# Joao-M-Silva/padel_analytics

Measured on AMD Instinct MI355X. Metric: frames/sec (all trackers) on 1280x720, higher is better.
Workload: dtype f32-equivalent (h2: fp16 pairs h + m/2048, 2 or 3 f16 MFMA products per multiply, fp32 accumulate)

## Files before the change

### include/padel_hip.h

```cpp
#ifndef PADEL_HIP_H
#define PADEL_HIP_H

#include <stddef.h>
#include <stdint.h>

#ifdef __cplusplus
extern "C" {
#endif

typedef struct pa_engine pa_engine;
typedef struct pa_model pa_model;

#define PA_ABI_VERSION 5


enum pa_op_kind {
    PA_OP_STEM = 1,
    PA_OP_CONV = 2,
    PA_OP_SPPF_POOL = 3,
    PA_OP_UPSAMPLE2X = 4,
    PA_OP_MAXPOOL2 = 5,
    PA_OP_STEM7 = 6,
    PA_OP_MAXPOOL3S2 = 7,
    PA_OP_GAP_FC = 8,
    PA_OP_DWCONV3 = 9,
    PA_OP_PSA_ATTN = 10
};

enum pa_act { PA_ACT_NONE = 0, PA_ACT_SILU = 1, PA_ACT_RELU = 2, PA_ACT_SIGMOID = 3, PA_ACT_LEAKY = 4  };

typedef struct pa_buf_desc {
    int32_t level;
    int32_t channels;
} pa_buf_desc;

typedef struct pa_op_desc {
    int32_t kind;
    int32_t in_buf, in_choff, cin;
    int32_t out_buf, out_choff, cout;
    int32_t ksize, stride, act;
    int32_t res_buf, res_choff;
    int32_t npad;
    int32_t reserved;
    int64_t w_off, b_off;
    int32_t flags;
    int32_t pad_;
} pa_op_desc;
#define PA_CONV_W_SINGLE 1
#define PA_CONV_RES_PREACT 4

enum pa_task { PA_TASK_DETECT = 0, PA_TASK_POSE = 1, PA_TASK_TRACKNET = 2, PA_TASK_RESNET = 3  };

enum pa_dtype { PA_DTYPE_F32 = 0, PA_DTYPE_F16 = 1, PA_DTYPE_H2 = 2 };

typedef struct pa_model_desc {
    int32_t task;
    int32_t nc;
    int32_t nk, kpt_dim;
    int32_t n_bufs;
    const pa_buf_desc* bufs;
    int32_t n_ops;
    const pa_op_desc* ops;
    int32_t head_buf[3];
    int32_t in_channels;
    int32_t dtype;
} pa_model_desc;

int pa_abi_version(void);
int pa_device_count(void);
int pa_engine_create(int device_id, pa_engine** out);
void pa_engine_destroy(pa_engine* eng);
const char* pa_last_error(pa_engine* eng);
int pa_engine_synchronize(pa_engine* eng);

int pa_device_malloc(pa_engine* eng, size_t nbytes, void** out_dev);
int pa_device_free(pa_engine* eng, void* dev);
int pa_memcpy_h2d(pa_engine* eng, void* dst_dev, const void* src_host, size_t nbytes);
int pa_memcpy_d2h(pa_engine* eng, void* dst_host, const void* src_dev, size_t nbytes);
int pa_upload(pa_engine* eng, void* dst_dev, const void* src_host, size_t nbytes);

int pa_host_register(pa_engine* eng, void* ptr, size_t nbytes);
int pa_host_unregister(pa_engine* eng, void* ptr);

enum pa_yuv_layout {
    PA_YUV_NV12 = 0,
    PA_YUV_I420 = 1
};
typedef struct pa_yuv_desc {
    int32_t layout;
    int32_t pitch_y, pitch_c;
    int32_t off_u, off_v;
    int32_t reserved;
    int64_t frame_stride;
    int32_t y_off, cy, cvr, cug, cvg, cub;
} pa_yuv_desc;
int pa_yuv420_to_bgr(pa_engine* eng, const uint8_t* src, int src_on_device, int n, int h, int w,
                     const pa_yuv_desc* d, uint8_t* dst_bgr_dev);
int pa_yuv_last_path(pa_engine* eng);

enum pa_mark_kind { PA_MARK_DISC = 1, PA_MARK_SEGMENT = 2, PA_MARK_FILL = 3, PA_MARK_BOX = 4, PA_MARK_GLYPH = 5, PA_MARK_BLEND = 6 };
typedef struct pa_mark {
    int32_t kind;
    int32_t x0, y0, x1, y1;
    int32_t size;
    uint32_t bgr;
    int32_t arg;
} pa_mark;
typedef struct pa_yuv_enc {
    int32_t y_off;
    int32_t yr, yg, yb, ur, ug, ub, vr, vg, vb;
} pa_yuv_enc;
enum pa_render_out { PA_RENDER_BGR = 0, PA_RENDER_YUV420 = 1 };
int pa_render(pa_engine* eng, const uint8_t* src_bgr_dev, int n, int h, int w, const pa_mark* marks_host, const int32_t* first_host,
              int out, const pa_yuv_desc* geom, const pa_yuv_enc* enc, uint8_t* dst_dev);
int pa_render_check(int n, int h, int w, const pa_mark* marks_host, const int32_t* first_host, int out, const pa_yuv_desc* geom,
                    const pa_yuv_enc* enc, char* why, size_t cap);
int pa_render_last_path(pa_engine* eng);
int pa_glyph_rows(int code, uint8_t rows[7]);

#define PA_JPEG_MAX_WIDTH 2560
int pa_jpeg_encode(pa_engine* eng, const uint8_t* src_yuv_dev, int n, int h, int w, const pa_yuv_desc* geom, int quality,
                   uint8_t* dst_host, size_t cap, int64_t* offsets_host);
int pa_jpeg_check(int n, int h, int w, const pa_yuv_desc* geom, int quality, char* why, size_t cap);
size_t pa_jpeg_interval_bytes(int w);

#define PA_JPEG_DEC_MAX_DIM 4096
#define PA_JPEG_DEC_MAX_BYTES (1 << 27)
enum { PA_JPEG_ST_CODE = 1, PA_JPEG_ST_INDEX = 2, PA_JPEG_ST_SIZE = 4, PA_JPEG_ST_DATA = 8, PA_JPEG_ST_MARKERS = 16 };
typedef struct pa_jpeg_huff {
    uint8_t bits[16];
    uint8_t vals[256];
    int32_t nvals;
} pa_jpeg_huff;
typedef struct pa_jpeg_interval {
    int64_t begin, end;
    int32_t first_mcu, mcus;
} pa_jpeg_interval;
typedef struct pa_jpeg_frame_info {
    int32_t w, h, mcus_x, mcus_y;
    int32_t restart_interval;
    int32_t n_intervals;
    int32_t default_huffman;
    int32_t status;
    int64_t scan_begin, scan_end;
    uint8_t quant[3][64];
    uint8_t comp_dc[3], comp_ac[3], pad_[2];
    pa_jpeg_huff dc[2], ac[2];
} pa_jpeg_frame_info;
int pa_jpeg_parse(const uint8_t* jpeg, size_t len, pa_jpeg_frame_info* info, pa_jpeg_interval* ivls, size_t ivl_cap, char* why,
                  size_t cap);
int pa_jpeg_decode(pa_engine* eng, const uint8_t* jpegs_host, const int64_t* offsets, int n, int h, int w, uint8_t* dst_bgr_dev,
                   int32_t* status_host);
int pa_jpeg_decode_last_path(pa_engine* eng);
int pa_jpeg_decode_last_times(pa_engine* eng, double ms[5]);

int pa_engine_timer_start(pa_engine* eng);
int pa_engine_timer_stop(pa_engine* eng, float* ms);

int pa_engine_set_tuning(pa_engine* eng, const char* key, int value);
int pa_engine_set_timeline_path(pa_engine* eng, const char* path);

int pa_model_create(pa_engine* eng, const pa_model_desc* desc, const float* weights, size_t n_floats,
                    pa_model** out);
void pa_model_destroy(pa_model* m);
int pa_model_take_overflow(pa_model* m, int* out);
int pa_model_set_max_batch(pa_model* m, int max_batch);
int pa_model_plan_bytes(pa_model* m, size_t* arena_bytes, size_t* logical_bytes);

int pa_model_fill_arena(pa_model* m, int byte_value);

enum pa_pre_mode {
    PA_PRE_LETTERBOX = 0,
    PA_PRE_PIL_STRETCH = 1
};

typedef struct pa_yolo_params {
    int32_t imgsz;
    int32_t pre_mode;
    int32_t channel_reverse;
    int32_t letterbox_auto;
    float conf, iou;
    int32_t max_det;
    int32_t n_classes;
    const int32_t* classes;
    int32_t frames_on_device;
} pa_yolo_params;

int pa_yolo_infer(pa_model* m, const uint8_t* frames, int n, int h, int w, const pa_yolo_params* p,
                  float* out_boxes, float* out_kpts, int32_t* out_counts);

#define PA_MAX_INFLIGHT 4
int pa_yolo_submit(pa_model* m, const uint8_t* frames, int n, int h, int w, const pa_yolo_params* p,
                   float* out_boxes, float* out_kpts, int32_t* out_counts, int* ticket);
int pa_yolo_wait(pa_model* m, int ticket, int* overflow);

int pa_yolo_postprocess(pa_model* m, const float* const* heads, int n, int h, int w, const pa_yolo_params* p,
                        float* out_boxes, float* out_kpts, int32_t* out_counts);

int pa_yolo_head_shape(pa_model* m, int level, int* h, int* w, int* c);
int pa_yolo_read_head(pa_model* m, int level, int n, float* out);

int pa_yolo_netin_shape(pa_model* m, int* h, int* w);
int pa_yolo_read_netin(pa_model* m, int n, uint8_t* out);

int pa_tracknet_infer(pa_model* m, const float* x, int n, int h, int w, int x_on_device, float* out,
                      int out_on_device);

int pa_resnet_infer(pa_model* m, const uint8_t* frames, int n, int h, int w, int frames_on_device, float* out_xy, float* out_logits);
int pa_resnet_read_netin(pa_model* m, int n, uint8_t* out);
int pa_resnet_read_fc(pa_model* m, int n, float* out_xy, float* out_logits);
int pa_resnet_read_head(pa_model* m, int n, float* out);

int pa_pil_coeffs(int in_size, int out_size, int filter, int32_t* bounds, int32_t* coefs, int coefs_cap, int* ksize);

typedef struct pa_ball pa_ball;
int pa_ball_create(pa_model* tracknet, int src_h, int src_w, pa_ball** out);
void pa_ball_destroy(pa_ball* b);
int pa_ball_set_background(pa_ball* b, const uint8_t* median_rgb);
int pa_ball_background_from_frames(pa_ball* b, const uint8_t* frames_bgr, int n, int frames_on_device,
                                   uint8_t* out_median_rgb);
int pa_ball_feed(pa_ball* b, const uint8_t* frames_bgr, int n, int frames_on_device, int flush,
                 uint8_t* out_masks, float* out_heat, int32_t* out_rects, int* out_count);

int pa_ball_locate(pa_ball* b, const uint8_t* masks, int n, int32_t* out_rects);

int pa_ball_read_resized(pa_ball* b, long long frame, uint8_t* out);

int pa_comm_unique_id(void* out, size_t cap);
int pa_engine_comm_init(pa_engine* eng, const void* unique_id, size_t id_bytes, int nranks, int rank);
void pa_engine_comm_destroy(pa_engine* eng);
int pa_engine_bcast_weights(pa_engine* eng, pa_model* m, int root);
int pa_engine_bcast_weights_from(pa_engine* eng, pa_model* src, pa_model* dst, int root);
int pa_engine_bcast(pa_engine* eng, void* dev_ptr, size_t nbytes, int root);
int pa_engine_allreduce_max(pa_engine* eng, double* value);
int pa_engine_gather_sizes(pa_engine* eng, size_t nbytes, uint64_t* sizes);
int pa_engine_gather(pa_engine* eng, const void* send, size_t nbytes, void* recv, size_t recv_cap, const uint64_t* sizes, int root);

typedef struct pa_bytetrack pa_bytetrack;
int pa_bytetrack_create(double track_activation_threshold, int lost_track_buffer, double minimum_matching_threshold,
                        int frame_rate, pa_bytetrack** out);
void pa_bytetrack_destroy(pa_bytetrack* b);
void pa_bytetrack_reset(pa_bytetrack* b);
int pa_bytetrack_update_batch(pa_bytetrack* b, const float* boxes, const int32_t* counts, const uint8_t* keep,
                              int n_frames, int stride, int32_t* out_ids);

int pa_engine_set_profiling(pa_engine* eng, int enable);
int pa_model_last_profile(pa_model* m, int cap, int32_t* kinds, float* ms, double* flops, int32_t* ksizes);
int pa_model_profile_text(pa_model* m, char* buf, size_t cap);

#ifdef __cplusplus
}
#endif
#endif
```

### padel_analytics_amd/csrc/engine.cpp

```cpp
#include "engine_internal.h"

thread_local std::string g_err;

static int knob_raw(int v) { return v; }
static int knob_flag(int v) { return v ? 1 : 0; }
static int knob_tap_pd(int v) { return v == 3 ? 3 : 2; }
static const struct Knob { const char* key; const char* env; int Tuning::*field; int (*norm)(int); } kKnobs[] = {
    {"variant", "PADEL_CONV_VARIANT", &Tuning::variant, knob_raw},
    {"tune", "PADEL_CONV_TUNE", &Tuning::tune, knob_raw},
    {"tap_pd", "PADEL_CONV_TAP_PD", &Tuning::tap_pd, knob_tap_pd},
    {"graph", "PADEL_GRAPH", &Tuning::graph, knob_flag},
    {"timeline", nullptr, &Tuning::timeline, knob_flag},
    {"alias", "PADEL_ALIAS", &Tuning::alias, knob_flag},
    {"fold_up", "PADEL_FOLD_UP", &Tuning::fold_up, knob_flag},
    {"fuse_stem", "PADEL_FUSE_STEM", &Tuning::fuse_stem, knob_raw},
    {"fuse_sppf", "PADEL_FUSE_SPPF", &Tuning::fuse_sppf, knob_raw},
    {"w_single", nullptr, &Tuning::w_single, knob_flag},
};

int pa_abi_version(void) { return PA_ABI_VERSION; }

int pa_device_count(void) {
    int n = 0;
    if (hipGetDeviceCount(&n) != hipSuccess) return 0;
    return n;
}

const char* pa_last_error(pa_engine* eng) { return eng ? eng->err.c_str() : g_err.c_str(); }

int pa_engine_create(int device_id, pa_engine** out) {
    if (!out) PA_FAIL((pa_engine*)nullptr, "pa_engine_create: out is NULL");
    int n = 0;
    PA_HIP((pa_engine*)nullptr, hipGetDeviceCount(&n));
    if (device_id < 0 || device_id >= n) PA_FAIL((pa_engine*)nullptr, "pa_engine_create: device %d of %d", device_id, n);
    PA_HIP((pa_engine*)nullptr, hipSetDevice(device_id));
    pa_engine* e = new pa_engine();
    e->dev = device_id;
    hipError_t r = hipStreamCreateWithFlags(&e->stream, hipStreamNonBlocking);
    if (r != hipSuccess) { delete e; PA_FAIL((pa_engine*)nullptr, "hipStreamCreate: %s", hipGetErrorString(r)); }
    if (r == hipSuccess) r = hipStreamCreateWithFlags(&e->copy_stream, hipStreamNonBlocking);
    if (r != hipSuccess) { delete e; PA_FAIL((pa_engine*)nullptr, "hipStreamCreate: %s", hipGetErrorString(r)); }
    r = hipMalloc((void**)&e->zeros, 256);
    if (r == hipSuccess) r = hipMemset(e->zeros, 0, 256);
    if (r != hipSuccess) { delete e; PA_FAIL((pa_engine*)nullptr, "zero page: %s", hipGetErrorString(r)); }
    r = padel::init_misc_kernels();
    if (r != hipSuccess) { delete e; PA_FAIL((pa_engine*)nullptr, "kernel attributes: %s", hipGetErrorString(r)); }
    if (const char* v = getenv("PADEL_CONV_IMPL")) {
        if (v[0] == 'l') { delete e; PA_FAIL((pa_engine*)nullptr, "PADEL_CONV_IMPL=%s: the LDS kernel was retired in round 5; tap or bx3", v); }
        e->t.impl = (v[0] == 'b') ? 2 : 0;
    }
    for (const Knob& k : kKnobs)
        if (const char* v = k.env ? getenv(k.env) : nullptr) e->t.*k.field = k.norm(atoi(v));
    *out = e;
    return 0;
}

int pa_engine_set_tuning(pa_engine* e, const char* key, int value) {
    if (!e || !key) return 1;
    if (!strcmp(key, "impl")) {
        if (value != 0 && value != 2) PA_FAIL(e, "tuning impl = %d: 0 (fp32-input MFMA tap kernels) or 2 (bf16x3); 1 was the LDS kernel, retired in round 5 (tools/legacy_conv)", value);
        e->t.impl = value;
    } else {
        const Knob* k = std::find_if(std::begin(kKnobs), std::end(kKnobs), [&](const Knob& c) { return !strcmp(c.key, key); });
        if (k == std::end(kKnobs)) PA_FAIL(e, "pa_engine_set_tuning: unknown key '%s'", key);
        e->t.*k->field = k->norm(value);
    }
    e->tuning_epoch++;
    return 0;
}

int pa_engine_set_timeline_path(pa_engine* e, const char* path) {
    if (!e) return 1;
    e->timeline_path = path ? path : "";
    return 0;
}

void pa_engine_destroy(pa_engine* e) {
    if (!e) return;
    hipSetDevice(e->dev);
    pa_engine_comm_destroy(e);
    if (e->zeros) hipFree(e->zeros);
    if (e->yuv_stage) { if (e->stream) hipStreamSynchronize(e->stream); hipFree(e->yuv_stage); }
    if (e->render_stage) { if (e->stream) hipStreamSynchronize(e->stream); hipFree(e->render_stage); }
    jpeg_scratch_free(e);
    jpeg_dec_scratch_free(e);
    for (hipEvent_t ev : e->timer_ev) if (ev) hipEventDestroy(ev);
    if (e->stream) hipStreamDestroy(e->stream);
    if (e->copy_stream) hipStreamDestroy(e->copy_stream);
    delete e;
}

int pa_engine_synchronize(pa_engine* e) {
    PA_HIP(e, hipSetDevice(e->dev));
    PA_HIP(e, hipStreamSynchronize(e->stream));
    return 0;
}

int pa_engine_set_profiling(pa_engine* e, int enable) { e->profiling = enable != 0; return 0; }

int pa_device_malloc(pa_engine* e, size_t nbytes, void** out) {
    PA_HIP(e, hipSetDevice(e->dev));
    PA_HIP(e, hipMalloc(out, nbytes));
    return 0;
}
int pa_device_free(pa_engine* e, void* p) {
    PA_HIP(e, hipSetDevice(e->dev));
    PA_HIP(e, hipFree(p));
    return 0;
}
int pa_memcpy_h2d(pa_engine* e, void* dst, const void* src, size_t n) {
    PA_HIP(e, hipSetDevice(e->dev));
    PA_HIP(e, hipMemcpyAsync(dst, src, n, hipMemcpyHostToDevice, e->stream));
    PA_HIP(e, hipStreamSynchronize(e->stream));
    return 0;
}
int pa_upload(pa_engine* e, void* dst, const void* src, size_t n) {
    PA_HIP(e, hipSetDevice(e->dev));
    PA_HIP(e, hipMemcpyAsync(dst, src, n, hipMemcpyHostToDevice, e->copy_stream));
    PA_HIP(e, hipStreamSynchronize(e->copy_stream));
    return 0;
}
int pa_host_register(pa_engine* e, void* ptr, size_t nbytes) {
    PA_HIP(e, hipSetDevice(e->dev));
    PA_HIP(e, hipHostRegister(ptr, nbytes, hipHostRegisterDefault));
    return 0;
}
int pa_host_unregister(pa_engine* e, void* ptr) {
    PA_HIP(e, hipSetDevice(e->dev));
    PA_HIP(e, hipHostUnregister(ptr));
    return 0;
}
int pa_memcpy_d2h(pa_engine* e, void* dst, const void* src, size_t n) {
    PA_HIP(e, hipSetDevice(e->dev));
    PA_HIP(e, hipMemcpyAsync(dst, src, n, hipMemcpyDeviceToHost, e->stream));
    PA_HIP(e, hipStreamSynchronize(e->stream));
    return 0;
}

int pa_engine_timer_start(pa_engine* e) {
    if (!e) return 1;
    PA_HIP(e, hipSetDevice(e->dev));
    for (hipEvent_t& ev : e->timer_ev) if (!ev) PA_HIP(e, hipEventCreate(&ev));
    PA_HIP(e, hipEventRecord(e->timer_ev[0], e->stream));
    return 0;
}
int pa_engine_timer_stop(pa_engine* e, float* ms) {
    if (!e || !ms) return 1;
    if (!e->timer_ev[0] || !e->timer_ev[1]) PA_FAIL(e, "pa_engine_timer_stop without pa_engine_timer_start");
    PA_HIP(e, hipSetDevice(e->dev));
    PA_HIP(e, hipEventRecord(e->timer_ev[1], e->stream));
    PA_HIP(e, hipEventSynchronize(e->timer_ev[1]));
    PA_HIP(e, hipEventElapsedTime(ms, e->timer_ev[0], e->timer_ev[1]));
    return 0;
}

int pa_model_create(pa_engine* e, const pa_model_desc* desc, const float* weights, size_t n_floats, pa_model** out) {
    if (!e || !desc || !out) PA_FAIL(e, "pa_model_create: NULL argument");
    std::string why;
    if (validate_desc(desc, n_floats, why)) PA_FAIL(e, "%s", why.c_str());
    PA_HIP(e, hipSetDevice(e->dev));
    pa_model* m = new pa_model();
    m->e = e;
    m->d = *desc;
    m->bufs.assign(desc->bufs, desc->bufs + desc->n_bufs);
    m->ops.assign(desc->ops, desc->ops + desc->n_ops);
    m->d.bufs = m->bufs.data();
    m->d.ops = m->ops.data();
    find_upsample_folds(m->d, m->fold_src, m->fold_dst);
    m->stem_fuse.resize(m->ops.size());
    for (size_t i = 0; i < m->ops.size(); ++i) m->stem_fuse[i] = stem_fusable(m->d, i);
    m->n_w = n_floats;
    hipError_t r = hipMalloc((void**)&m->d_w, n_floats * sizeof(float) + kConvReadSlack);
    if (r == hipSuccess)
        r = weights ? hipMemcpyAsync(m->d_w, weights, n_floats * sizeof(float), hipMemcpyHostToDevice, e->stream)
                    : hipMemsetAsync(m->d_w, 0, n_floats * sizeof(float), e->stream);
    if (r == hipSuccess) r = hipMemsetAsync(m->d_w + n_floats, 0, kConvReadSlack, e->stream);
    if (r == hipSuccess) r = hipMalloc((void**)&m->d_ovf, 256);
    if (r == hipSuccess) r = hipMemsetAsync(m->d_ovf, 0, 256, e->stream);
    if (r == hipSuccess) r = hipHostMalloc((void**)&m->h_pin, 64 * sizeof(unsigned), hipHostMallocDefault);
    if (r == hipSuccess) memset(m->h_pin, 0, 64 * sizeof(unsigned));
    for (int k = 0; k < PA_MAX_INFLIGHT && r == hipSuccess; ++k) r = hipEventCreateWithFlags(&m->tk_ev[k], hipEventDisableTiming);
    if (r == hipSuccess) r = hipStreamSynchronize(e->stream);
    if (r != hipSuccess) { delete m; PA_FAIL(e, "weights upload: %s", hipGetErrorString(r)); }
    *out = m;
    return 0;
}

static void destroy_graphs(pa_model* m) {
    for (auto& g : m->graphs) hipGraphExecDestroy(g.second);
    m->graphs.clear();
}

void free_plan(pa_model* m) {
    destroy_graphs(m);
    if (m->arena) hipFree(m->arena);
    m->arena = nullptr;
    m->bptr.clear();
    void* ptrs[] = {m->d_netin, m->d_xtab, m->d_ytab, m->d_cand,
                    m->d_cidx, m->d_ccnt, m->d_keys, m->d_order, m->d_supp, m->d_oboxes, m->d_okpts, m->d_ocnt, m->d_fc};
    for (void* p : ptrs) if (p) hipFree(p);
    resample_free(&m->rs);
    m->d_fc = nullptr;
    m->d_netin = nullptr;
    m->d_xtab = m->d_ytab = nullptr;
    m->d_cand = nullptr; m->d_cidx = m->d_ccnt = nullptr; m->d_keys = nullptr; m->d_order = nullptr; m->d_supp = nullptr;
    m->d_oboxes = m->d_okpts = nullptr; m->d_ocnt = nullptr;
    m->planned = false;
}

void pa_model_destroy(pa_model* m) {
    if (!m) return;
    hipSetDevice(m->e->dev);
    hipStreamSynchronize(m->e->stream);
    free_plan(m);
    for (auto& r : m->prof) { hipEventDestroy(r.e0); hipEventDestroy(r.e1); }
    if (m->d_frames) hipFree(m->d_frames);
    if (m->d_classes) hipFree(m->d_classes);
    if (m->d_w) hipFree(m->d_w);
    if (m->d_wr) hipFree(m->d_wr);
    if (m->d_ovf) hipFree(m->d_ovf);
    if (m->d_stage) hipFree(m->d_stage);
    if (m->h_pin) hipHostFree(m->h_pin);
    for (int k = 0; k < PA_MAX_INFLIGHT; ++k) if (m->tk_ev[k]) hipEventDestroy(m->tk_ev[k]);
    delete m;
}

int pa_model_take_overflow(pa_model* m, int* out) {
    if (!m || !out) return 1;
    pa_engine* e = m->e;
    *out = 0;
    if (m->d.dtype != PA_DTYPE_H2) return 0;
    PA_HIP(e, hipSetDevice(e->dev));
    unsigned v = 0;
    if (m->ovf_cached) {
        v = m->h_ovf;
    } else {
        PA_HIP(e, hipMemcpyAsync(&v, m->d_ovf, sizeof(v), hipMemcpyDeviceToHost, e->stream));
        PA_HIP(e, hipStreamSynchronize(e->stream));
    }
    m->ovf_cached = false;
    m->h_ovf = 0;
    if (v) {
        PA_HIP(e, hipMemsetAsync(m->d_ovf, 0, sizeof(v), e->stream));
        PA_HIP(e, hipStreamSynchronize(e->stream));
    }
    *out = v ? 1 : 0;
    return 0;
}

int pa_model_set_max_batch(pa_model* m, int max_batch) {
    if (max_batch < 1) PA_FAIL(m->e, "max_batch %d", max_batch);
    if (max_batch != m->max_batch) { hipSetDevice(m->e->dev); hipStreamSynchronize(m->e->stream); free_plan(m); m->max_batch = max_batch; }
    return 0;
}

int plan_buffers(pa_model* m, int batch) {
    pa_engine* e = m->e;
    BufferPlan bp;
    std::string why;
    if (plan_activations(m->d, m->fold_src, m->net_h, m->net_w, batch, e->t.alias != 0, bp, why)) PA_FAIL(e, "%s", why.c_str());
    m->fc_nout = 0;
    for (const auto& o : m->ops) if (o.kind == PA_OP_GAP_FC) m->fc_nout = o.cout;
    if (m->fc_nout) {
        PA_HIP(e, hipMalloc((void**)&m->d_fc, (size_t)batch * 2 * kGapFcMaxOut * sizeof(float)));
        PA_HIP(e, hipMemsetAsync(m->d_fc, 0, (size_t)batch * 2 * kGapFcMaxOut * sizeof(float), e->stream));
    }
    PA_HIP(e, hipMalloc(&m->arena, bp.arena_bytes + kConvReadSlack));
    PA_HIP(e, hipMemsetAsync(m->arena, 0, bp.arena_bytes + kConvReadSlack, e->stream));
    m->bptr.assign(m->bufs.size(), nullptr);
    for (size_t i = 0; i < m->bufs.size(); ++i) m->bptr[i] = reinterpret_cast<float*>(static_cast<char*>(m->arena) + bp.off[i]);
    m->arena_bytes = bp.arena_bytes;
    m->logical_bytes = bp.logical_bytes;
    m->p_batch = batch;
    return 0;
}

ProfRec* prof_begin(pa_model* m, size_t idx, int kind, int ksize, double flops) {
    if (!m->e->profiling) return nullptr;
    if (m->prof.size() <= idx) {
        m->prof.resize(idx + 1);
        hipEventCreate(&m->prof[idx].e0);
        hipEventCreate(&m->prof[idx].e1);
    }
    ProfRec* r = &m->prof[idx];
    r->kind = kind; r->ksize = ksize; r->flops = flops; r->ms = 0.f;
    r->M = r->cout = r->cin = r->stride = r->mf = r->nf = r->res = 0;
    r->tile = -1; r->family = "";
    hipEventRecord(r->e0, m->e->stream);
    return r;
}

static bool fold_active(const pa_model* m, int conv_op) {
    if (m->d.dtype == PA_DTYPE_H2) return m->e->t.fold_up && m->fold_src[conv_op] >= 0;
    return m->e->t.fold_up && m->e->t.impl == 2 && m->d.dtype != PA_DTYPE_F16 && m->fold_src[conv_op] >= 0;
}

static int conv_launch_args(const pa_model* m, size_t i, int n, ConvArgs& a, int* path_out = nullptr) {
    const pa_engine* e = m->e;
    const pa_op_desc& o = m->ops[i];
    const pa_buf_desc& ob = m->bufs[o.out_buf];
    const pa_buf_desc& ib = m->bufs[o.in_buf];
    const int Ho = m->net_h >> ob.level, Wo = m->net_w >> ob.level;
    a.in = m->bptr[o.in_buf]; a.in_cs = ib.channels; a.in_choff = o.in_choff;
    a.out = m->bptr[o.out_buf]; a.out_cs = ob.channels; a.out_choff = o.out_choff;
    a.res = o.res_buf >= 0 ? m->bptr[o.res_buf] : nullptr;
    a.res_cs = o.res_buf >= 0 ? m->bufs[o.res_buf].channels : 0; a.res_choff = o.res_choff;
    a.res_pre = (o.res_buf >= 0 && (o.flags & PA_CONV_RES_PREACT)) ? 1 : 0;
    a.zeros = e->zeros;
    a.w = m->d_w + o.w_off; a.bias = m->d_w + o.b_off;
    a.H = m->net_h >> ib.level; a.W = m->net_w >> ib.level; a.Ho = Ho; a.Wo = Wo;
    a.cin = o.cin; a.cout = o.cout; a.n16 = o.npad / 16; a.ksize = o.ksize; a.stride = o.stride; a.act = o.act;
    a.M = n * Ho * Wo;
    fill_fastdiv((unsigned)(Ho * Wo), &a.howo_magic, &a.howo_shift);
    fill_fastdiv((unsigned)Wo, &a.wo_magic, &a.wo_shift);
    a.tune = e->t.tune; a.tap_pd = e->t.tap_pd;
    const bool f16 = m->d.dtype == PA_DTYPE_F16, h2 = m->d.dtype == PA_DTYPE_H2;
    const bool use_bx3 = !f16 && !h2 && e->t.impl == 2 && o.reserved > 0;
    a.w3 = use_bx3 ? (const void*)(m->d_w + o.reserved) : nullptr;
    a.out_f32 = (f16 || h2) && is_head_buf(m->d, o.out_buf);
    const int path = h2 ? CONV_PATH_H2 : f16 ? CONV_PATH_F16 : use_bx3 ? CONV_PATH_BX3 : CONV_PATH_TAP;
    if (path_out) *path_out = path;
    if (h2) {
        a.oscale = m->d_w + o.reserved;
        a.ovf_flag = m->d_ovf;
        a.w_single = (o.flags & PA_CONV_W_SINGLE) && e->t.w_single ? 1 : 0;
        a.wr = (m->wr_valid && i < m->wr_off.size() && m->wr_off[i] >= 0) ? (const void*)(m->d_wr + m->wr_off[i]) : nullptr;
    }
    const int lv = e->t.variant >= 0 ? e->t.variant
                   : h2 ? choose_conv_h2_variant(a)
                   : f16 ? choose_conv_tap16_variant(a)
                   : use_bx3 ? choose_conv_bx3_variant(a)
                         : choose_conv_tap_variant(a.M, a.n16);
    if ((h2 || use_bx3) && fold_active(m, (int)i)) {
        const pa_op_desc& u = m->ops[m->fold_src[i]];
        a.in2 = m->bptr[u.in_buf]; a.in2_cs = m->bufs[u.in_buf].channels; a.in2_choff = u.in_choff; a.up_c = u.cin;
        if (!resolve_conv(path, a, lv, nullptr)) { a.in2 = nullptr; a.in2_cs = a.in2_choff = a.up_c = 0; }
    }
    return lv;
}

static int run_ops(pa_model* m, int n, size_t* pi) {
    pa_engine* e = m->e;
    hipStream_t s = e->stream;
    for (size_t i = 0; i < m->ops.size(); ++i) {
        const pa_op_desc& o = m->ops[i];
        const pa_buf_desc& ob = m->bufs[o.out_buf];
        const int Ho = m->net_h >> ob.level, Wo = m->net_w >> ob.level;
        hipError_t r = hipSuccess;
        ProfRec* pr = nullptr;
        if (o.kind == PA_OP_CONV) {
            ConvArgs a{};
            int path = CONV_PATH_TAP;
            const int lv = conv_launch_args(m, i, n, a, &path);
            const bool f16 = path == CONV_PATH_F16, h2 = path == CONV_PATH_H2, use_bx3 = path == CONV_PATH_BX3;
            int bm = 0, bn = 0;
            conv_tile_shape(path, lv, &bm, &bn);
            pr = prof_begin(m, (*pi)++, o.kind, o.ksize, 2.0 * a.M * (double)o.cout * o.cin * o.ksize * o.ksize);
            if (pr) { pr->M = a.M; pr->cout = o.cout; pr->cin = o.cin; pr->stride = o.stride; pr->mf = bm; pr->nf = bn; pr->res = a.res != nullptr; }
            unsigned long long* dbg_dev = nullptr;
            size_t dbg_bytes = 0;
            ConvLaunched will{-1, ""};
            if (e->t.timeline && !e->timeline_path.empty() && resolve_conv(path, a, lv, &will) && will.tile == lv) {
                const size_t patches = (size_t)n * ((a.Ho + 7) / 8) * ((a.Wo + 15) / 16);
                const size_t records = h2 ? 8 * ((patches + 7) / 8) * (size_t)((a.n16 + 5) / 6) : (size_t)((a.M + 63) / 64) * ((o.npad + 95) / 96);
                dbg_bytes = records * conv_timeline_words(will, o.ksize) * 8;
            }
            if (dbg_bytes) {
                if (hipMalloc(&dbg_dev, dbg_bytes) == hipSuccess) (void)hipMemsetAsync(dbg_dev, 0, dbg_bytes, s);
                else dbg_dev = nullptr;
                a.dbg = dbg_dev;
            }
            ConvLaunched ran{-1, ""};
            if (a.res_pre && !h2 && !use_bx3)
                PA_FAIL(e, "op %zu: PA_CONV_RES_PREACT needs the h2 or the bf16x3 kernels (tuning impl = 2, bf16x3 weights in the blob), not the %s family",
                        i, f16 ? "fp16" : "fp32-MFMA tap");
            r = launch_conv(path, a, lv, s, &ran);
            if (pr) { pr->tile = ran.tile; pr->family = ran.family; }
            if (dbg_dev) {
                (void)hipStreamSynchronize(s);
                std::vector<unsigned long long> host(dbg_bytes / 8);
                (void)hipMemcpy(host.data(), dbg_dev, dbg_bytes, hipMemcpyDeviceToHost);
                if (FILE* f = fopen(e->timeline_path.c_str(), "wb")) { fwrite(host.data(), 1, dbg_bytes, f); fclose(f); }
                (void)hipFree(dbg_dev);
            }
        } else if (o.kind == PA_OP_STEM) {
            StemArgs a{};
            a.in = m->d_netin; a.w = m->d_w + o.w_off; a.bias = m->d_w + o.b_off;
            a.out = m->bptr[o.out_buf]; a.out_cs = ob.channels; a.out_choff = o.out_choff;
            a.H = m->net_h; a.W = m->net_w; a.Ho = Ho; a.Wo = Wo; a.cout = o.cout; a.B = n;
            a.out_f16 = m->d.dtype == PA_DTYPE_F16 ? 1 : m->d.dtype == PA_DTYPE_H2 ? 2 : 0;
            a.ovf_flag = m->d_ovf;
            a.opw = (m->wr_valid && i < m->wr_off.size() && m->wr_off[i] >= 0) ? (const void*)(m->d_wr + m->wr_off[i]) : nullptr;
            pr = prof_begin(m, (*pi)++, o.kind, 3, 2.0 * n * Ho * Wo * (double)o.cout * 27);
            if (e->t.fuse_stem && m->d.dtype == PA_DTYPE_H2 && m->stem_fuse[i]) {
                ConvArgs ca{};
                conv_launch_args(m, i + 1, n, ca);
                if (stem_l1_h2_supported(a, ca)) {
                    r = launch_stem_l1_h2(a, ca, s);
                    prof_end(m, pr);
                    if (r != hipSuccess) PA_FAIL(e, "fused stem + layer 1 launch failed: %s", hipGetErrorString(r));
                    ++i;
                    continue;
                }
            }
            r = launch_stem(a, s);
        } else if (o.kind == PA_OP_SPPF_POOL) {
            pr = prof_begin(m, (*pi)++, o.kind, 5, 0.0);
            r = launch_sppf_pool(m->bptr[o.in_buf], m->bufs[o.in_buf].channels, o.in_choff, o.cin, n, Ho, Wo, s, (int)m->d.dtype, e->t.fuse_sppf);
        } else if (o.kind == PA_OP_UPSAMPLE2X) {
            if (m->fold_dst[i] >= 0) {
                ConvArgs ca{};
                conv_launch_args(m, (size_t)m->fold_dst[i], n, ca);
                if (ca.in2) continue;
            }
            pr = prof_begin(m, (*pi)++, o.kind, 0, 0.0);
            r = launch_upsample2x(m->bptr[o.in_buf], m->bufs[o.in_buf].channels, o.in_choff, m->bptr[o.out_buf],
                                  ob.channels, o.out_choff, o.cin, n, Ho / 2, Wo / 2, s, (int)m->d.dtype);
        } else if (o.kind == PA_OP_MAXPOOL2) {
            pr = prof_begin(m, (*pi)++, o.kind, 2, 0.0);
            r = launch_maxpool2(m->bptr[o.in_buf], m->bufs[o.in_buf].channels, o.in_choff, m->bptr[o.out_buf],
                                ob.channels, o.out_choff, o.cin, n, Ho * 2, Wo * 2, s, (int)m->d.dtype);
        } else if (o.kind == PA_OP_MAXPOOL3S2) {
            const int lin = m->bufs[o.in_buf].level;
            pr = prof_begin(m, (*pi)++, o.kind, 3, 0.0);
            r = launch_maxpool3s2(m->bptr[o.in_buf], m->bufs[o.in_buf].channels, o.in_choff, m->bptr[o.out_buf], ob.channels, o.out_choff,
                                  o.cin, n, m->net_h >> lin, m->net_w >> lin, Ho, Wo, s, m->d.dtype == PA_DTYPE_H2 ? 1 : 0);
        } else if (o.kind == PA_OP_STEM7) {
            if (!m->d_netin) PA_FAIL(e, "op %zu: the 7x7 stem reads the u8 network input of pa_resnet_infer", i);
            const bool head = is_head_buf(m->d, o.out_buf);
            Stem7Args a{};
            a.in = m->d_netin; a.w = m->d_w + o.w_off; a.bias = m->d_w + o.b_off; a.lut = m->d_w + o.reserved;
            a.out = m->bptr[o.out_buf]; a.out_cs = ob.channels; a.out_choff = o.out_choff;
            a.H = m->net_h; a.W = m->net_w; a.Ho = Ho; a.Wo = Wo; a.B = n; a.act = o.act;
            a.out_h2 = (m->d.dtype == PA_DTYPE_H2 && !head) ? 1 : 0;
            a.ovf_flag = m->d_ovf;
            pr = prof_begin(m, (*pi)++, o.kind, 7, 2.0 * n * Ho * Wo * 64.0 * 147.0);
            if (pr) { pr->M = n * Ho * Wo; pr->cout = 64; pr->cin = 3; pr->stride = 2; }
            r = launch_stem7(a, s);
        } else if (o.kind == PA_OP_GAP_FC) {
            const int lin = m->bufs[o.in_buf].level;
            const int hw = (m->net_h >> lin) * (m->net_w >> lin);
            pr = prof_begin(m, (*pi)++, o.kind, 0, 2.0 * n * (double)o.cout * o.cin);
            if (pr) { pr->M = n; pr->cout = o.cout; pr->cin = o.cin; }
            r = launch_gap_fc(m->bptr[o.in_buf], m->bufs[o.in_buf].channels, o.in_choff, o.cin, n, hw, m->d_w + o.w_off, m->d_w + o.b_off,
                              o.cout, m->d_fc, m->d_fc + (size_t)m->p_batch * kGapFcMaxOut, s, m->d.dtype == PA_DTYPE_H2 ? 1 : 0);
        } else if (o.kind == PA_OP_DWCONV3) {
            const bool h2 = m->d.dtype == PA_DTYPE_H2;
            const bool head = is_head_buf(m->d, o.out_buf);
            DwConvArgs a{};
            a.in = m->bptr[o.in_buf]; a.in_cs = m->bufs[o.in_buf].channels; a.in_choff = o.in_choff;
            a.w = m->d_w + o.w_off; a.bias = m->d_w + o.b_off;
            a.out = m->bptr[o.out_buf]; a.out_cs = ob.channels; a.out_choff = o.out_choff;
            if (o.res_buf >= 0) { a.res = m->bptr[o.res_buf]; a.res_cs = m->bufs[o.res_buf].channels; a.res_choff = o.res_choff; }
            a.C = o.cin; a.B = n; a.H = Ho; a.W = Wo; a.act = o.act;
            a.h2 = h2 ? 1 : 0; a.out_f32 = (h2 && head) ? 1 : 0; a.ovf_flag = m->d_ovf;
            pr = prof_begin(m, (*pi)++, o.kind, 3, 2.0 * n * Ho * Wo * (double)o.cin * 9.0);
            if (pr) { pr->M = n * Ho * Wo; pr->cout = o.cout; pr->cin = o.cin; pr->stride = 1; pr->res = o.res_buf >= 0; }
            r = launch_dwconv3(a, s);
        } else if (o.kind == PA_OP_PSA_ATTN) {
            const bool h2 = m->d.dtype == PA_DTYPE_H2;
            const bool head = is_head_buf(m->d, o.out_buf);
            AttnArgs a{};
            a.heads = o.stride; a.kd = o.ksize; a.hd = o.npad;
            a.qkv = m->bptr[o.in_buf]; a.cs = m->bufs[o.in_buf].channels;
            a.q_choff = o.in_choff; a.k_choff = o.in_choff + a.heads * a.kd; a.v_choff = o.in_choff + 2 * a.heads * a.kd;
            a.out = m->bptr[o.out_buf]; a.out_cs = ob.channels; a.out_choff = o.out_choff;
            a.N = Ho * Wo; a.B = n; a.scale = (float)(1.0 / std::sqrt((double)a.kd));
            a.h2 = h2 ? 1 : 0; a.out_f32 = (h2 && head) ? 1 : 0; a.ovf_flag = m->d_ovf;
            pr = prof_begin(m, (*pi)++, o.kind, 0, 2.0 * n * (double)a.heads * a.N * (double)a.N * (a.kd + a.hd));
            if (pr) { pr->M = n * a.N; pr->cout = o.cout; pr->cin = o.cin; pr->stride = a.heads; }
            r = launch_psa_attn(a, s);
        }
        prof_end(m, pr);
        if (r != hipSuccess) PA_FAIL(e, "op %zu (kind %d) launch failed: %s", i, o.kind, hipGetErrorString(r));
    }
    return 0;
}

static int ensure_operand_copies(pa_model* m) {
    if (m->wr_valid || m->d.dtype != PA_DTYPE_H2) return 0;
    pa_engine* e = m->e;
    {
        bool any = false;
        PA_HIP(e, hipMemsetAsync(m->d_ovf + 32, 0, sizeof(unsigned) * 8, e->stream));
        for (size_t i = 0; i < m->ops.size(); ++i) {
            const pa_op_desc& o = m->ops[i];
            if (o.kind != PA_OP_CONV || !(o.flags & PA_CONV_W_SINGLE)) continue;
            PA_HIP(e, launch_h2_mplane_check(m->d_w + o.w_off, (long long)o.npad * h2_ksteps(o.cin, o.ksize), m->d_ovf + 32, e->stream));
            any = true;
        }
        if (any) {
            unsigned bad = 0;
            PA_HIP(e, hipMemcpyAsync(&bad, m->d_ovf + 32, sizeof(bad), hipMemcpyDeviceToHost, e->stream));
            PA_HIP(e, hipStreamSynchronize(e->stream));
            if (bad) PA_FAIL(e, "a conv flagged PA_CONV_W_SINGLE has a non-zero m plane in the weight blob (pack it without the flag, or with fp16-number weights)");
        }
    }
    if (m->wr_off.empty()) {
        std::vector<long long> off(m->ops.size(), -1);
        size_t total = 0;
        for (size_t i = 0; i < m->ops.size(); ++i) {
            const pa_op_desc& o = m->ops[i];
            if (o.kind == PA_OP_STEM && m->stem_fuse[i] && (o.cout == 16 || o.cout == 32 || o.cout == 48)) {
                off[i] = (long long)total;
                total += (stem_l1_operand_bytes(o.cout) + 2047) / 2048 * 2048;
                continue;
            }
            if (o.kind != PA_OP_CONV || !conv_wants_operand_copy(o.ksize, o.stride, o.cin, (o.flags & PA_CONV_W_SINGLE) != 0)) continue;
            off[i] = (long long)total;
            total += conv_h2r_copy_bytes(o.npad / 16, o.cin, o.ksize);
        }
        if (total) {
            PA_HIP(e, hipMalloc((void**)&m->d_wr, total + 8192));
            PA_HIP(e, hipMemsetAsync(m->d_wr + total, 0, 8192, e->stream));
        }
        m->wr_off = std::move(off);
    }
    for (size_t i = 0; i < m->ops.size(); ++i) {
        if (m->wr_off[i] < 0) continue;
        const pa_op_desc& o = m->ops[i];
        if (o.kind == PA_OP_STEM) {
            PA_HIP(e, launch_stem_l1_operands(m->d_w + o.w_off, o.cout, m->d_wr + m->wr_off[i], e->stream));
            continue;
        }
        PA_HIP(e, launch_h2r_repack(m->d_w + o.w_off, m->d_wr + m->wr_off[i], o.npad / 16, o.cin, o.ksize, e->stream));
    }
    m->wr_valid = true;
    return 0;
}

int run_graph(pa_model* m, int n, size_t* pi) {
    pa_engine* e = m->e;
    if (ensure_operand_copies(m)) return 1;
    if (!e->t.graph || e->profiling || e->t.timeline) return run_ops(m, n, pi);
    if (m->graph_epoch != e->tuning_epoch) {
        PA_HIP(e, hipStreamSynchronize(e->stream));
        destroy_graphs(m);
        m->graph_epoch = e->tuning_epoch;
    }
    auto it = m->graphs.find(n);
    if (it == m->graphs.end()) {
        hipGraph_t g = nullptr;
        hipGraphExec_t ge = nullptr;
        PA_HIP(e, hipStreamBeginCapture(e->stream, hipStreamCaptureModeThreadLocal));
        size_t dummy = 0;
        const int rc = run_ops(m, n, &dummy);
        const hipError_t r = hipStreamEndCapture(e->stream, &g);
        if (rc) { if (g) hipGraphDestroy(g); return 1; }
        if (r != hipSuccess) PA_FAIL(e, "hipStreamEndCapture: %s", hipGetErrorString(r));
        const hipError_t ri = hipGraphInstantiate(&ge, g, nullptr, nullptr, 0);
        hipGraphDestroy(g);
        if (ri != hipSuccess) PA_FAIL(e, "hipGraphInstantiate: %s", hipGetErrorString(ri));
        it = m->graphs.emplace(n, ge).first;
    }
    PA_HIP(e, hipGraphLaunch(it->second, e->stream));
    return 0;
}

int finish_profile(pa_model* m, size_t n_rec) {
    if (!m->e->profiling) { m->n_prof = 0; return 0; }
    for (size_t i = 0; i < n_rec && i < m->prof.size(); ++i)
        hipEventElapsedTime(&m->prof[i].ms, m->prof[i].e0, m->prof[i].e1);
    m->n_prof = n_rec;
    return 0;
}

int pa_model_plan_bytes(pa_model* m, size_t* arena_bytes, size_t* logical_bytes) {
    if (!m->planned) PA_FAIL(m->e, "pa_model_plan_bytes: no plan yet");
    if (arena_bytes) *arena_bytes = m->arena_bytes;
    if (logical_bytes) *logical_bytes = m->logical_bytes;
    return 0;
}

int pa_model_fill_arena(pa_model* m, int byte_value) {
    if (!m) return 1;
    pa_engine* e = m->e;
    if (!m->planned || !m->arena) PA_FAIL(e, "pa_model_fill_arena: no plan yet");
    PA_HIP(e, hipSetDevice(e->dev));
    PA_HIP(e, hipMemsetAsync(m->arena, byte_value & 0xFF, m->arena_bytes, e->stream));
    if (m->d_netin) PA_HIP(e, hipMemsetAsync(m->d_netin, byte_value & 0xFF, (size_t)m->p_batch * m->net_h * m->net_w * 4, e->stream));
    PA_HIP(e, hipStreamSynchronize(e->stream));
    return 0;
}

int pa_model_profile_text(pa_model* m, char* buf, size_t cap) {
    size_t off = 0;
    for (size_t i = 0; i < m->n_prof && i < m->prof.size(); ++i) {
        const ProfRec& r = m->prof[i];
        int n = snprintf(buf + off, off < cap ? cap - off : 0, "%d,%d,%d,%d,%d,%d,%d,%d,%.5f,%.0f,%d,%d,%s\n", r.kind, r.ksize, r.M, r.cout,
                         r.cin, r.stride, r.mf, r.nf, r.ms, r.flops, r.res, r.tile, r.family ? r.family : "");
        if (n < 0 || off + n >= cap) break;
        off += n;
    }
    if (off < cap) buf[off] = 0;
    return (int)off;
}

int pa_model_last_profile(pa_model* m, int cap, int32_t* kinds, float* ms, double* flops, int32_t* ksizes) {
    int n = 0;
    for (size_t i = 0; i < m->n_prof && i < m->prof.size() && n < cap; ++i, ++n) {
        kinds[n] = m->prof[i].kind; ms[n] = m->prof[i].ms; flops[n] = m->prof[i].flops; ksizes[n] = m->prof[i].ksize;
    }
    return n;
}
```

### padel_analytics_amd/csrc/engine_internal.h

```cpp
#pragma once
#include "../../include/padel_hip.h"
#include "graph_plan.h"
#include "kernels.h"

#include <algorithm>
#include <cmath>
#include <cstdio>
#include <cstdlib>
#include <cstring>
#include <map>
#include <string>
#include <vector>

using namespace padel;

struct Tuning {
    int impl = 2;
    int variant = -1;
    int tune = 1;
    int tap_pd = 2;
    int graph = 0;
    int timeline = 0;
    int alias = 1;
    int fuse_stem = 1;
    int w_single = 1;
    int fuse_sppf = 1;
    int fold_up = 1;
};

struct pa_comm;
struct JpegScratch;
struct JpegDecScratch;

struct pa_engine {
    int dev = 0;
    hipStream_t stream = nullptr;
    hipStream_t copy_stream = nullptr;
    std::string err;
    bool profiling = false;
    float* zeros = nullptr;
    Tuning t;
    int tuning_epoch = 0;
    std::string timeline_path;
    pa_comm* comm = nullptr;
    uint8_t* yuv_stage = nullptr; size_t yuv_stage_cap = 0;
    int yuv_last_path = 0;
    hipEvent_t timer_ev[2]{};
    uint8_t* render_stage = nullptr; size_t render_stage_cap = 0;
    int render_last_path = 0;
    JpegScratch* jpeg = nullptr;
    JpegDecScratch* jpeg_dec = nullptr;
    int jpeg_dec_last_path = 0;
};

extern thread_local std::string g_err;

#define PA_FAIL(eng, ...)                                        \
    do {                                                         \
        char _b[512];                                            \
        snprintf(_b, sizeof(_b), __VA_ARGS__);                   \
        if (eng) (eng)->err = _b; else g_err = _b;               \
        return 1;                                                \
    } while (0)

#define PA_HIP(eng, call)                                                                  \
    do {                                                                                   \
        hipError_t _e = (call);                                                            \
        if (_e != hipSuccess) {                                                            \
            (void)hipGetLastError();    \
            PA_FAIL(eng, "%s failed: %s (%s:%d)", #call, hipGetErrorString(_e), __FILE__, __LINE__); \
        }                                                                                  \
    } while (0)

struct ProfRec { int kind; int ksize; double flops; hipEvent_t e0, e1; float ms; int M, cout, cin, stride, mf, nf, res; int tile; const char* family; };
enum { PROF_PRE = 100, PROF_DECODE = 101, PROF_NMS = 102 };

struct ResamplePlan {
    int sh = 0, sw = 0, dh = 0, dw = 0;
    int32_t *d_hb = nullptr, *d_hk = nullptr, *d_vb = nullptr, *d_vk = nullptr;
    int hks = 0, vks = 0;
    uint8_t* d_tmp = nullptr;
};

struct pa_model {
    pa_engine* e = nullptr;
    pa_model_desc d{};
    std::vector<pa_buf_desc> bufs;
    std::vector<pa_op_desc> ops;
    std::vector<int> fold_src;
    std::vector<int> fold_dst;
    std::vector<char> stem_fuse;
    float* d_w = nullptr;
    size_t n_w = 0;
    char* d_wr = nullptr;
    std::vector<long long> wr_off;
    bool wr_valid = false;
    unsigned* d_ovf = nullptr;
    float* d_stage = nullptr; size_t stage_cap = 0;
    float* d_fc = nullptr;
    int fc_nout = 0;
    int max_batch = 64;

    bool planned = false;
    int p_h0 = 0, p_w0 = 0, p_imgsz = 0, p_pre = 0, p_auto = 0, p_batch = 0;
    int net_h = 0, net_w = 0;
    int rw = 0, rh = 0, top = 0, left = 0, lb_mode = 0;
    std::vector<float*> bptr;
    void* arena = nullptr;
    size_t arena_bytes = 0, logical_bytes = 0;
    unsigned h_ovf = 0;
    bool ovf_cached = false;
    unsigned* h_pin = nullptr;
    hipEvent_t tk_ev[PA_MAX_INFLIGHT]{};
    bool tk_busy[PA_MAX_INFLIGHT]{};
    int next_ticket = 0, n_inflight = 0;
    std::vector<int32_t> classes_host;
    std::map<int, hipGraphExec_t> graphs;
    int graph_epoch = -1;
    uint8_t* d_frames = nullptr; size_t frames_cap = 0;
    uint8_t* d_netin = nullptr;
    int32_t *d_xtab = nullptr, *d_ytab = nullptr;
    ResamplePlan rs;
    int A = 0, P2 = 0;
    HeadLevel lv[3]{};
    float* d_cand = nullptr; int32_t* d_cidx = nullptr; int32_t* d_ccnt = nullptr;
    uint64_t* d_keys = nullptr; int32_t* d_order = nullptr; uint8_t* d_supp = nullptr;
    float* d_oboxes = nullptr; float* d_okpts = nullptr; int32_t* d_ocnt = nullptr;
    int32_t* d_classes = nullptr; int classes_cap = 0;
    int last_n = 0;
    std::vector<ProfRec> prof;
    size_t n_prof = 0;
};

ProfRec* prof_begin(pa_model* m, size_t idx, int kind, int ksize, double flops);
inline void prof_end(pa_model* m, ProfRec* r) { if (r) hipEventRecord(r->e1, m->e->stream); }
int finish_profile(pa_model* m, size_t n_rec);
void free_plan(pa_model* m);
int plan_buffers(pa_model* m, int batch);
int run_graph(pa_model* m, int n, size_t* pi);

void jpeg_scratch_free(pa_engine* e);

void jpeg_dec_scratch_free(pa_engine* e);

hipError_t upload_table(pa_engine* e, int32_t** dptr, const std::vector<int32_t>& v);
int stage_frames(pa_model* m, const uint8_t** src, int nb, size_t frame_bytes);
int resample_plan(pa_engine* e, ResamplePlan* rs, int sh, int sw, int dh, int dw, int filter, int max_batch, bool identity_pass = false);
void resample_free(ResamplePlan* rs);
hipError_t resample_enqueue(const ResamplePlan& rs, const uint8_t* src, uint8_t* dst, int n, int out_c, int reverse, hipStream_t s);
```

### padel_analytics_amd/csrc/engine_yolo.cpp

```cpp
#include "engine_internal.h"

static int plan_yolo(pa_model* m, int h0, int w0, const pa_yolo_params* p) {
    pa_engine* e = m->e;
    PA_HIP(e, hipStreamSynchronize(e->stream));
    free_plan(m);
    const int S = p->imgsz;
    YoloGeometry g;
    std::string why;
    if (yolo_geometry(h0, w0, S, p->pre_mode, p->letterbox_auto, g, why)) PA_FAIL(e, "%s", why.c_str());
    m->rw = g.rw; m->rh = g.rh; m->top = g.top; m->left = g.left; m->lb_mode = g.lb_mode;
    m->net_h = g.net_h; m->net_w = g.net_w;
    if (m->lb_mode == 2) {
        std::vector<int32_t> xt, yt;
        cv2_linear_table(w0, m->rw, xt);
        cv2_linear_table(h0, m->rh, yt);
        PA_HIP(e, upload_table(e, &m->d_xtab, xt));
        PA_HIP(e, upload_table(e, &m->d_ytab, yt));
    }
    if (p->pre_mode == PA_PRE_PIL_STRETCH && resample_plan(e, &m->rs, h0, w0, S, S, PIL_BICUBIC, m->max_batch)) return 1;
    const int B = m->max_batch;
    PA_HIP(e, hipMalloc((void**)&m->d_netin, (size_t)B * m->net_h * m->net_w * 4));
    if (plan_buffers(m, B)) return 1;
    for (int l = 0; l < 3; ++l) m->lv[l] = HeadLevel{m->bptr[m->d.head_buf[l]], g.lv[l].H, g.lv[l].W, g.lv[l].stride, g.lv[l].anchor0};
    m->A = g.A;
    m->P2 = g.P2;
    PA_HIP(e, hipMalloc((void**)&m->d_cand, (size_t)B * m->A * 6 * sizeof(float)));
    PA_HIP(e, hipMalloc((void**)&m->d_cidx, (size_t)B * m->A * sizeof(int32_t)));
    PA_HIP(e, hipMalloc((void**)&m->d_ccnt, (size_t)B * sizeof(int32_t)));
    PA_HIP(e, hipMalloc((void**)&m->d_keys, (size_t)B * m->P2 * sizeof(uint64_t)));
    PA_HIP(e, hipMalloc((void**)&m->d_order, (size_t)B * m->A * sizeof(int32_t)));
    PA_HIP(e, hipMalloc((void**)&m->d_supp, (size_t)B * m->A));
    PA_HIP(e, hipMalloc((void**)&m->d_oboxes, (size_t)B * 300 * 6 * sizeof(float)));
    PA_HIP(e, hipMalloc((void**)&m->d_ocnt, (size_t)B * sizeof(int32_t)));
    if (m->d.nk) PA_HIP(e, hipMalloc((void**)&m->d_okpts, (size_t)B * 300 * m->d.nk * sizeof(float)));
    PA_HIP(e, hipStreamSynchronize(e->stream));
    m->p_h0 = h0; m->p_w0 = w0; m->p_imgsz = S; m->p_pre = p->pre_mode; m->p_auto = p->letterbox_auto;
    m->planned = true;
    return 0;
}

static int run_post(pa_model* m, const pa_yolo_params* p, int nb, int oh, int ow, size_t* ppi, float* out_boxes, float* out_kpts,
                int32_t* out_counts, int ovf_slot) {
    pa_engine* e = m->e;
    hipStream_t s = e->stream;
    size_t& pi = *ppi;
    ProfRec* pr = nullptr;
    hipError_t r = hipSuccess;
    const double gain = std::min((double)m->net_h / oh, (double)m->net_w / ow);
    const double kpx = (m->net_w - ow * gain) / 2, kpy = (m->net_h - oh * gain) / 2;
    DecodeArgs da{};
    for (int l = 0; l < 3; ++l) da.lv[l] = m->lv[l];
    da.cs = m->bufs[m->d.head_buf[0]].channels; da.nc = m->d.nc; da.nk = m->d.nk; da.kdim = m->d.kpt_dim;
    da.A = m->A; da.B = nb; da.conf = p->conf; da.classes = m->d_classes; da.n_classes = p->n_classes;
    da.cand = m->d_cand; da.cand_idx = m->d_cidx; da.cand_cnt = m->d_ccnt;
    pr = prof_begin(m, pi++, PROF_DECODE, 0, 0.0);
    r = launch_decode(da, s);
    prof_end(m, pr);
    if (r != hipSuccess) PA_FAIL(e, "decode launch failed: %s", hipGetErrorString(r));
    NmsArgs na{};
    na.cand = m->d_cand; na.cand_idx = m->d_cidx; na.cand_cnt = m->d_ccnt; na.keys = m->d_keys;
    na.order = m->d_order; na.supp = m->d_supp;
    for (int l = 0; l < 3; ++l) na.lv[l] = m->lv[l];
    na.cs = da.cs; na.nc = m->d.nc; na.nk = m->d.nk; na.kdim = m->d.kpt_dim; na.A = m->A; na.B = nb; na.P2 = m->P2;
    na.iou = p->iou; na.max_det = p->max_det; na.max_nms = 30000;
    na.gain = (float)gain;
    na.pad_x = (float)std::nearbyint(kpx - 0.1); na.pad_y = (float)std::nearbyint(kpy - 0.1);
    na.kpad_x = (float)kpx; na.kpad_y = (float)kpy;
    na.w0 = (float)ow; na.h0 = (float)oh;
    na.out_boxes = m->d_oboxes; na.out_kpts = m->d_okpts; na.out_cnt = m->d_ocnt;
    pr = prof_begin(m, pi++, PROF_NMS, 0, 0.0);
    r = launch_nms(na, s);
    prof_end(m, pr);
    if (r != hipSuccess) PA_FAIL(e, "nms launch failed: %s", hipGetErrorString(r));
    if (m->d.dtype == PA_DTYPE_H2)
        PA_HIP(e, hipMemcpyAsync(m->h_pin + ovf_slot, m->d_ovf, sizeof(unsigned), hipMemcpyDeviceToHost, s));
    PA_HIP(e, hipMemcpyAsync(out_counts, m->d_ocnt, nb * sizeof(int32_t), hipMemcpyDeviceToHost, s));
    PA_HIP(e, hipMemcpyAsync(out_boxes, m->d_oboxes,
                             (size_t)nb * p->max_det * 6 * sizeof(float), hipMemcpyDeviceToHost, s));
    if (m->d.nk)
        PA_HIP(e, hipMemcpyAsync(out_kpts, m->d_okpts,
                                 (size_t)nb * p->max_det * m->d.nk * sizeof(float), hipMemcpyDeviceToHost, s));
    return 0;
}

static bool yolo_plan_current(const pa_model* m, int h, int w, const pa_yolo_params* p) {
    return m->planned && m->p_h0 == h && m->p_w0 == w && m->p_imgsz == p->imgsz && m->p_pre == p->pre_mode &&
           m->p_auto == p->letterbox_auto && m->p_batch == m->max_batch;
}

static int set_classes(pa_model* m, const pa_yolo_params* p) {
    pa_engine* e = m->e;
    if (p->n_classes <= 0) return 0;
    if ((int)m->classes_host.size() == p->n_classes && !memcmp(m->classes_host.data(), p->classes, p->n_classes * sizeof(int32_t))) return 0;
    PA_HIP(e, hipStreamSynchronize(e->stream));
    if (p->n_classes > m->classes_cap) {
        if (m->d_classes) hipFree(m->d_classes);
        m->d_classes = nullptr; m->classes_cap = 0; m->classes_host.clear();
        PA_HIP(e, hipMalloc((void**)&m->d_classes, p->n_classes * sizeof(int32_t)));
        m->classes_cap = p->n_classes;
    }
    m->classes_host.assign(p->classes, p->classes + p->n_classes);
    PA_HIP(e, hipMemcpy(m->d_classes, m->classes_host.data(), p->n_classes * sizeof(int32_t), hipMemcpyHostToDevice));
    return 0;
}

static int yolo_prepare(pa_model* m, const uint8_t* frames, int n, int h, int w, const pa_yolo_params* p, float* out_boxes,
                        float* out_kpts, int32_t* out_counts, const char* who) {
    pa_engine* e = m->e;
    if (m->d.task != PA_TASK_DETECT && m->d.task != PA_TASK_POSE) PA_FAIL(e, "%s on a non-YOLO model", who);
    if (!frames || n <= 0 || h <= 0 || w <= 0 || !out_boxes || !out_counts) PA_FAIL(e, "%s: bad arguments", who);
    if (m->d.nk && !out_kpts) PA_FAIL(e, "%s: out_kpts is NULL for a pose model", who);
    if (p->max_det < 1 || p->max_det > 300) PA_FAIL(e, "max_det %d outside [1,300]", p->max_det);
    PA_HIP(e, hipSetDevice(e->dev));
    if (!yolo_plan_current(m, h, w, p)) {
        if (m->n_inflight) PA_FAIL(e, "%s: the plan would change (source size / imgsz / batch) with %d ticket(s) in flight", who, m->n_inflight);
        if (plan_yolo(m, h, w, p)) return 1;
    }
    return set_classes(m, p);
}

static int yolo_enqueue(pa_model* m, const uint8_t* src, int nb, int h, int w, const pa_yolo_params* p, float* out_boxes,
                        float* out_kpts, int32_t* out_counts, int ovf_slot, size_t* ppi) {
    pa_engine* e = m->e;
    hipStream_t s = e->stream;
    size_t& pi = *ppi;
    const size_t frame_bytes = (size_t)h * w * 3;
    const int S = p->imgsz;
    const int oh = p->pre_mode == PA_PRE_PIL_STRETCH ? S : h, ow = p->pre_mode == PA_PRE_PIL_STRETCH ? S : w;
    if (!p->frames_on_device && stage_frames(m, &src, nb, frame_bytes)) return 1;
    ProfRec* pr = prof_begin(m, pi++, PROF_PRE, 0, 0.0);
    hipError_t r = hipSuccess;
    if (p->pre_mode == PA_PRE_LETTERBOX || (h == S && w == S)) {
        LetterboxArgs a{};
        a.src = src; a.dst = m->d_netin; a.B = nb; a.h0 = h; a.w0 = w; a.rw = m->rw; a.rh = m->rh;
        a.top = m->top; a.left = m->left; a.nh = m->net_h; a.nw = m->net_w; a.mode = m->lb_mode;
        a.reverse = p->channel_reverse; a.xtab = m->d_xtab; a.ytab = m->d_ytab;
        r = launch_letterbox(a, s);
    } else {
        r = resample_enqueue(m->rs, src, m->d_netin, nb, 4, p->channel_reverse, s);
    }
    prof_end(m, pr);
    if (r != hipSuccess) PA_FAIL(e, "preprocess launch failed: %s", hipGetErrorString(r));
    if (run_graph(m, nb, &pi)) return 1;
    return run_post(m, p, nb, oh, ow, &pi, out_boxes, m->d.nk ? out_kpts : nullptr, out_counts, ovf_slot);
}

int pa_yolo_infer(pa_model* m, const uint8_t* frames, int n, int h, int w, const pa_yolo_params* p,
                  float* out_boxes, float* out_kpts, int32_t* out_counts) {
    if (!m || !p) return 1;
    pa_engine* e = m->e;
    if (yolo_prepare(m, frames, n, h, w, p, out_boxes, out_kpts, out_counts, "pa_yolo_infer")) return 1;
    hipStream_t s = e->stream;
    const size_t frame_bytes = (size_t)h * w * 3;
    size_t pi = 0;
    for (int c0 = 0; c0 < n; c0 += m->max_batch) {
        const int nb = std::min(m->max_batch, n - c0);
        if (yolo_enqueue(m, frames + (size_t)c0 * frame_bytes, nb, h, w, p, out_boxes + (size_t)c0 * p->max_det * 6,
                         m->d.nk ? out_kpts + (size_t)c0 * p->max_det * m->d.nk : nullptr, out_counts + c0, PA_MAX_INFLIGHT, &pi))
            return 1;
        PA_HIP(e, hipStreamSynchronize(s));
        m->last_n = nb;
        if (m->d.dtype == PA_DTYPE_H2) { m->h_ovf |= m->h_pin[PA_MAX_INFLIGHT]; m->ovf_cached = true; }
    }
    finish_profile(m, pi);
    return 0;
}

int pa_yolo_submit(pa_model* m, const uint8_t* frames, int n, int h, int w, const pa_yolo_params* p,
                   float* out_boxes, float* out_kpts, int32_t* out_counts, int* ticket) {
    if (!m || !p || !ticket) return 1;
    pa_engine* e = m->e;
    if (!p->frames_on_device) PA_FAIL(e, "pa_yolo_submit: frames must be in HBM (frames_on_device = 1)");
    if (n > m->max_batch) PA_FAIL(e, "pa_yolo_submit: n = %d > max_batch %d", n, m->max_batch);
    if (e->profiling || e->t.timeline) PA_FAIL(e, "pa_yolo_submit: not while profiling (use pa_yolo_infer)");
    const int slot = m->next_ticket % PA_MAX_INFLIGHT;
    if (m->tk_busy[slot]) PA_FAIL(e, "pa_yolo_submit: %d tickets in flight (PA_MAX_INFLIGHT)", PA_MAX_INFLIGHT);
    if (yolo_prepare(m, frames, n, h, w, p, out_boxes, out_kpts, out_counts, "pa_yolo_submit")) return 1;
    size_t pi = 0;
    if (yolo_enqueue(m, frames, n, h, w, p, out_boxes, out_kpts, out_counts, slot, &pi)) {
        (void)hipStreamSynchronize(e->stream);
        return 1;
    }
    PA_HIP(e, hipEventRecord(m->tk_ev[slot], e->stream));
    m->tk_busy[slot] = true;
    ++m->n_inflight;
    m->last_n = n;
    m->n_prof = 0;
    m->ovf_cached = false;
    *ticket = m->next_ticket++;
    return 0;
}

int pa_yolo_wait(pa_model* m, int ticket, int* overflow) {
    if (!m) return 1;
    pa_engine* e = m->e;
    const int slot = ticket % PA_MAX_INFLIGHT;
    if (ticket < 0 || ticket >= m->next_ticket || ticket + PA_MAX_INFLIGHT < m->next_ticket || !m->tk_busy[slot])
        PA_FAIL(e, "pa_yolo_wait: ticket %d is not in flight", ticket);
    PA_HIP(e, hipSetDevice(e->dev));
    PA_HIP(e, hipEventSynchronize(m->tk_ev[slot]));
    m->tk_busy[slot] = false;
    --m->n_inflight;
    if (overflow) *overflow = (m->d.dtype == PA_DTYPE_H2 && m->h_pin[slot]) ? 1 : 0;
    return 0;
}

int pa_yolo_postprocess(pa_model* m, const float* const* heads, int n, int h, int w, const pa_yolo_params* p,
                        float* out_boxes, float* out_kpts, int32_t* out_counts) {
    if (!m || !p || !heads) return 1;
    pa_engine* e = m->e;
    if (m->d.task != PA_TASK_DETECT && m->d.task != PA_TASK_POSE) PA_FAIL(e, "pa_yolo_postprocess on a non-YOLO model");
    if (n <= 0 || n > m->max_batch || !out_boxes || !out_counts || (m->d.nk && !out_kpts)) PA_FAIL(e, "pa_yolo_postprocess: bad arguments");
    if (p->max_det < 1 || p->max_det > 300) PA_FAIL(e, "max_det %d outside [1,300]", p->max_det);
    PA_HIP(e, hipSetDevice(e->dev));
    if (!yolo_plan_current(m, h, w, p) && plan_yolo(m, h, w, p)) return 1;
    if (set_classes(m, p)) return 1;
    hipStream_t s = e->stream;
    const int cs = m->bufs[m->d.head_buf[0]].channels;
    for (int l = 0; l < 3; ++l) {
        if (!heads[l]) PA_FAIL(e, "pa_yolo_postprocess: heads[%d] is NULL", l);
        PA_HIP(e, hipMemcpyAsync(const_cast<float*>(m->lv[l].buf), heads[l], (size_t)n * m->lv[l].H * m->lv[l].W * cs * sizeof(float),
                                 hipMemcpyHostToDevice, s));
    }
    const int S = p->imgsz;
    const int oh = p->pre_mode == PA_PRE_PIL_STRETCH ? S : h, ow = p->pre_mode == PA_PRE_PIL_STRETCH ? S : w;
    size_t pi = 0;
    if (run_post(m, p, n, oh, ow, &pi, out_boxes, out_kpts, out_counts, PA_MAX_INFLIGHT)) return 1;
    PA_HIP(e, hipStreamSynchronize(s));
    m->last_n = n;
    finish_profile(m, pi);
    return 0;
}

int pa_yolo_head_shape(pa_model* m, int level, int* h, int* w, int* c) {
    if (!m->planned || level < 0 || level > 2) PA_FAIL(m->e, "pa_yolo_head_shape: no plan / bad level");
    *h = m->lv[level].H; *w = m->lv[level].W; *c = m->bufs[m->d.head_buf[0]].channels;
    return 0;
}

int pa_yolo_read_head(pa_model* m, int level, int n, float* out) {
    pa_engine* e = m->e;
    if (!m->planned || level < 0 || level > 2 || n > m->last_n) PA_FAIL(e, "pa_yolo_read_head: no plan / bad level / n");
    PA_HIP(e, hipSetDevice(e->dev));
    const size_t bytes = (size_t)n * m->lv[level].H * m->lv[level].W * m->bufs[m->d.head_buf[0]].channels * sizeof(float);
    PA_HIP(e, hipMemcpyAsync(out, m->lv[level].buf, bytes, hipMemcpyDeviceToHost, e->stream));
    PA_HIP(e, hipStreamSynchronize(e->stream));
    return 0;
}

int pa_yolo_netin_shape(pa_model* m, int* h, int* w) {
    if (!m->planned || m->d.task == PA_TASK_TRACKNET) PA_FAIL(m->e, "pa_yolo_netin_shape: no YOLO plan");
    *h = m->net_h; *w = m->net_w;
    return 0;
}

int pa_yolo_read_netin(pa_model* m, int n, uint8_t* out) {
    pa_engine* e = m->e;
    if (!m->planned || !m->d_netin || n < 1 || n > m->last_n || !out) PA_FAIL(e, "pa_yolo_read_netin: no plan / bad n");
    PA_HIP(e, hipSetDevice(e->dev));
    PA_HIP(e, hipMemcpyAsync(out, m->d_netin, (size_t)n * m->net_h * m->net_w * 4, hipMemcpyDeviceToHost, e->stream));
    PA_HIP(e, hipStreamSynchronize(e->stream));
    return 0;
}
```

### padel_analytics_amd/csrc/graph_plan.cpp

```cpp
#include "graph_plan.h"
#include "kernels.h"

#include <algorithm>
#include <cmath>
#include <cstdio>

namespace padel {

#define FAIL(...)                                                \
    do {                                                         \
        char _b[512];                                            \
        snprintf(_b, sizeof(_b), __VA_ARGS__);                   \
        err = _b;                                                \
        return 1;                                                \
    } while (0)

int validate_desc(const pa_model_desc* d, size_t n_floats, std::string& err) {
    if (d->n_bufs <= 0 || d->n_ops <= 0 || !d->bufs || !d->ops) FAIL("model desc: empty graph");
    const bool f16 = d->dtype == PA_DTYPE_F16, h2 = d->dtype == PA_DTYPE_H2;
    if (d->dtype != PA_DTYPE_F32 && d->dtype != PA_DTYPE_F16 && d->dtype != PA_DTYPE_H2) FAIL("model desc: dtype %d", d->dtype);
    const int kalign = f16 ? 31 : 15, valign = f16 ? 7 : 3;
    for (int i = 0; i < d->n_bufs; ++i)
        if (d->bufs[i].level < 0 || d->bufs[i].level > 6 || d->bufs[i].channels <= 0 || (d->bufs[i].channels & 3))
            FAIL("model desc: buffer %d (level %d, channels %d)", i, d->bufs[i].level, d->bufs[i].channels);
    auto okslice = [&](int b, int off, int c) {
        return b >= 0 && b < d->n_bufs && off >= 0 && c > 0 && off + c <= d->bufs[b].channels;
    };
    if (h2)
        for (int i = 0; i < d->n_bufs; ++i)
            if (!is_head_buf(*d, i) && (d->bufs[i].channels & 15)) FAIL("model desc: h2 buffer %d has %d channels", i, d->bufs[i].channels);
    for (int i = 0; i < d->n_ops; ++i) {
        const pa_op_desc& o = d->ops[i];
        if (o.kind != PA_OP_GAP_FC && !okslice(o.out_buf, o.out_choff, o.cout)) FAIL("op %d: bad output slice", i);
        if (f16 && (o.kind == PA_OP_SPPF_POOL || o.kind == PA_OP_UPSAMPLE2X || o.kind == PA_OP_MAXPOOL2) &&
            ((d->bufs[o.out_buf].channels & 7) || (o.in_buf >= 0 && o.in_buf < d->n_bufs && (d->bufs[o.in_buf].channels & 7))))
            FAIL("op %d: fp16 pool / upsample buffers must be a multiple of 8 channels wide", i);
        const bool from_netin = o.kind == PA_OP_STEM || o.kind == PA_OP_STEM7;
        if (h2 && !from_netin && (((o.in_choff | o.cin) & 15) || (!is_head_buf(*d, o.out_buf) && (o.out_choff & 3))))
            FAIL("op %d: h2 slices must start on a 16-channel group", i);
        if (!from_netin && !okslice(o.in_buf, o.in_choff, o.cin)) FAIL("op %d: bad input slice", i);
        if (o.kind == PA_OP_CONV) {
            if ((o.cin & kalign) || (o.in_choff & valign) || (o.ksize != 1 && o.ksize != 3) || (o.stride != 1 && o.stride != 2))
                FAIL("op %d: unsupported conv (cin %d choff %d k %d s %d)", i, o.cin, o.in_choff, o.ksize, o.stride);
            if (o.npad < o.cout || (o.npad & 15)) FAIL("op %d: npad %d for cout %d", i, o.npad, o.cout);
            const size_t ksteps3 = (size_t)h2_ksteps(o.cin, o.ksize);
            const size_t wn = h2 ? (size_t)o.npad * ksteps3 * 32 : (size_t)o.npad * o.cin * o.ksize * o.ksize / (f16 ? 2 : 1);
            if (o.w_off < 0 || (o.w_off & 3) || (size_t)o.w_off + wn > n_floats || o.b_off < 0 ||
                (size_t)o.b_off + o.npad > n_floats)
                FAIL("op %d: weights outside the blob", i);
            if (o.res_buf >= 0 && !okslice(o.res_buf, o.res_choff, o.cout)) FAIL("op %d: bad residual slice", i);
            if (o.flags & PA_CONV_RES_PREACT) {
                if (o.res_buf < 0) FAIL("op %d: PA_CONV_RES_PREACT without a residual slice", i);
                if (f16) FAIL("op %d: PA_CONV_RES_PREACT is not implemented for fp16 storage (h2 and fp32 / bf16x3 models only)", i);
            }
            if (h2) {
                if (o.reserved <= 0 || (o.reserved & 3) || (size_t)o.reserved + o.npad > n_floats) FAIL("op %d: h2 row scales outside the blob", i);
                if (o.res_buf >= 0 && (o.res_choff & 3)) FAIL("op %d: h2 residual slice alignment", i);
            } else if (o.reserved < 0 || (o.reserved & 3) || (o.reserved > 0 && (size_t)o.reserved + (size_t)o.npad * 48 * ksteps3 > n_floats))
                FAIL("op %d: bf16x3 weights outside the blob", i);
            const int lin = d->bufs[o.in_buf].level, lout = d->bufs[o.out_buf].level;
            if (lout != lin + (o.stride == 2 ? 1 : 0)) FAIL("op %d: level mismatch", i);
        } else if (o.kind == PA_OP_STEM) {
            if ((o.cout & 15) || (size_t)o.w_off + (size_t)o.cout * 27 > n_floats || (size_t)o.b_off + o.cout > n_floats)
                FAIL("op %d: bad stem", i);
            if (d->bufs[o.out_buf].level != 1) FAIL("op %d: stem output must be level 1", i);
        } else if (o.kind == PA_OP_SPPF_POOL) {
            if ((o.cin & valign) || (o.in_choff & valign) || o.in_buf != o.out_buf || !okslice(o.in_buf, o.in_choff, 4 * o.cin))
                FAIL("op %d: bad sppf slices", i);
        } else if (o.kind == PA_OP_UPSAMPLE2X) {
            if (d->bufs[o.out_buf].level != d->bufs[o.in_buf].level - 1 || o.cin != o.cout || ((o.cin | o.in_choff | o.out_choff) & valign))
                FAIL("op %d: bad upsample", i);
        } else if (o.kind == PA_OP_MAXPOOL2) {
            if (d->bufs[o.out_buf].level != d->bufs[o.in_buf].level + 1 || o.cin != o.cout || ((o.cin | o.in_choff | o.out_choff) & valign))
                FAIL("op %d: bad maxpool", i);
        } else if (o.kind == PA_OP_MAXPOOL3S2) {
            if (f16) FAIL("op %d: MaxPool2d(3, 2, 1) is not implemented for fp16 storage", i);
            if (d->bufs[o.out_buf].level != d->bufs[o.in_buf].level + 1 || o.cin != o.cout || ((o.cin | o.in_choff | o.out_choff) & 3))
                FAIL("op %d: bad 3x3 stride-2 maxpool", i);
        } else if (o.kind == PA_OP_STEM7) {
            if (f16) FAIL("op %d: the 7x7 stem is not implemented for fp16 storage", i);
            if (o.cout != 64 || o.w_off < 0 || (o.w_off & 3) || (size_t)o.w_off + 148 * 64 > n_floats || o.b_off < 0 || (o.b_off & 3) ||
                (size_t)o.b_off + 64 > n_floats || o.reserved <= 0 || (size_t)o.reserved + 768 > n_floats || (o.out_choff & (h2 ? 15 : 3)) ||
                (o.act != PA_ACT_RELU && o.act != PA_ACT_NONE))
                FAIL("op %d: bad 7x7 stem", i);
            if (d->bufs[o.out_buf].level != 1) FAIL("op %d: stem output must be level 1", i);
        } else if (o.kind == PA_OP_GAP_FC) {
            if (f16) FAIL("op %d: the pooled linear head is not implemented for fp16 storage", i);
            if (o.out_buf != o.in_buf || (o.cin & 3) || (o.in_choff & 3) || o.cin > kGapFcMaxC || o.cout < 1 || o.cout > kGapFcMaxOut || o.w_off < 0 ||
                (size_t)o.w_off + (size_t)o.cout * o.cin > n_floats || o.b_off < 0 || (size_t)o.b_off + o.cout > n_floats || o.act != PA_ACT_SIGMOID)
                FAIL("op %d: bad pooled linear head", i);
            for (int k = 0; k < i; ++k) if (d->ops[k].kind == PA_OP_GAP_FC) FAIL("op %d: a graph has one pooled linear head", i);
        } else if (o.kind == PA_OP_DWCONV3) {
            if (f16) FAIL("op %d: the depthwise conv is not implemented for fp16 storage", i);
            if (o.ksize != 3 || o.stride != 1 || o.cin != o.cout || ((o.cin | o.in_choff | o.out_choff) & 3) ||
                d->bufs[o.out_buf].level != d->bufs[o.in_buf].level || (o.act != PA_ACT_NONE && o.act != PA_ACT_SILU))
                FAIL("op %d: bad depthwise conv (3x3, stride 1, cin = cout, act none | SiLU)", i);
            if (o.w_off < 0 || (o.w_off & 3) || (size_t)o.w_off + (size_t)9 * o.cin > n_floats || o.b_off < 0 || (o.b_off & 3) ||
                (size_t)o.b_off + o.cin > n_floats)
                FAIL("op %d: weights outside the blob", i);
            if (h2 && is_head_buf(*d, o.in_buf)) FAIL("op %d: a depthwise conv cannot read an fp32 head map of an h2 model", i);
            if (o.in_buf == o.out_buf && o.in_choff < o.out_choff + o.cout && o.out_choff < o.in_choff + o.cin)
                FAIL("op %d: a depthwise conv cannot write the slice it reads", i);
            if (o.res_buf >= 0 && (!okslice(o.res_buf, o.res_choff, o.cout) || (o.res_choff & 3) || d->bufs[o.res_buf].level != d->bufs[o.out_buf].level ||
                                   (h2 && is_head_buf(*d, o.res_buf))))
                FAIL("op %d: bad residual slice", i);
        } else if (o.kind == PA_OP_PSA_ATTN) {
            if (f16) FAIL("op %d: PSA attention is not implemented for fp16 storage", i);
            if (o.ksize != 32 || o.npad != 64)
                FAIL("op %d: PSA attention is implemented for key dim 32 and head dim 64 only (got kd %d, hd %d)", i, o.ksize, o.npad);
            if (o.stride < 1 || o.cin != o.stride * 128 || o.cout != o.stride * 64 || ((o.in_choff | o.out_choff) & 3) ||
                d->bufs[o.out_buf].level != d->bufs[o.in_buf].level)
                FAIL("op %d: bad PSA attention (heads %d, cin %d, cout %d)", i, o.stride, o.cin, o.cout);
            if (h2 && is_head_buf(*d, o.in_buf)) FAIL("op %d: PSA attention cannot read an fp32 head map of an h2 model", i);
            if (o.in_buf == o.out_buf && o.in_choff < o.out_choff + o.cout && o.out_choff < o.in_choff + o.cin)
                FAIL("op %d: PSA attention cannot write the slice it reads", i);
        } else {
            FAIL("op %d: unknown kind %d", i, o.kind);
        }
    }
    if (d->task == PA_TASK_DETECT || d->task == PA_TASK_POSE) {
        for (int l = 0; l < 3; ++l) {
            const int b = d->head_buf[l];
            if (b < 0 || b >= d->n_bufs || d->bufs[b].channels < 64 + d->nc + d->nk || d->bufs[b].level != 3 + l ||
                d->bufs[b].channels != d->bufs[d->head_buf[0]].channels)
                FAIL("model desc: head buffer %d", l);
        }
        if (d->nk && (d->kpt_dim < 2 || d->kpt_dim > 3 || d->nk % d->kpt_dim)) FAIL("model desc: kpt shape");
    }
    return 0;
}

void find_upsample_folds(const pa_model_desc& d, std::vector<int>& fold_src, std::vector<int>& fold_dst) {
    const int nops = d.n_ops;
    fold_src.assign(nops, -1);
    fold_dst.assign(nops, -1);
    auto overlap = [](int a0, int an, int b0, int bn) { return a0 < b0 + bn && b0 < a0 + an; };
    for (int j = 0; j < nops; ++j) {
        const pa_op_desc& u = d.ops[j];
        if (u.kind != PA_OP_UPSAMPLE2X || (u.cin & 31)) continue;
        if (is_head_buf(d, u.out_buf)) continue;
        int reader = -1, readers = 0;
        for (int k = 0; k < nops; ++k) {
            const pa_op_desc& o = d.ops[k];
            if (k == j) continue;
            bool reads = false;
            if (o.kind == PA_OP_CONV) {
                reads = (o.in_buf == u.out_buf && overlap(o.in_choff, o.cin, u.out_choff, u.cin)) ||
                        (o.res_buf == u.out_buf && overlap(o.res_choff, o.cout, u.out_choff, u.cin));
            } else if (o.kind == PA_OP_DWCONV3) {
                reads = (o.in_buf == u.out_buf && overlap(o.in_choff, o.cin, u.out_choff, u.cin)) ||
                        (o.res_buf >= 0 && o.res_buf == u.out_buf && overlap(o.res_choff, o.cout, u.out_choff, u.cin));
            } else if (o.kind == PA_OP_SPPF_POOL) {
                reads = o.in_buf == u.out_buf && overlap(o.in_choff, 4 * o.cin, u.out_choff, u.cin);
            } else if (o.kind != PA_OP_STEM && o.kind != PA_OP_STEM7) {
                reads = o.in_buf == u.out_buf && overlap(o.in_choff, o.cin, u.out_choff, u.cin);
            }
            if (reads) { reader = k; ++readers; }
        }
        if (readers != 1 || reader < j) continue;
        const pa_op_desc& c = d.ops[reader];
        const bool shape_ok = c.kind == PA_OP_CONV && c.stride == 1 && (c.ksize == 1 || (c.ksize == 3 && (c.cin & 31) == 0));
        if (!shape_ok || c.reserved <= 0 || c.in_buf != u.out_buf || c.in_choff != u.out_choff || c.cin < u.cin ||
            fold_src[reader] >= 0)
            continue;
        bool clobbered = false;
        for (int k = j + 1; k < reader && !clobbered; ++k) {
            const pa_op_desc& o = d.ops[k];
            const int wc = o.kind == PA_OP_SPPF_POOL ? 4 * o.cin : o.cout;
            clobbered = o.out_buf == u.in_buf && overlap(o.out_choff, wc, u.in_choff, u.cin);
        }
        if (clobbered) continue;
        fold_src[reader] = j;
        fold_dst[j] = reader;
    }
}

bool stem_fusable(const pa_model_desc& d, size_t i) {
    if (i + 1 >= (size_t)d.n_ops) return false;
    const pa_op_desc& st = d.ops[i];
    const pa_op_desc& c = d.ops[i + 1];
    if (c.kind != PA_OP_CONV || c.ksize != 3 || c.stride != 2 || c.in_buf != st.out_buf || c.in_choff != st.out_choff || c.cin != st.cout ||
        c.res_buf >= 0)
        return false;
    if (is_head_buf(d, st.out_buf)) return false;
    for (size_t k = 0; k < (size_t)d.n_ops; ++k) {
        if (k == i || k == i + 1) continue;
        const pa_op_desc& o = d.ops[k];
        if (o.kind != PA_OP_STEM && o.in_buf == st.out_buf) return false;
        if ((o.kind == PA_OP_CONV || o.kind == PA_OP_DWCONV3) && o.res_buf == st.out_buf) return false;
    }
    return true;
}

int plan_activations(const pa_model_desc& d, const std::vector<int>& fold_src, int net_h, int net_w, int batch, bool alias,
                     BufferPlan& out, std::string& err) {
    int maxl = 0;
    for (int i = 0; i < d.n_bufs; ++i) maxl = std::max(maxl, d.bufs[i].level);
    const int mask = (1 << maxl) - 1;
    if ((net_h & mask) || (net_w & mask)) FAIL("network input %dx%d is not a multiple of %d", net_h, net_w, mask + 1);
    const int nb = d.n_bufs, nops = d.n_ops;
    std::vector<int> first(nb, nops + 1), last(nb, -2);
    auto touch = [&](int b, int i) { if (b >= 0 && b < nb) { first[b] = std::min(first[b], i); last[b] = std::max(last[b], i); } };
    for (int i = 0; i < nops; ++i) {
        const pa_op_desc& o = d.ops[i];
        if (o.kind != PA_OP_STEM && o.kind != PA_OP_STEM7) touch(o.in_buf, i);
        touch(o.out_buf, i);
        if ((o.kind == PA_OP_CONV || o.kind == PA_OP_DWCONV3) && o.res_buf >= 0) touch(o.res_buf, i);
        if (o.kind == PA_OP_CONV && fold_src[i] >= 0) touch(d.ops[fold_src[i]].in_buf, i);
    }
    if (d.task == PA_TASK_TRACKNET) touch(0, -1);
    const bool f16 = d.dtype == PA_DTYPE_F16;
    for (int l = 0; l < 3; ++l) touch(d.head_buf[l], nops + 1);
    if (f16) for (int l = 0; l < 3; ++l) touch(d.head_buf[l], -1);
    std::vector<size_t> bytes(nb), off(nb, 0);
    size_t logical = 0;
    for (int i = 0; i < nb; ++i) {
        const size_t H = net_h >> d.bufs[i].level, W = net_w >> d.bufs[i].level;
        const size_t es = (f16 && !is_head_buf(d, i)) ? 2 : 4;
        bytes[i] = ((size_t)batch * H * W * d.bufs[i].channels * es + kConvReadSlack + 255) & ~(size_t)255;
        logical += bytes[i];
    }
    size_t total = 0;
    if (alias) {
        std::vector<int> order(nb);
        for (int i = 0; i < nb; ++i) order[i] = i;
        std::stable_sort(order.begin(), order.end(), [&](int a, int b) { return first[a] < first[b]; });
        std::vector<int> act;
        for (int b : order) {
            if (last[b] < first[b]) continue;
            act.erase(std::remove_if(act.begin(), act.end(), [&](int a) { return last[a] < first[b]; }), act.end());
            size_t o = 0;
            for (int a : act) {
                if (o + bytes[b] <= off[a]) break;
                o = std::max(o, off[a] + bytes[a]);
            }
            off[b] = o;
            act.insert(std::upper_bound(act.begin(), act.end(), b, [&](int x, int y) { return off[x] < off[y]; }), b);
            total = std::max(total, o + bytes[b]);
        }
    } else {
        for (int i = 0; i < nb; ++i) { off[i] = total; total += bytes[i]; }
    }
    out.off = std::move(off);
    out.bytes = std::move(bytes);
    out.arena_bytes = total;
    out.logical_bytes = logical;
    return 0;
}

int yolo_geometry(int h0, int w0, int imgsz, int pre_mode, int letterbox_auto, YoloGeometry& g, std::string& err) {
    const int S = imgsz;
    if (S <= 0 || (S & 31)) FAIL("imgsz %d must be a positive multiple of 32", S);
    if (pre_mode == PA_PRE_LETTERBOX) {
        const double r = std::min((double)S / h0, (double)S / w0);
        g.rw = (int)std::nearbyint(w0 * r);
        g.rh = (int)std::nearbyint(h0 * r);
        double dw = S - g.rw, dh = S - g.rh;
        if (letterbox_auto) { dw = std::fmod(dw, 32.0); dh = std::fmod(dh, 32.0); }
        dw /= 2; dh /= 2;
        g.top = (int)std::nearbyint(dh - 0.1);
        const int bottom = (int)std::nearbyint(dh + 0.1);
        g.left = (int)std::nearbyint(dw - 0.1);
        const int right = (int)std::nearbyint(dw + 0.1);
        g.net_h = g.rh + g.top + bottom;
        g.net_w = g.rw + g.left + right;
        if (w0 == g.rw && h0 == g.rh) g.lb_mode = 0;
        else if (w0 == 2 * g.rw && h0 == 2 * g.rh) g.lb_mode = 1;
        else g.lb_mode = 2;
    } else if (pre_mode == PA_PRE_PIL_STRETCH) {
        g.net_h = g.net_w = S;
        g.rw = g.rh = S; g.top = g.left = 0; g.lb_mode = 0;
    } else {
        FAIL("unknown pre_mode %d", pre_mode);
    }
    int a0 = 0;
    for (int l = 0; l < 3; ++l) {
        g.lv[l].H = g.net_h >> (3 + l);
        g.lv[l].W = g.net_w >> (3 + l);
        g.lv[l].stride = 8 << l;
        g.lv[l].anchor0 = a0;
        a0 += g.lv[l].H * g.lv[l].W;
    }
    g.A = a0;
    if (g.A >= 65536) FAIL("%d anchors per image exceed the 16-bit sort key", g.A);
    g.P2 = 1;
    while (g.P2 < g.A) g.P2 <<= 1;
    return 0;
}

void cv2_linear_table(int src, int dst, std::vector<int32_t>& tab) {
    tab.resize((size_t)dst * 3);
    const double scale = (double)src / dst;
    for (int d = 0; d < dst; ++d) {
        float f = (float)((d + 0.5) * scale - 0.5);
        int s = (int)std::floor(f);
        f -= s;
        if (s < 0) { s = 0; f = 0.f; }
        if (s >= src - 1) { s = src - 1; f = 0.f; }
        tab[d * 3 + 0] = s;
        tab[d * 3 + 1] = (int)std::nearbyint((1.f - f) * 2048.f);
        tab[d * 3 + 2] = (int)std::nearbyint(f * 2048.f);
    }
}

static double pil_bicubic(double x) {
    const double a = -0.5;
    if (x < 0.0) x = -x;
    if (x < 1.0) return ((a + 2.0) * x - (a + 3.0)) * x * x + 1;
    if (x < 2.0) return (((x - 5) * x + 8) * x - 4) * a;
    return 0.0;
}
static double pil_bilinear(double x) {
    if (x < 0.0) x = -x;
    return x < 1.0 ? 1.0 - x : 0.0;
}
int pil_coeffs(int in_size, int out_size, std::vector<int32_t>& bounds, std::vector<int32_t>& kk, int filter) {
    const double scale = (double)in_size / out_size;
    double filterscale = scale < 1.0 ? 1.0 : scale;
    const double support = (filter == PIL_BILINEAR ? 1.0 : 2.0) * filterscale;
    const int ksize = (int)std::ceil(support) * 2 + 1;
    bounds.assign((size_t)out_size * 2, 0);
    kk.assign((size_t)out_size * ksize, 0);
    std::vector<double> k(ksize);
    for (int xx = 0; xx < out_size; ++xx) {
        const double center = (xx + 0.5) * scale;
        const double ss = 1.0 / filterscale;
        int xmin = (int)(center - support + 0.5);
        if (xmin < 0) xmin = 0;
        int xmax = (int)(center + support + 0.5);
        if (xmax > in_size) xmax = in_size;
        xmax -= xmin;
        double ww = 0.0;
        for (int x = 0; x < xmax; ++x) {
            const double arg = (x + xmin - center + 0.5) * ss;
            k[x] = filter == PIL_BILINEAR ? pil_bilinear(arg) : pil_bicubic(arg);
            ww += k[x];
        }
        for (int x = 0; x < xmax; ++x) {
            double v = ww != 0.0 ? k[x] / ww : k[x];
            kk[(size_t)xx * ksize + x] = v < 0 ? (int)(-0.5 + v * (1 << 22)) : (int)(0.5 + v * (1 << 22));
        }
        bounds[xx * 2] = xmin;
        bounds[xx * 2 + 1] = xmax;
    }
    return ksize;
}

int yuv_validate(int n, int h, int w, const pa_yuv_desc* d, size_t* span, std::string& err) {
    if (!d) FAIL("pa_yuv420_to_bgr: descriptor is NULL");
    if (w < 2 || h < 2 || (w & 1) || (h & 1)) FAIL("pa_yuv420_to_bgr: %d x %d frames: 4:2:0 needs an even width and height of at least 2", w, h);
    if (n < 1 || n > 65535) FAIL("pa_yuv420_to_bgr: n = %d frames outside [1, 65535]", n);
    if (d->layout != PA_YUV_NV12 && d->layout != PA_YUV_I420) FAIL("pa_yuv420_to_bgr: unknown layout %d", d->layout);
    const bool nv12 = d->layout == PA_YUV_NV12;
    const int crow = nv12 ? w : w / 2;
    if (d->pitch_y < w) FAIL("pa_yuv420_to_bgr: pitch_y %d is smaller than a luma row of %d bytes", d->pitch_y, w);
    if (d->pitch_c < crow) FAIL("pa_yuv420_to_bgr: pitch_c %d is smaller than a chroma row of %d bytes", d->pitch_c, crow);
    if (d->off_u < 0 || d->off_v < 0) FAIL("pa_yuv420_to_bgr: negative plane offset (off_u %d, off_v %d)", d->off_u, d->off_v);
    if (nv12 && d->off_v != d->off_u + 1) FAIL("pa_yuv420_to_bgr: NV12 needs off_v == off_u + 1 (off_u %d, off_v %d)", d->off_u, d->off_v);
    const long long y_end = (long long)(h - 1) * d->pitch_y + w;
    const long long c_len = (long long)(h / 2 - 1) * d->pitch_c + crow;
    const long long extent = std::max(y_end, std::max(d->off_u + c_len, nv12 ? 0ll : d->off_v + c_len));
    if (extent > 0x7fffffffll) FAIL("pa_yuv420_to_bgr: a frame of %lld bytes is beyond 2 GiB", extent);
    if (d->frame_stride < extent)
        FAIL("pa_yuv420_to_bgr: frame_stride %lld is smaller than the %lld bytes the planes of one frame span (they would overlap the next frame)",
                (long long)d->frame_stride, extent);
    const auto mag = [](int32_t c) { return (long long)(c < 0 ? -(long long)c : c); };
    const long long worst = 255 * mag(d->cy) + (1 << 19) + 128 * std::max(mag(d->cvr), std::max(mag(d->cug) + mag(d->cvg), mag(d->cub)));
    if (d->y_off < 0 || d->y_off > 255 || worst > 0x7fffffffll) FAIL("pa_yuv420_to_bgr: coefficients leave int32 (worst case %lld) or y_off %d outside [0, 255]", worst, d->y_off);
    *span = (size_t)(n - 1) * (size_t)d->frame_stride + (size_t)extent;
    return 0;
}

}
```

### padel_analytics_amd/csrc/graph_plan.h

```cpp
#pragma once
#include "../../include/padel_hip.h"

#include <cstddef>
#include <cstdint>
#include <string>
#include <vector>

namespace padel {

inline bool is_head_buf(const pa_model_desc& d, int b) { return b == d.head_buf[0] || b == d.head_buf[1] || b == d.head_buf[2]; }

int validate_desc(const pa_model_desc* d, size_t n_floats, std::string& err);
void find_upsample_folds(const pa_model_desc& d, std::vector<int>& fold_src, std::vector<int>& fold_dst);
bool stem_fusable(const pa_model_desc& d, size_t i);

struct BufferPlan {
    std::vector<size_t> off, bytes;
    size_t arena_bytes = 0, logical_bytes = 0;
};
int plan_activations(const pa_model_desc& d, const std::vector<int>& fold_src, int net_h, int net_w, int batch, bool alias,
                     BufferPlan& out, std::string& err);

struct YoloGeometry {
    int rw = 0, rh = 0, top = 0, left = 0, net_h = 0, net_w = 0, lb_mode = 0;
    struct { int H, W, stride, anchor0; } lv[3]{};
    int A = 0, P2 = 0;
};
int yolo_geometry(int h0, int w0, int imgsz, int pre_mode, int letterbox_auto, YoloGeometry& g, std::string& err);

void cv2_linear_table(int src, int dst, std::vector<int32_t>& tab);
enum { PIL_BICUBIC = 0, PIL_BILINEAR = 1 };
int pil_coeffs(int in_size, int out_size, std::vector<int32_t>& bounds, std::vector<int32_t>& kk, int filter = PIL_BICUBIC);

int yuv_validate(int n, int h, int w, const pa_yuv_desc* d, size_t* span, std::string& err);

}
```

### padel_analytics_amd/csrc/kernels.h

```cpp
#pragma once
#include <hip/hip_runtime.h>
#include <stdint.h>

namespace padel {

enum Act : int { ACT_NONE = 0, ACT_SILU = 1, ACT_RELU = 2, ACT_SIGMOID = 3, ACT_LEAKY = 4 };

struct ConvArgs {
    const float* in;
    const float* w;
    const void* w3;
    const float* bias;
    const float* res;
    int res_pre;
    const float* zeros;
    const float* in2;
    int in2_cs, in2_choff, up_c;
    float* out;
    int in_cs, in_choff;
    int out_cs, out_choff;
    int res_cs, res_choff;
    int H, W;
    int Ho, Wo;
    int cin;
    int cout;
    int n16;
    int ksize, stride;
    int act;
    int M;
    int n_mtiles;
    int n_ntiles;
    int tune;
    int tap_pd;
    int out_f32;
    const float* oscale;
    unsigned* ovf_flag;
    int w_single;
    const void* wr;
    unsigned long long* dbg;
    unsigned howo_magic, howo_shift, wo_magic, wo_shift;
};
inline void fill_fastdiv(unsigned d, unsigned* magic, unsigned* shift) {
    unsigned s = 0;
    while ((1ull << s) < d) ++s;
    *magic = (unsigned)((((1ull << 32) * ((1ull << s) - d)) / d) + 1ull);
    *shift = s;
}
constexpr int conv_dbg_words(int steps) { return 8 + 4 * steps * 5; }
constexpr int kConvDbgSteps = 64;
constexpr int kConvDbgWords = conv_dbg_words(kConvDbgSteps);
constexpr int kPatchDbgSteps = 32;
constexpr int kPatchDbgWords = conv_dbg_words(kPatchDbgSteps);

enum ConvPath : int { CONV_PATH_TAP = 0, CONV_PATH_BX3 = 1, CONV_PATH_H2 = 2, CONV_PATH_F16 = 3 };
bool conv_tile_shape(int path, int id, int* bm, int* bn);
struct ConvLaunched { int tile; const char* family; };
enum ConvFamily : int { CONV_TAP, CONV_BX3T, CONV_BX3P, CONV_H2T, CONV_H2D, CONV_H2S, CONV_H2S3, CONV_H2P, CONV_H2Q, CONV_H2R, CONV_H2W, CONV_H2V,
                        CONV_TAP16, CONV_TAP16D, CONV_P16, CONV_P16Q };
const char* conv_family_name(ConvFamily f);
bool resolve_conv(int path, const ConvArgs& a, int requested, ConvLaunched* out, ConvFamily* family = nullptr);
int conv_timeline_words(const ConvLaunched& k, int ksize);
hipError_t launch_conv(int path, const ConvArgs& a, int variant, hipStream_t s, ConvLaunched* ran = nullptr);
constexpr size_t kConvReadSlack = 512;
int choose_conv_tap_variant(int M, int n16);
int choose_conv_bx3_variant(const ConvArgs& a);
int choose_conv_h2_variant(const ConvArgs& a);
int choose_conv_tap16_variant(const ConvArgs& a);
bool conv_wants_operand_copy(int ksize, int stride, int cin, bool w_single);
int h2_ksteps(int cin, int ksize);
size_t conv_h2r_copy_bytes(int n16, int cin, int ksize);

hipError_t launch_conv_tapt(const ConvArgs& a, int tile, hipStream_t s);
hipError_t launch_conv_bx3t(const ConvArgs& a, int tile, hipStream_t s);
hipError_t launch_conv_bx3p(const ConvArgs& a, int tile, hipStream_t s);
hipError_t launch_conv_h2t(const ConvArgs& a, int tile, hipStream_t s);
hipError_t launch_conv_h2d(const ConvArgs& a, int tile, hipStream_t s);
hipError_t launch_conv_h2s(const ConvArgs& a, int tile, hipStream_t s);
hipError_t launch_conv_h2s3(const ConvArgs& a, int tile, hipStream_t s);
hipError_t launch_conv_h2p(const ConvArgs& a, int tile, hipStream_t s);
hipError_t launch_conv_h2q(const ConvArgs& a, int tile, hipStream_t s);
hipError_t launch_conv_h2r(const ConvArgs& a, int tile, hipStream_t s);
hipError_t launch_conv_h2w(const ConvArgs& a, int tile, hipStream_t s);
hipError_t launch_conv_h2v(const ConvArgs& a, int tile, hipStream_t s);
hipError_t launch_conv_t16(const ConvArgs& a, int tile, hipStream_t s);
hipError_t launch_conv_p16(const ConvArgs& a, int tile, hipStream_t s);
hipError_t launch_h2r_repack(const float* w, void* wr, int n16, int cin, int ksize, hipStream_t s);
hipError_t launch_h2_mplane_check(const float* w, long long rows_x_ksteps, unsigned* flag, hipStream_t s);

struct StemArgs {
    const uint8_t* in;
    const float* w;
    const float* bias;
    float* out;
    int out_cs, out_choff;
    int H, W, Ho, Wo, cout, B;
    int out_f16;
    unsigned* ovf_flag;
    unsigned howo_magic, howo_shift, wo_magic, wo_shift;
    const void* opw;
};
hipError_t launch_stem(const StemArgs& a, hipStream_t s);
struct ConvArgs;
bool stem_l1_h2_supported(const StemArgs& st, const ConvArgs& cv);
hipError_t launch_stem_l1_h2(const StemArgs& st, const ConvArgs& cv, hipStream_t s);
size_t stem_l1_operand_bytes(int cout);
hipError_t launch_stem_l1_operands(const float* w, int cout, void* blk, hipStream_t s);

hipError_t init_misc_kernels();
hipError_t launch_sppf_pool(float* buf, int cs, int choff, int c, int B, int H, int W, hipStream_t s, int f16 = 0, int fused = 1);
hipError_t launch_upsample2x(const float* in, int in_cs, int in_choff, float* out, int out_cs, int out_choff,
                             int c, int B, int H, int W, hipStream_t s, int f16 = 0);
hipError_t launch_h2_encode(const float* in, float* out, long long n_floats, unsigned* ovf_flag, hipStream_t s);
hipError_t launch_maxpool2(const float* in, int in_cs, int in_choff, float* out, int out_cs, int out_choff,
                           int c, int B, int H, int W, hipStream_t s, int f16 = 0);

struct Stem7Args {
    const uint8_t* in;
    const float* w;
    const float* bias;
    const float* lut;
    float* out;
    int out_cs, out_choff;
    int H, W, Ho, Wo, B;
    int act;
    int out_h2;
    unsigned* ovf_flag;
    unsigned howo_magic, howo_shift, wo_magic, wo_shift;
};
hipError_t launch_stem7(const Stem7Args& a, hipStream_t s);
hipError_t launch_maxpool3s2(const float* in, int in_cs, int in_choff, float* out, int out_cs, int out_choff,
                             int c, int B, int H, int W, int Ho, int Wo, hipStream_t s, int h2);
hipError_t launch_gap_fc(const float* in, int in_cs, int in_choff, int c, int B, int HW, const float* w, const float* bias, int nout,
                         float* logits, float* probs, hipStream_t s, int h2);
constexpr int kGapFcMaxC = 4096, kGapFcMaxOut = 64;

struct DwConvArgs {
    const float* in;
    const float* w;
    const float* bias;
    const float* res;
    float* out;
    int in_cs, in_choff, out_cs, out_choff, res_cs, res_choff;
    int C, B, H, W;
    int act;
    int h2, out_f32;
    unsigned* ovf_flag;
};
hipError_t launch_dwconv3(const DwConvArgs& a, hipStream_t s);
struct AttnArgs {
    const float* qkv;
    float* out;
    int cs, q_choff, k_choff, v_choff, out_cs, out_choff;
    int heads, kd, hd, N, B;
    float scale;
    int h2, out_f32;
    unsigned* ovf_flag;
};
hipError_t launch_psa_attn(const AttnArgs& a, hipStream_t s);

struct LetterboxArgs {
    const uint8_t* src;
    uint8_t* dst;
    int B, h0, w0;
    int rw, rh;
    int top, left;
    int nh, nw;
    int mode;
    int reverse;
    const int32_t* xtab;
    const int32_t* ytab;
};
hipError_t launch_letterbox(const LetterboxArgs& a, hipStream_t s);

struct YuvArgs {
    const uint8_t* src;
    uint8_t* dst;
    int n, h, w;
    int nv12;
    int pitch_y, pitch_c;
    int off_u, off_v;
    long long frame_stride;
    int y_off, cy, cvr, cug, cvg, cub;
};
bool yuv_vector_path_ok(const YuvArgs& a);
hipError_t launch_yuv420_to_bgr(const YuvArgs& a, hipStream_t s, int* vec_out = nullptr);

struct RenderArgs {
    const uint8_t* src;
    uint8_t* dst;
    const void* marks;
    const void* boxes;
    const int32_t* first;
    int n, h, w;
    int out;
    int in_place;
    int pitch_y, pitch_c, off_u, off_v;
    long long frame_stride;
    int y_off, yr, yg, yb, ur, ug, ub, vr, vg, vb;
#ifdef PADEL_RENDER_PROBE
    unsigned long long* probe;
#endif
};
bool render_vector_path_ok(const RenderArgs& a);
hipError_t launch_render(const RenderArgs& a, hipStream_t s, int* vec_out = nullptr);

struct ResamplePassArgs {
    const uint8_t* in; uint8_t* out;
    int B, in_h, in_w, in_c;
    int out_h, out_w, out_c;
    int vertical;
    const int32_t* bounds;
    const int32_t* coefs;
    int ksize;
    int reverse;
};
hipError_t launch_resample_pass(const ResamplePassArgs& a, hipStream_t s);

struct HeadLevel { const float* buf; int H, W, stride, anchor0; };
struct DecodeArgs {
    HeadLevel lv[3];
    int cs;
    int nc, nk, kdim;
    int A, B;
    float conf;
    const int32_t* classes; int n_classes;
    float* cand;
    int32_t* cand_idx;
    int32_t* cand_cnt;
};
hipError_t launch_decode(const DecodeArgs& a, hipStream_t s);

struct NmsArgs {
    const float* cand; const int32_t* cand_idx; const int32_t* cand_cnt;
    uint64_t* keys;
    int32_t* order;
    uint8_t* supp;
    HeadLevel lv[3];
    int cs, nc, nk, kdim, A, B, P2;
    float iou; int max_det; int max_nms;
    float gain; float pad_x, pad_y;
    float kpad_x, kpad_y;
    float w0, h0;
    float* out_boxes;
    float* out_kpts;
    int32_t* out_cnt;
};
hipError_t launch_nms(const NmsArgs& a, hipStream_t s);

struct BallAssembleArgs {
    const uint8_t* median;
    const uint8_t* frames;
    const float* lut;
    float* out;
    int B, H, W, ring, first_slot;
    int out_f16;
};
hipError_t launch_ball_assemble(const BallAssembleArgs& a, hipStream_t s);

struct BallEnsembleArgs {
    const float* Y;
    int cs, H, W;
    const int32_t* row0;
    const int32_t* mode;
    const float* div;
    float w[8];
    float threshold;
    float* heat;
    uint8_t* mask;
};
hipError_t launch_ball_ensemble(const BallEnsembleArgs& a, int nout, hipStream_t s);

struct BallLocateArgs {
    const uint8_t* mask;
    int32_t* label;
    int32_t* bbox;
    int32_t* rect;
    int H, W;
};
hipError_t launch_ball_locate(const BallLocateArgs& a, int nout, hipStream_t s);
hipError_t launch_median(const uint8_t* frames, int N, long long frame_bytes, uint8_t* out_rgb, hipStream_t s);

}
```

### padel_analytics_amd/csrc/postproc.hip

```cpp
#include "kernels.h"

namespace padel {

__device__ __forceinline__ float sigmoidf_(float x) { return 1.0f / (1.0f + expf(-x)); }

__global__ void __launch_bounds__(256) decode_kernel(const DecodeArgs a) {
    const int b = blockIdx.y;
    const int ai = blockIdx.x * 256 + threadIdx.x;
    bool pass = ai < a.A;
    int l = 0;
    if (pass) { if (ai >= a.lv[2].anchor0) l = 2; else if (ai >= a.lv[1].anchor0) l = 1; }
    const HeadLevel lv = a.lv[l];
    const int pix = pass ? ai - lv.anchor0 : 0;
    const float* h = lv.buf + ((long long)b * lv.H * lv.W + pix) * a.cs;

    const float* cl = h + 64;
    float score = 0.0f;
    int cls = 0;
    if (pass) {
        float mx = cl[0];
        for (int c = 1; c < a.nc; ++c) mx = fmaxf(mx, cl[c]);
        score = sigmoidf_(mx);
        pass = score > a.conf;
    }
    if (pass) {
        for (int c = 0; c < a.nc; ++c) {
            if (sigmoidf_(cl[c]) == score) { cls = c; break; }
        }
        if (a.n_classes > 0) {
            bool ok = false;
            for (int k = 0; k < a.n_classes; ++k) ok |= (a.classes[k] == cls);
            pass = ok;
        }
    }
    float bx[4] = {0.f, 0.f, 0.f, 0.f};
    if (pass) {
        float d[4];
#pragma unroll
        for (int s = 0; s < 4; ++s) {
            float v[16];
            float m = h[s * 16];
#pragma unroll
            for (int i = 0; i < 16; ++i) { v[i] = h[s * 16 + i]; m = fmaxf(m, v[i]); }
            float sum = 0.0f;
#pragma unroll
            for (int i = 0; i < 16; ++i) { v[i] = expf(v[i] - m); sum += v[i]; }
            float e = 0.0f;
#pragma unroll
            for (int i = 0; i < 16; ++i) e += (v[i] / sum) * (float)i;
            d[s] = e;
        }
        const float ax = (float)(pix % lv.W) + 0.5f, ay = (float)(pix / lv.W) + 0.5f;
        const float st = (float)lv.stride;
        const float x1 = ax - d[0], y1 = ay - d[1], x2 = ax + d[2], y2 = ay + d[3];
        const float cx = ((x1 + x2) / 2.0f) * st, cy = ((y1 + y2) / 2.0f) * st;
        const float w = (x2 - x1) * st, hh = (y2 - y1) * st;
        const float hw = w / 2.0f, hhh = hh / 2.0f;
        bx[0] = cx - hw; bx[1] = cy - hhh; bx[2] = cx + hw; bx[3] = cy + hhh;
    }
    const unsigned long long m = __builtin_amdgcn_ballot_w64(pass);
    if (m == 0ull) return;
    const int lane = threadIdx.x & 63;
    int base = 0;
    if (lane == 0) base = atomicAdd(&a.cand_cnt[b], __builtin_popcountll(m));
    base = __builtin_amdgcn_readfirstlane(base);
    if (!pass) return;
    const int slot = base + __builtin_popcountll(m & ((1ull << lane) - 1ull));
    float* o = a.cand + ((long long)b * a.A + slot) * 6;
    o[0] = bx[0]; o[1] = bx[1]; o[2] = bx[2]; o[3] = bx[3]; o[4] = score; o[5] = (float)cls;
    a.cand_idx[(long long)b * a.A + slot] = ai;
}

__global__ void zero_i32_kernel(int32_t* p, int n) {
    const int i = blockIdx.x * 256 + threadIdx.x;
    if (i < n) p[i] = 0;
}

hipError_t launch_decode(const DecodeArgs& a, hipStream_t s) {
    hipLaunchKernelGGL(zero_i32_kernel, dim3((a.B + 255) / 256), dim3(256), 0, s, a.cand_cnt, a.B);
    hipError_t e = hipGetLastError();
    if (e != hipSuccess) return e;
    dim3 grid((a.A + 255) / 256, a.B, 1);
    hipLaunchKernelGGL(decode_kernel, grid, dim3(256), 0, s, a);
    return hipGetLastError();
}

#define NMS_THREADS 1024
#define NMS_WAVES (NMS_THREADS / 64)
#define NMS_LDS_KEYS 16384
#define NMS_CHUNK 4096

__device__ __forceinline__ bool nms_over(const float4 bi, const float iarea, const float4 bj, const float jarea, const float iou) {
    const float xx1 = fmaxf(bi.x, bj.x), yy1 = fmaxf(bi.y, bj.y);
    const float xx2 = fminf(bi.z, bj.z), yy2 = fminf(bi.w, bj.w);
    const float ww = fmaxf(0.0f, xx2 - xx1), hh = fmaxf(0.0f, yy2 - yy1);
    const float inter = ww * hh;
    if (!(inter > 0.0f)) return false;
    const float uni = iarea + jarea - inter;
    const float t = iou * uni;
    if (inter > t * 1.000001f) return true;
    if (inter < t * 0.999999f) return false;
    return inter / uni > iou;
}

__global__ void __launch_bounds__(NMS_THREADS) nms_kernel(const NmsArgs a) {
    __shared__ uint64_t skeys[NMS_LDS_KEYS];
    float4* const sbox = reinterpret_cast<float4*>(skeys);
    float* const sarea = reinterpret_cast<float*>(skeys + NMS_CHUNK * 2);
    int* const sord = reinterpret_cast<int*>(skeys + NMS_CHUNK * 2 + NMS_CHUNK / 2);
    static_assert(NMS_CHUNK * (16 + 4 + 4) <= NMS_LDS_KEYS * 8, "chunk staging fits the sort buffer");
    __shared__ int skeep[300];
    __shared__ float4 kbox[300];
    __shared__ float karea[300];
    __shared__ unsigned long long smask[64];
    __shared__ unsigned long long s_sup;
    __shared__ int s_kept, s_done;
    const int b = blockIdx.x;
    const int tid = threadIdx.x;
    const int lane = tid & 63, wave = tid >> 6;
    int n = a.cand_cnt[b];
    if (n > a.A) n = a.A;
    const float* cand = a.cand + (long long)b * a.A * 6;
    const int32_t* cidx = a.cand_idx + (long long)b * a.A;
    int32_t* order = a.order + (long long)b * a.A;

    int p2 = 1;
    while (p2 < n) p2 <<= 1;
    uint64_t* keys = (p2 <= NMS_LDS_KEYS) ? skeys : (a.keys + (long long)b * a.P2);

    for (int i = tid; i < p2; i += NMS_THREADS) {
        uint64_t k = ~0ull;
        if (i < n) {
            const uint32_t sb = __float_as_uint(cand[i * 6 + 4]);
            k = ((uint64_t)(~sb) << 32) | ((uint64_t)(uint32_t)cidx[i] << 16) | (uint32_t)i;
        }
        keys[i] = k;
    }
    __syncthreads();
    for (int k = 2; k <= p2; k <<= 1) {
        for (int j = k >> 1; j > 0; j >>= 1) {
            for (int i = tid; i < p2; i += NMS_THREADS) {
                const int ixj = i ^ j;
                if (ixj > i) {
                    const uint64_t x = keys[i], y = keys[ixj];
                    const bool up = (i & k) == 0;
                    if ((x > y) == up) { keys[i] = y; keys[ixj] = x; }
                }
            }
            __syncthreads();
        }
    }
    int ne = n < a.max_nms ? n : a.max_nms;
    for (int i = tid; i < ne; i += NMS_THREADS) order[i] = (int)(keys[i] & 0xffffu);
    if (tid == 0) { s_kept = 0; s_done = 0; s_sup = 0ull; }
    __syncthreads();

    for (int c0 = 0; c0 < ne && !s_done; c0 += NMS_CHUNK) {
        const int nc = min(NMS_CHUNK, ne - c0);
        __syncthreads();
        for (int i = tid; i < nc; i += NMS_THREADS) {
            const int slot = order[c0 + i];
            sord[i] = slot;
            const float* bi = cand + slot * 6;
            const float off = bi[5] * 7680.0f;
            const float4 bx = make_float4(bi[0] + off, bi[1] + off, bi[2] + off, bi[3] + off);
            sbox[i] = bx;
            sarea[i] = (bx.z - bx.x) * (bx.w - bx.y);
        }
        __syncthreads();
        for (int w0 = 0; w0 < nc; w0 += 64) {
            const int j = w0 + lane;
            const bool valid = j < nc;
            const float4 bj = sbox[valid ? j : w0];
            const float ja = sarea[valid ? j : w0];
            const unsigned long long vmask = __ballot(valid);
            const int K = s_kept;
            bool sup = false;
            for (int k = wave; k < K; k += NMS_WAVES) {
                sup = sup || nms_over(kbox[k], karea[k], bj, ja, a.iou);
                if ((__ballot(sup) & vmask) == vmask) break;
            }
            const unsigned long long sw = __ballot(sup);
            if (lane == 0 && sw) atomicOr(&s_sup, sw);
#pragma unroll
            for (int r = 0; r < 64 / NMS_WAVES; ++r) {
                const int il = wave * (64 / NMS_WAVES) + r, i = w0 + il;
                unsigned long long bits = 0ull;
                if (i < nc) bits = __ballot(valid && lane > il && nms_over(sbox[i], sarea[i], bj, ja, a.iou));
                if (lane == 0) smask[il] = bits;
            }
            __syncthreads();
            if (wave == 0) {
                unsigned long long rem = s_sup | ~vmask;
                int k = K;
                bool done = false;
                unsigned long long cur = ~rem;
                while (cur) {
                    const int il = __builtin_ctzll(cur);
                    if (lane == 0) { skeep[k] = sord[w0 + il]; kbox[k] = sbox[w0 + il]; karea[k] = sarea[w0 + il]; }
                    ++k;
                    if (k >= a.max_det) { done = true; break; }
                    rem |= smask[il];
                    cur = il == 63 ? 0ull : (~rem & (~0ull << (il + 1)));
                }
                if (lane == 0) { s_kept = k; s_done = done ? 1 : 0; s_sup = 0ull; }
            }
            __syncthreads();
            if (s_done) break;
        }
    }
    const int kept = s_kept;
    __syncthreads();
    if (tid == 0) a.out_cnt[b] = kept;

    const int nkv = a.nk;
    for (int k = kept * 6 + tid; k < a.max_det * 6; k += NMS_THREADS) a.out_boxes[(long long)b * a.max_det * 6 + k] = 0.0f;
    if (nkv > 0 && a.out_kpts)
        for (int k = kept * nkv + tid; k < a.max_det * nkv; k += NMS_THREADS) a.out_kpts[(long long)b * a.max_det * nkv + k] = 0.0f;
    for (int k = tid; k < kept; k += NMS_THREADS) {
        const int slot = skeep[k];
        const float* c = cand + slot * 6;
        float* o = a.out_boxes + ((long long)b * a.max_det + k) * 6;
        float x1 = (c[0] - a.pad_x) / a.gain, y1 = (c[1] - a.pad_y) / a.gain;
        float x2 = (c[2] - a.pad_x) / a.gain, y2 = (c[3] - a.pad_y) / a.gain;
        o[0] = fminf(fmaxf(x1, 0.0f), a.w0); o[1] = fminf(fmaxf(y1, 0.0f), a.h0);
        o[2] = fminf(fmaxf(x2, 0.0f), a.w0); o[3] = fminf(fmaxf(y2, 0.0f), a.h0);
        o[4] = c[4]; o[5] = c[5];
        if (nkv > 0 && a.out_kpts) {
            const int ai = cidx[slot];
            int l = 0;
            if (ai >= a.lv[2].anchor0) l = 2; else if (ai >= a.lv[1].anchor0) l = 1;
            const HeadLevel lv = a.lv[l];
            const int pix = ai - lv.anchor0;
            const float* h = lv.buf + ((long long)b * lv.H * lv.W + pix) * a.cs + 64 + a.nc;
            const float ax = (float)(pix % lv.W) + 0.5f, ay = (float)(pix / lv.W) + 0.5f;
            const float st = (float)lv.stride;
            float* ko = a.out_kpts + ((long long)b * a.max_det + k) * nkv;
            const int K = nkv / a.kdim;
            for (int q = 0; q < K; ++q) {
                float kx = (h[q * a.kdim] * 2.0f + (ax - 0.5f)) * st;
                float ky = (h[q * a.kdim + 1] * 2.0f + (ay - 0.5f)) * st;
                kx = (kx - a.kpad_x) / a.gain;
                ky = (ky - a.kpad_y) / a.gain;
                ko[q * a.kdim] = fminf(fmaxf(kx, 0.0f), a.w0);
                ko[q * a.kdim + 1] = fminf(fmaxf(ky, 0.0f), a.h0);
                if (a.kdim == 3) ko[q * a.kdim + 2] = sigmoidf_(h[q * a.kdim + 2]);
            }
        }
    }
}

hipError_t launch_nms(const NmsArgs& a, hipStream_t s) {
    hipLaunchKernelGGL(nms_kernel, dim3(a.B), dim3(NMS_THREADS), 0, s, a);
    return hipGetLastError();
}

}
```

### padel_analytics_amd/engine.py

```python
from __future__ import annotations

import ctypes as C
import sys as _sys
import os
from pathlib import Path
from typing import Optional, Sequence

import numpy as np

from . import graph as G

_LIB_PATH = Path(os.environ["PADEL_LIB"]).resolve() if os.environ.get("PADEL_LIB") else Path(__file__).resolve().parent / "libpadel_hip.so"
_lib = None


class EngineUnavailable(RuntimeError):
    pass


class EngineError(RuntimeError):
    pass


class RangeOverflow(EngineError):
    """An activation of an h2 model (fp16 pairs, |x| <= 65504) did not fit: the results of that call are invalid and
    the caller repeats it on the full-range fp32 (bf16x3) model (yolo.py / trackers/ball_tracker.py do)."""


def fp32_mode() -> str:
    m = os.environ.get("PADEL_FP32_MODE", "h2").lower()
    if m not in ("h2", "bx3"):
        raise ValueError(f"PADEL_FP32_MODE={m!r}: expected 'h2' or 'bx3'")
    return m


class pa_buf_desc(C.Structure):
    _fields_ = [("level", C.c_int32), ("channels", C.c_int32)]


class pa_op_desc(C.Structure):
    _fields_ = [("kind", C.c_int32), ("in_buf", C.c_int32), ("in_choff", C.c_int32), ("cin", C.c_int32),
                ("out_buf", C.c_int32), ("out_choff", C.c_int32), ("cout", C.c_int32),
                ("ksize", C.c_int32), ("stride", C.c_int32), ("act", C.c_int32),
                ("res_buf", C.c_int32), ("res_choff", C.c_int32), ("npad", C.c_int32), ("reserved", C.c_int32),
                ("w_off", C.c_int64), ("b_off", C.c_int64), ("flags", C.c_int32), ("pad_", C.c_int32)]


class pa_model_desc(C.Structure):
    _fields_ = [("task", C.c_int32), ("nc", C.c_int32), ("nk", C.c_int32), ("kpt_dim", C.c_int32),
                ("n_bufs", C.c_int32), ("bufs", C.POINTER(pa_buf_desc)),
                ("n_ops", C.c_int32), ("ops", C.POINTER(pa_op_desc)),
                ("head_buf", C.c_int32 * 3), ("in_channels", C.c_int32), ("dtype", C.c_int32)]


class pa_yolo_params(C.Structure):
    _fields_ = [("imgsz", C.c_int32), ("pre_mode", C.c_int32), ("channel_reverse", C.c_int32),
                ("letterbox_auto", C.c_int32), ("conf", C.c_float), ("iou", C.c_float),
                ("max_det", C.c_int32), ("n_classes", C.c_int32), ("classes", C.POINTER(C.c_int32)),
                ("frames_on_device", C.c_int32)]


class pa_yuv_desc(C.Structure):
    _fields_ = [("layout", C.c_int32), ("pitch_y", C.c_int32), ("pitch_c", C.c_int32), ("off_u", C.c_int32),
                ("off_v", C.c_int32), ("reserved", C.c_int32), ("frame_stride", C.c_int64),
                ("y_off", C.c_int32), ("cy", C.c_int32), ("cvr", C.c_int32), ("cug", C.c_int32), ("cvg", C.c_int32),
                ("cub", C.c_int32)]


class pa_mark(C.Structure):
    _fields_ = [("kind", C.c_int32), ("x0", C.c_int32), ("y0", C.c_int32), ("x1", C.c_int32), ("y1", C.c_int32),
                ("size", C.c_int32), ("bgr", C.c_uint32), ("arg", C.c_int32)]


class pa_yuv_enc(C.Structure):
    _fields_ = [("y_off", C.c_int32), ("yr", C.c_int32), ("yg", C.c_int32), ("yb", C.c_int32), ("ur", C.c_int32), ("ug", C.c_int32),
                ("ub", C.c_int32), ("vr", C.c_int32), ("vg", C.c_int32), ("vb", C.c_int32)]


MARK_DTYPE = np.dtype([("kind", "<i4"), ("x0", "<i4"), ("y0", "<i4"), ("x1", "<i4"), ("y1", "<i4"), ("size", "<i4"), ("bgr", "<u4"),
                       ("arg", "<i4")])
MARK_DISC, MARK_SEGMENT, MARK_FILL, MARK_BOX, MARK_GLYPH, MARK_BLEND = 1, 2, 3, 4, 5, 6
RENDER_BGR, RENDER_YUV420 = 0, 1
RENDER_PATH_VECTOR, RENDER_PATH_BYTE = 1, 2

PRE_LETTERBOX, PRE_PIL_STRETCH = 0, 1
YUV_NV12, YUV_I420 = 0, 1
YUV_PATH_VECTOR, YUV_PATH_BYTE = 1, 2

ABI_SYMBOLS = [
    "pa_abi_version", "pa_device_count", "pa_engine_create", "pa_engine_destroy", "pa_last_error",
    "pa_engine_synchronize", "pa_device_malloc", "pa_device_free", "pa_memcpy_h2d", "pa_memcpy_d2h",
    "pa_model_create", "pa_model_destroy", "pa_model_set_max_batch", "pa_yolo_infer", "pa_yolo_head_shape",
    "pa_yolo_read_head", "pa_tracknet_infer", "pa_engine_set_profiling", "pa_model_last_profile",
    "pa_model_profile_text", "pa_ball_create", "pa_ball_destroy", "pa_ball_set_background", "pa_ball_feed",
    "pa_ball_locate", "pa_ball_background_from_frames",
    "pa_upload", "pa_engine_set_tuning", "pa_engine_set_timeline_path", "pa_model_plan_bytes",
    "pa_yolo_netin_shape", "pa_yolo_read_netin",
    "pa_comm_unique_id", "pa_engine_comm_init", "pa_engine_comm_destroy", "pa_engine_bcast_weights",
    "pa_engine_bcast", "pa_engine_allreduce_max", "pa_engine_gather_sizes", "pa_engine_gather",
    "pa_bytetrack_create", "pa_bytetrack_destroy", "pa_bytetrack_reset", "pa_bytetrack_update_batch",
    "pa_model_take_overflow", "pa_yolo_postprocess", "pa_host_register", "pa_host_unregister",
    "pa_engine_bcast_weights_from", "pa_model_fill_arena", "pa_yolo_submit", "pa_yolo_wait",
    "pa_resnet_infer", "pa_resnet_read_netin", "pa_resnet_read_fc", "pa_resnet_read_head", "pa_pil_coeffs",
    "pa_yuv420_to_bgr", "pa_yuv_last_path", "pa_engine_timer_start", "pa_engine_timer_stop",
    "pa_render", "pa_render_check", "pa_render_last_path", "pa_glyph_rows", "pa_ball_read_resized",
    "pa_jpeg_encode", "pa_jpeg_check", "pa_jpeg_interval_bytes",
    "pa_jpeg_parse", "pa_jpeg_decode", "pa_jpeg_decode_last_path", "pa_jpeg_decode_last_times",
]


def lib_path() -> Path:
    return _LIB_PATH


def load_library():
    global _lib
    if _lib is not None:
        return _lib
    if not _LIB_PATH.exists():
        raise EngineUnavailable(f"{_LIB_PATH} not built — run `python -c 'import __graft_entry__ as g; g.build()'`")
    if os.environ.get("PADEL_HIP_STANDALONE") != "1":
        import torch
    lib = C.CDLL(str(_LIB_PATH))
    vp, i32, sz = C.c_void_p, C.c_int, C.c_size_t
    lib.pa_abi_version.restype = i32
    lib.pa_device_count.restype = i32
    lib.pa_engine_create.argtypes = [i32, C.POINTER(vp)]
    lib.pa_engine_destroy.argtypes = [vp]
    lib.pa_engine_destroy.restype = None
    lib.pa_last_error.argtypes = [vp]
    lib.pa_last_error.restype = C.c_char_p
    lib.pa_engine_synchronize.argtypes = [vp]
    lib.pa_device_malloc.argtypes = [vp, sz, C.POINTER(vp)]
    lib.pa_device_free.argtypes = [vp, vp]
    lib.pa_memcpy_h2d.argtypes = [vp, vp, vp, sz]
    lib.pa_memcpy_d2h.argtypes = [vp, vp, vp, sz]
    lib.pa_model_create.argtypes = [vp, C.POINTER(pa_model_desc), vp, sz, C.POINTER(vp)]
    lib.pa_model_destroy.argtypes = [vp]
    lib.pa_model_destroy.restype = None
    lib.pa_model_set_max_batch.argtypes = [vp, i32]
    lib.pa_yolo_infer.argtypes = [vp, vp, i32, i32, i32, C.POINTER(pa_yolo_params), vp, vp, vp]
    lib.pa_yolo_submit.argtypes = [vp, vp, i32, i32, i32, C.POINTER(pa_yolo_params), vp, vp, vp, C.POINTER(C.c_int)]
    lib.pa_yolo_wait.argtypes = [vp, i32, C.POINTER(C.c_int)]
    lib.pa_yolo_head_shape.argtypes = [vp, i32, C.POINTER(i32), C.POINTER(i32), C.POINTER(i32)]
    lib.pa_yolo_read_head.argtypes = [vp, i32, i32, vp]
    lib.pa_tracknet_infer.argtypes = [vp, vp, i32, i32, i32, i32, vp, i32]
    lib.pa_resnet_infer.argtypes = [vp, vp, i32, i32, i32, i32, vp, vp]
    lib.pa_resnet_read_netin.argtypes = [vp, i32, vp]
    lib.pa_resnet_read_fc.argtypes = [vp, i32, vp, vp]
    lib.pa_resnet_read_head.argtypes = [vp, i32, vp]
    lib.pa_pil_coeffs.argtypes = [i32, i32, i32, vp, vp, i32, C.POINTER(i32)]
    lib.pa_engine_set_profiling.argtypes = [vp, i32]
    lib.pa_model_last_profile.argtypes = [vp, i32, vp, vp, vp, vp]
    lib.pa_model_profile_text.argtypes = [vp, C.c_char_p, sz]
    lib.pa_ball_create.argtypes = [vp, i32, i32, C.POINTER(vp)]
    lib.pa_ball_destroy.argtypes = [vp]
    lib.pa_ball_destroy.restype = None
    lib.pa_ball_set_background.argtypes = [vp, vp]
    lib.pa_ball_feed.argtypes = [vp, vp, i32, i32, i32, vp, vp, vp, C.POINTER(i32)]
    lib.pa_ball_locate.argtypes = [vp, vp, i32, vp]
    lib.pa_ball_background_from_frames.argtypes = [vp, vp, i32, i32, vp]
    lib.pa_ball_read_resized.argtypes = [vp, C.c_longlong, vp]
    lib.pa_upload.argtypes = [vp, vp, vp, sz]
    lib.pa_engine_set_tuning.argtypes = [vp, C.c_char_p, i32]
    lib.pa_engine_set_timeline_path.argtypes = [vp, C.c_char_p]
    lib.pa_model_plan_bytes.argtypes = [vp, C.POINTER(sz), C.POINTER(sz)]
    lib.pa_yolo_netin_shape.argtypes = [vp, C.POINTER(i32), C.POINTER(i32)]
    lib.pa_yolo_read_netin.argtypes = [vp, i32, vp]
    lib.pa_comm_unique_id.argtypes = [vp, sz]
    lib.pa_engine_comm_init.argtypes = [vp, vp, sz, i32, i32]
    lib.pa_engine_comm_destroy.argtypes = [vp]
    lib.pa_engine_comm_destroy.restype = None
    lib.pa_engine_bcast_weights.argtypes = [vp, vp, i32]
    lib.pa_engine_bcast.argtypes = [vp, vp, sz, i32]
    lib.pa_engine_bcast_weights_from.argtypes = [vp, vp, vp, i32]
    lib.pa_engine_allreduce_max.argtypes = [vp, C.POINTER(C.c_double)]
    lib.pa_engine_gather_sizes.argtypes = [vp, sz, C.POINTER(C.c_uint64)]
    lib.pa_engine_gather.argtypes = [vp, vp, sz, vp, sz, C.POINTER(C.c_uint64), i32]
    lib.pa_bytetrack_create.argtypes = [C.c_double, i32, C.c_double, i32, C.POINTER(vp)]
    lib.pa_bytetrack_destroy.argtypes = [vp]
    lib.pa_bytetrack_destroy.restype = None
    lib.pa_bytetrack_reset.argtypes = [vp]
    lib.pa_bytetrack_reset.restype = None
    lib.pa_bytetrack_update_batch.argtypes = [vp, vp, vp, vp, i32, i32, vp]
    lib.pa_model_fill_arena.argtypes = [vp, i32]
    lib.pa_host_register.argtypes = [vp, vp, sz]
    lib.pa_host_unregister.argtypes = [vp, vp]
    lib.pa_model_take_overflow.argtypes = [vp, C.POINTER(i32)]
    lib.pa_yolo_postprocess.argtypes = [vp, C.POINTER(vp), i32, i32, i32, C.POINTER(pa_yolo_params), vp, vp, vp]
    lib.pa_yuv420_to_bgr.argtypes = [vp, vp, i32, i32, i32, i32, C.POINTER(pa_yuv_desc), vp]
    lib.pa_yuv_last_path.argtypes = [vp]
    lib.pa_render.argtypes = [vp, vp, i32, i32, i32, vp, vp, i32, C.POINTER(pa_yuv_desc), C.POINTER(pa_yuv_enc), vp]
    lib.pa_render_check.argtypes = [i32, i32, i32, vp, vp, i32, C.POINTER(pa_yuv_desc), C.POINTER(pa_yuv_enc), C.c_char_p, sz]
    lib.pa_render_last_path.argtypes = [vp]
    lib.pa_glyph_rows.argtypes = [i32, vp]
    lib.pa_jpeg_encode.argtypes = [vp, vp, i32, i32, i32, C.POINTER(pa_yuv_desc), i32, vp, sz, vp]
    lib.pa_jpeg_check.argtypes = [i32, i32, i32, C.POINTER(pa_yuv_desc), i32, C.c_char_p, sz]
    lib.pa_jpeg_interval_bytes.argtypes = [i32]
    lib.pa_jpeg_interval_bytes.restype = sz
    lib.pa_jpeg_parse.argtypes = [vp, sz, C.POINTER(pa_jpeg_frame_info), vp, sz, C.c_char_p, sz]
    lib.pa_jpeg_decode.argtypes = [vp, vp, vp, i32, i32, i32, vp, vp]
    lib.pa_jpeg_decode_last_path.argtypes = [vp]
    lib.pa_jpeg_decode_last_times.argtypes = [vp, vp]
    lib.pa_engine_timer_start.argtypes = [vp]
    lib.pa_engine_timer_stop.argtypes = [vp, C.POINTER(C.c_float)]
    if lib.pa_abi_version() != 5:
        raise EngineUnavailable("libpadel_hip.so ABI version mismatch")
    _lib = lib
    return lib


PIL_BICUBIC, PIL_BILINEAR = 0, 1


def pil_coeffs(in_size: int, out_size: int, filter: int = PIL_BICUBIC):
    lib = load_library()
    ks = C.c_int(0)
    if lib.pa_pil_coeffs(in_size, out_size, filter, None, None, 0, C.byref(ks)) != 0:
        raise EngineError("pa_pil_coeffs: bad arguments")
    bounds = np.zeros((out_size, 2), np.int32)
    coefs = np.zeros((out_size, ks.value), np.int32)
    if lib.pa_pil_coeffs(in_size, out_size, filter, bounds.ctypes.data, coefs.ctypes.data, coefs.size, C.byref(ks)) != 0:
        raise EngineError("pa_pil_coeffs failed")
    return bounds, coefs


def graph_dtype(mode: Optional[str] = None) -> str:
    return {"h2": "h2", "bx3": "f32"}[mode or fp32_mode()]


def yuv_span_bytes(n: int, h: int, w: int, d: "pa_yuv_desc") -> Optional[int]:
    if n < 1 or h < 2 or w < 2 or h % 2 or w % 2 or d.layout not in (YUV_NV12, YUV_I420):
        return None
    crow = w if d.layout == YUV_NV12 else w // 2
    if d.pitch_y < w or d.pitch_c < crow or d.off_u < 0 or d.off_v < 0:
        return None
    c_len = (h // 2 - 1) * d.pitch_c + crow
    extent = max((h - 1) * d.pitch_y + w, d.off_u + c_len, 0 if d.layout == YUV_NV12 else d.off_v + c_len)
    if d.frame_stride < extent:
        return None
    return (n - 1) * d.frame_stride + extent


def glyph_rows(code) -> Optional[np.ndarray]:
    rows = np.zeros(7, np.uint8)
    code = ord(code) if isinstance(code, str) else int(code)
    return rows if load_library().pa_glyph_rows(code, rows.ctypes.data) == 0 else None


def _render_args(marks, first, geom, enc):
    marks = np.ascontiguousarray(marks, MARK_DTYPE).reshape(-1)
    first = np.ascontiguousarray(first, np.int32).reshape(-1)
    if geom is not None and not isinstance(geom, pa_yuv_desc):
        geom = pa_yuv_desc(**{k: int(v) for k, v in geom.items()})
    if enc is not None and not isinstance(enc, pa_yuv_enc):
        enc = pa_yuv_enc(*(int(c) for c in enc))
    return marks, first, geom, enc


def render_check(n: int, h: int, w: int, marks, first, out: int = RENDER_BGR, geom=None, enc=None) -> Optional[str]:
    marks, first, geom, enc = _render_args(marks, first, geom, enc)
    if first.size != max(int(n), 0) + 1:
        return f"pa_render: first has {first.size} entries, n + 1 = {int(n) + 1} are needed"
    if marks.size < int(first[-1]):
        return f"pa_render: first[] announces {int(first[-1])} marks, marks holds {marks.size}"
    why = C.create_string_buffer(512)
    rc = load_library().pa_render_check(int(n), int(h), int(w), marks.ctypes.data if marks.size else None, first.ctypes.data, int(out),
                                        C.byref(geom) if geom is not None else None, C.byref(enc) if enc is not None else None, why, 512)
    return why.value.decode() if rc else None


JPEG_MAX_WIDTH = 2560


def _yuv_desc_arg(desc):
    return desc if desc is None or isinstance(desc, pa_yuv_desc) else pa_yuv_desc(**{k: int(v) for k, v in desc.items()})


def jpeg_check(n: int, h: int, w: int, desc, quality: int = 90) -> Optional[str]:
    desc = _yuv_desc_arg(desc)
    why = C.create_string_buffer(512)
    rc = load_library().pa_jpeg_check(int(n), int(h), int(w), C.byref(desc) if desc is not None else None, int(quality), why, 512)
    return why.value.decode() if rc else None


def jpeg_interval_bytes(w: int) -> int:
    return int(load_library().pa_jpeg_interval_bytes(int(w)))


JPEG_DEC_MAX_DIM = 4096
JPEG_DEC_PATH_VECTOR, JPEG_DEC_PATH_BYTE = 1, 2


class pa_jpeg_huff(C.Structure):
    _fields_ = [("bits", C.c_uint8 * 16), ("vals", C.c_uint8 * 256), ("nvals", C.c_int32)]


class pa_jpeg_interval(C.Structure):
    _fields_ = [("begin", C.c_int64), ("end", C.c_int64), ("first_mcu", C.c_int32), ("mcus", C.c_int32)]


class pa_jpeg_frame_info(C.Structure):
    _fields_ = [("w", C.c_int32), ("h", C.c_int32), ("mcus_x", C.c_int32), ("mcus_y", C.c_int32), ("restart_interval", C.c_int32),
                ("n_intervals", C.c_int32), ("default_huffman", C.c_int32), ("status", C.c_int32), ("scan_begin", C.c_int64),
                ("scan_end", C.c_int64), ("quant", (C.c_uint8 * 64) * 3), ("comp_dc", C.c_uint8 * 3), ("comp_ac", C.c_uint8 * 3),
                ("pad_", C.c_uint8 * 2), ("dc", pa_jpeg_huff * 2), ("ac", pa_jpeg_huff * 2)]


def jpeg_parse(jpeg) -> dict:
    raw = np.frombuffer(bytes(jpeg), np.uint8)
    info, why = pa_jpeg_frame_info(), C.create_string_buffer(512)
    lib = load_library()
    if lib.pa_jpeg_parse(raw.ctypes.data, raw.size, C.byref(info), None, 0, why, 512):
        raise ValueError(why.value.decode())
    ivls = (pa_jpeg_interval * max(info.n_intervals, 1))()
    if lib.pa_jpeg_parse(raw.ctypes.data, raw.size, C.byref(info), ivls, info.n_intervals, why, 512):
        raise ValueError(why.value.decode())
    table = lambda t: (list(t.bits), list(t.vals)[:t.nvals])
    return dict(w=info.w, h=info.h, mcus_x=info.mcus_x, mcus_y=info.mcus_y, restart_interval=info.restart_interval,
                n_intervals=info.n_intervals, default_huffman=info.default_huffman, status=info.status, scan_begin=info.scan_begin,
                scan_end=info.scan_end, quant=np.array([list(q) for q in info.quant], np.uint8), comp_dc=list(info.comp_dc),
                comp_ac=list(info.comp_ac), dc=[table(t) for t in info.dc], ac=[table(t) for t in info.ac],
                intervals=[(v.begin, v.end, v.first_mcu, v.mcus) for v in ivls[:info.n_intervals]])


class DeviceBuffer:

    def __init__(self, engine: "Engine", nbytes: int, _ptr: Optional[int] = None):
        self.engine, self.nbytes = engine, nbytes
        self.owner = _ptr is None
        if _ptr is None:
            p = C.c_void_p()
            engine._check(engine.lib.pa_device_malloc(engine.handle, nbytes, C.byref(p)))
            _ptr = p.value
        self.ptr = _ptr

    def view(self, offset: int, nbytes: int) -> "DeviceBuffer":
        assert 0 <= offset and offset + nbytes <= self.nbytes
        return DeviceBuffer(self.engine, nbytes, _ptr=self.ptr + offset)

    def upload(self, arr: np.ndarray, copy_stream: bool = False) -> "DeviceBuffer":
        arr = np.ascontiguousarray(arr)
        assert arr.nbytes <= self.nbytes
        f = self.engine.lib.pa_upload if copy_stream else self.engine.lib.pa_memcpy_h2d
        self.engine._check(f(self.engine.handle, self.ptr, arr.ctypes.data, arr.nbytes))
        return self

    def download(self, arr: np.ndarray) -> np.ndarray:
        assert arr.flags.c_contiguous and arr.nbytes <= self.nbytes
        self.engine._check(self.engine.lib.pa_memcpy_d2h(self.engine.handle, arr.ctypes.data, self.ptr, arr.nbytes))
        return arr

    def free(self):
        if self.ptr and self.owner:
            self.engine.lib.pa_device_free(self.engine.handle, self.ptr)
        self.ptr = None


class Engine:

    def __init__(self, device_id: int = 0):
        self.lib = load_library()
        if self.lib.pa_device_count() <= 0:
            raise EngineUnavailable("no HIP device visible: the padel_analytics_amd engine needs an AMD GPU (gfx950)")
        h = C.c_void_p()
        if self.lib.pa_engine_create(device_id, C.byref(h)) != 0:
            raise EngineUnavailable(self.lib.pa_last_error(None).decode())
        self.handle = h
        self.device_id = device_id

    def _check(self, rc: int):
        if rc != 0:
            raise EngineError(self.lib.pa_last_error(self.handle).decode())

    def synchronize(self):
        self._check(self.lib.pa_engine_synchronize(self.handle))

    def set_profiling(self, on: bool):
        self._check(self.lib.pa_engine_set_profiling(self.handle, 1 if on else 0))
        self.profiling = bool(on)

    def alloc(self, nbytes: int) -> DeviceBuffer:
        return DeviceBuffer(self, nbytes)

    def pin(self, arr: np.ndarray) -> None:
        assert arr.flags.c_contiguous
        self._check(self.lib.pa_host_register(self.handle, arr.ctypes.data, arr.nbytes))

    def unpin(self, arr: np.ndarray) -> None:
        self._check(self.lib.pa_host_unregister(self.handle, arr.ctypes.data))

    def yuv420_to_bgr(self, src, n: int, h: int, w: int, desc, dst: DeviceBuffer) -> None:
        if not isinstance(desc, pa_yuv_desc):
            desc = pa_yuv_desc(**{k: int(v) for k, v in desc.items()})
        on_dev = isinstance(src, DeviceBuffer)
        if on_dev:
            ptr, have = src.ptr, src.nbytes
        else:
            if not (isinstance(src, np.ndarray) and src.dtype == np.uint8 and src.ndim == 1 and src.flags.c_contiguous):
                raise TypeError("yuv420_to_bgr: src must be a contiguous 1-D uint8 array of raw bytes or a DeviceBuffer")
            ptr, have = src.ctypes.data, src.nbytes
        need = yuv_span_bytes(n, h, w, desc)
        if need is not None and have < need:
            raise EngineError(f"yuv420_to_bgr: {n} frames as described span {need} bytes, src holds {have}")
        if n >= 1 and h >= 1 and w >= 1 and dst.nbytes < n * h * w * 3:
            raise EngineError(f"yuv420_to_bgr: dst holds {dst.nbytes} bytes, {n} BGR frames need {n * h * w * 3}")
        self._check(self.lib.pa_yuv420_to_bgr(self.handle, ptr, int(on_dev), int(n), int(h), int(w), C.byref(desc), dst.ptr))

    def yuv_last_path(self) -> int:
        return int(self.lib.pa_yuv_last_path(self.handle))

    def render(self, src: DeviceBuffer, n: int, h: int, w: int, marks, first, dst: DeviceBuffer, out: int = RENDER_BGR, geom=None,
               enc=None) -> None:
        marks, first, geom, enc = _render_args(marks, first, geom, enc)
        if first.size != max(int(n), 0) + 1:
            raise EngineError(f"render: first has {first.size} entries, n + 1 = {int(n) + 1} are needed")
        if marks.size < int(first[-1]):
            raise EngineError(f"render: first[] announces {int(first[-1])} marks, marks holds {marks.size}")
        if n >= 1 and h >= 1 and w >= 1 and src.nbytes < n * h * w * 3:
            raise EngineError(f"render: src holds {src.nbytes} bytes, {n} BGR frames need {n * h * w * 3}")
        if out == RENDER_YUV420 and geom is not None:
            need = yuv_span_bytes(n, h, w, geom)
        else:
            need = n * h * w * 3 if (n >= 1 and h >= 1 and w >= 1) else None
        if need is not None and dst.nbytes < need:
            raise EngineError(f"render: {n} frames as described span {need} bytes, dst holds {dst.nbytes}")
        self._check(self.lib.pa_render(self.handle, src.ptr, int(n), int(h), int(w), marks.ctypes.data if marks.size else None,
                                       first.ctypes.data, int(out), C.byref(geom) if geom is not None else None,
                                       C.byref(enc) if enc is not None else None, dst.ptr))

    def render_last_path(self) -> int:
        return int(self.lib.pa_render_last_path(self.handle))

    def jpeg_encode(self, buffer: DeviceBuffer, n: int, h: int, w: int, desc, quality: int = 90, out: Optional[np.ndarray] = None):
        desc = _yuv_desc_arg(desc)
        need = yuv_span_bytes(n, h, w, desc)
        if need is not None and buffer.nbytes < need:
            raise EngineError(f"jpeg_encode: {n} frames as described span {need} bytes, the buffer holds {buffer.nbytes}")
        offsets = np.zeros(max(int(n), 0) + 1, np.int64)
        own = out is None
        if own:
            out = np.empty(max(int(n), 1) * (max(int(h), 1) * max(int(w), 1) // 4 + 4096), np.uint8)
        elif not (isinstance(out, np.ndarray) and out.dtype == np.uint8 and out.ndim == 1 and out.flags.c_contiguous):
            raise TypeError("jpeg_encode: out must be a contiguous 1-D uint8 array")
        for attempt in (0, 1):
            rc = self.lib.pa_jpeg_encode(self.handle, buffer.ptr, int(n), int(h), int(w), C.byref(desc), int(quality), out.ctypes.data,
                                         out.size, offsets.ctypes.data)
            if rc == 0:
                return out[:int(offsets[-1])], offsets
            needed = int(offsets[-1])
            if needed <= out.size or not own or attempt:
                err = EngineError(self.lib.pa_last_error(self.handle).decode())
                err.needed = needed if needed > out.size else None
                raise err
            out = np.empty(needed, np.uint8)

    def jpeg_decode(self, data, offsets, dst: DeviceBuffer, h: Optional[int] = None, w: Optional[int] = None) -> np.ndarray:
        data = np.frombuffer(data, np.uint8) if isinstance(data, (bytes, bytearray)) else data
        if not (isinstance(data, np.ndarray) and data.dtype == np.uint8 and data.ndim == 1 and data.flags.c_contiguous):
            raise TypeError("jpeg_decode: data must be bytes or a contiguous 1-D uint8 array")
        offsets = np.ascontiguousarray(offsets, np.int64)
        n = offsets.size - 1
        if n < 1 or offsets[0] < 0 or np.any(np.diff(offsets) < 0) or offsets[-1] > data.size:
            raise EngineError(f"jpeg_decode: offsets must be n + 1 >= 2 ascending positions inside the {data.size} bytes of data")
        if h is None or w is None:
            try:
                info = jpeg_parse(data[int(offsets[0]):int(offsets[1])].tobytes())
            except ValueError as e:
                raise EngineError(f"jpeg_decode: frame 0: {e}") from None
            h, w = info["h"], info["w"]
        h, w = int(h), int(w)
        if dst.nbytes < n * h * w * 3:
            raise EngineError(f"jpeg_decode: dst holds {dst.nbytes} bytes, {n} BGR frames of {w} x {h} need {n * h * w * 3}")
        status = np.zeros(n, np.int32)
        self._check(self.lib.pa_jpeg_decode(self.handle, data.ctypes.data, offsets.ctypes.data, n, h, w, dst.ptr, status.ctypes.data))
        return status

    def jpeg_decode_last_path(self) -> int:
        return int(self.lib.pa_jpeg_decode_last_path(self.handle))

    def jpeg_decode_last_times(self) -> dict:
        ms = (C.c_double * 5)()
        self._check(self.lib.pa_jpeg_decode_last_times(self.handle, ms))
        return dict(zip(("parse", "upload", "entropy", "idct", "colour"), (float(v) for v in ms)))

    def timer_start(self) -> None:
        self._check(self.lib.pa_engine_timer_start(self.handle))

    def timer_stop(self) -> float:
        ms = C.c_float(0.0)
        self._check(self.lib.pa_engine_timer_stop(self.handle, C.byref(ms)))
        return float(ms.value)

    def set_tuning(self, **kv):
        for k, v in kv.items():
            self._check(self.lib.pa_engine_set_tuning(self.handle, k.encode(), int(v)))
            if k == "timeline":
                self.timeline = bool(v)

    def comm_init(self, unique_id: bytes, nranks: int, rank: int):
        buf = C.create_string_buffer(bytes(unique_id), len(unique_id))
        self._check(self.lib.pa_engine_comm_init(self.handle, buf, len(unique_id), nranks, rank))
        self.nranks, self.rank = nranks, rank
        if nranks > 1:
            from . import dist as _dist
            _dist.use_engine_comm(self)

    def bcast_weights(self, model: "Model", root: int = 0):
        self._check(self.lib.pa_engine_bcast_weights(self.handle, model.handle, root))

    def bcast_weights_from(self, src: Optional["Model"], dst: "Model", root: int = 0):
        self._check(self.lib.pa_engine_bcast_weights_from(self.handle, src.handle if src is not None else None, dst.handle, root))

    def bcast(self, buf: DeviceBuffer, nbytes: int, root: int = 0):
        self._check(self.lib.pa_engine_bcast(self.handle, buf.ptr, nbytes, root))

    def gather_bytes(self, buf: np.ndarray, root: int = 0):
        buf = np.ascontiguousarray(buf, np.uint8).reshape(-1)
        n = max(getattr(self, "nranks", 1), 1)
        me = getattr(self, "rank", 0)
        sizes = (C.c_uint64 * n)()
        self._check(self.lib.pa_engine_gather_sizes(self.handle, int(buf.size), sizes))
        total = int(sum(sizes))
        recv = np.empty(max(total, 1), np.uint8) if me == root else None
        self._check(self.lib.pa_engine_gather(self.handle, buf.ctypes.data if buf.size else None, int(buf.size),
                                              recv.ctypes.data if recv is not None else None, total if recv is not None else 0, sizes, root))
        if me != root:
            return None
        out, off = [], 0
        for k in range(n):
            out.append(recv[off:off + int(sizes[k])])
            off += int(sizes[k])
        return out

    def allreduce_max(self, value: float) -> float:
        v = C.c_double(value)
        self._check(self.lib.pa_engine_allreduce_max(self.handle, C.byref(v)))
        return v.value

    def close(self):
        if self.handle:
            from . import dist as _dist
            if _dist._comm_engine is self:
                _dist.use_engine_comm(None)
            self.lib.pa_engine_destroy(self.handle)
            self.handle = None


_default_engines: dict = {}


def comm_unique_id() -> bytes:
    lib = load_library()
    buf = C.create_string_buffer(128)
    if lib.pa_comm_unique_id(buf, 128) != 0:
        raise EngineError(lib.pa_last_error(None).decode())
    return buf.raw


def default_engine(device_id: Optional[int] = None) -> Engine:
    if device_id is None:
        device_id = int(os.environ.get("LOCAL_RANK", "0")) if os.environ.get("PADEL_DEVICE") is None \
            else int(os.environ["PADEL_DEVICE"])
        load_library()
        n = _lib.pa_device_count()
        if n > 0:
            device_id %= n
    if device_id not in _default_engines:
        _default_engines[device_id] = Engine(device_id)
    return _default_engines[device_id]


_PAGE = 4096


def _round_up(x: int, a: int) -> int:
    return (int(x) + a - 1) // a * a


def _frames_arg(frames, n: Optional[int], h: int, w: int):
    if isinstance(frames, DeviceBuffer):
        assert n is not None and frames.nbytes >= n * h * w * 3
        return frames, frames.ptr, n, True
    frames = np.ascontiguousarray(frames, np.uint8)
    n = len(frames) if n is None else n
    assert frames.shape == (n, h, w, 3), frames.shape
    return frames, frames.ctypes.data, n, False


def _yolo_params(classes: Optional[Sequence[int]], **fields):
    cls_arr = (C.c_int32 * len(classes))(*[int(c) for c in classes]) if classes is not None and len(classes) else None
    return pa_yolo_params(n_classes=0 if cls_arr is None else len(cls_arr), classes=cls_arr, **fields), cls_arr


class _PinnedBlock:

    def __init__(self, engine, nbytes: int):
        import mmap
        size = _round_up(max(int(nbytes), 1), _PAGE)
        self._mm = mmap.mmap(-1, size, flags=mmap.MAP_PRIVATE | mmap.MAP_ANONYMOUS, prot=mmap.PROT_READ | mmap.PROT_WRITE)
        self.block = np.frombuffer(self._mm, np.uint8)
        self.engine = engine
        engine.pin(self.block)
        self._pinned = True

    def release(self) -> None:
        if self._pinned:
            self._pinned = False
            try:
                self.engine.unpin(self.block)
            except Exception as exc:
                if _sys is not None and getattr(_sys, "meta_path", None) is not None and getattr(self.engine, "handle", None):
                    print(f"padel_analytics_amd: hipHostUnregister of a result block failed ({exc}); pages left registered", file=_sys.stderr)

    def __del__(self):
        self.release()


class Model:

    def __init__(self, engine: Engine, graph: G.Graph, blob: Optional[np.ndarray] = None, *, empty: bool = False):
        self.engine, self.graph = engine, graph
        if not empty:
            blob = graph.blob() if blob is None else np.ascontiguousarray(blob, np.float32)
        bufs = (pa_buf_desc * len(graph.bufs))(*[pa_buf_desc(l, c) for l, c in graph.bufs])
        ops = (pa_op_desc * len(graph.ops))()
        for i, o in enumerate(graph.ops):
            for k, v in o.items():
                setattr(ops[i], k, int(v))
        d = pa_model_desc(task=graph.task, nc=graph.nc, nk=graph.nk, kpt_dim=graph.kpt_dim, n_bufs=len(graph.bufs),
                          bufs=bufs, n_ops=len(graph.ops), ops=ops, in_channels=graph.in_channels,
                          dtype=graph.dtype)
        for i in range(3):
            d.head_buf[i] = graph.head_buf[i] if i < len(graph.head_buf) else -1
        h = C.c_void_p()
        engine._check(engine.lib.pa_model_create(engine.handle, C.byref(d), None if empty else blob.ctypes.data,
                                                 graph.n_floats if empty else blob.size, C.byref(h)))
        self.handle = h
        self.max_batch = 64
        self._out_ring: dict = {}

    MAX_INFLIGHT = 4
    OUT_RING = MAX_INFLIGHT + 2

    def _ring_outputs(self, n: int, max_det: int):
        key = (int(n), int(max_det))
        ring = self._out_ring.get(key)
        if ring is None:
            nk = self.graph.nk
            sizes = [n * max_det * 6 * 4, n * max_det * nk * 4, n * 4]
            offs = [0, _round_up(sizes[0], 64), 0]
            offs[2] = offs[1] + _round_up(sizes[1], 64)
            sets = []
            for _ in range(self.OUT_RING):
                pb = _PinnedBlock(self.engine, offs[2] + sizes[2])
                block = pb.block
                boxes = block[offs[0]:offs[0] + sizes[0]].view(np.float32).reshape(n, max_det, 6)
                kpts = block[offs[1]:offs[1] + sizes[1]].view(np.float32).reshape(n, max_det, nk) if nk else None
                counts = block[offs[2]:offs[2] + sizes[2]].view(np.int32).reshape(n)
                sets.append((boxes, kpts, counts, pb))
            ring = self._out_ring[key] = [sets, 0]
        sets, i = ring
        ring[1] = (i + 1) % self.OUT_RING
        return sets[i][:3]

    def _fresh_outputs(self, n: int, max_det: int):
        nk = self.graph.nk
        return (np.zeros((n, max_det, 6), np.float32), np.zeros((n, max_det, nk), np.float32) if nk else None,
                np.zeros((n,), np.int32))

    def _free_rings(self):
        for sets, _ in self._out_ring.values():
            for arrs in sets:
                arrs[3].release()
        self._out_ring = {}

    def __del__(self):
        try:
            if self._out_ring and getattr(self, "handle", None) and self.engine.handle:
                self.engine.synchronize()
        except Exception:
            pass
        try:
            self._free_rings()
        except Exception:
            pass

    def set_max_batch(self, n: int):
        self.engine._check(self.engine.lib.pa_model_set_max_batch(self.handle, int(n)))
        self.max_batch = int(n)

    def yolo_infer(self, frames, n: int, h: int, w: int, *, imgsz: int, conf: float, iou: float,
                   classes: Optional[Sequence[int]] = None, max_det: int = 300, pre_mode: int = PRE_LETTERBOX,
                   channel_reverse: bool = False, letterbox_auto: bool = True, reuse_outputs: bool = False):
        frames, ptr, n, on_dev = _frames_arg(frames, n, h, w)
        p, cls_arr = _yolo_params(classes, imgsz=imgsz, pre_mode=pre_mode, channel_reverse=int(channel_reverse),
                                  letterbox_auto=int(letterbox_auto), conf=conf, iou=iou, max_det=max_det,
                                  frames_on_device=int(on_dev))
        boxes, kpts, counts = self._ring_outputs(n, max_det) if reuse_outputs else self._fresh_outputs(n, max_det)
        self.engine._check(self.engine.lib.pa_yolo_infer(
            self.handle, ptr, n, h, w, C.byref(p), boxes.ctypes.data,
            kpts.ctypes.data if kpts is not None else None, counts.ctypes.data))
        return boxes, kpts, counts

    def yolo_submit(self, frames: "DeviceBuffer", n: int, h: int, w: int, *, imgsz: int, conf: float, iou: float,
                    classes: Optional[Sequence[int]] = None, max_det: int = 300, pre_mode: int = PRE_LETTERBOX,
                    channel_reverse: bool = False, letterbox_auto: bool = True):
        assert isinstance(frames, DeviceBuffer) and frames.nbytes >= n * h * w * 3
        p, cls_arr = _yolo_params(classes, imgsz=imgsz, pre_mode=pre_mode, channel_reverse=int(channel_reverse),
                                  letterbox_auto=int(letterbox_auto), conf=conf, iou=iou, max_det=max_det, frames_on_device=1)
        boxes, kpts, counts = self._ring_outputs(n, max_det)
        t = C.c_int(-1)
        self.engine._check(self.engine.lib.pa_yolo_submit(
            self.handle, frames.ptr, n, h, w, C.byref(p), boxes.ctypes.data,
            kpts.ctypes.data if kpts is not None else None, counts.ctypes.data, C.byref(t)))
        return (t.value, boxes, kpts, counts)

    def yolo_wait(self, ticket):
        t, boxes, kpts, counts = ticket
        ovf = C.c_int(0)
        self.engine._check(self.engine.lib.pa_yolo_wait(self.handle, t, C.byref(ovf)))
        return boxes, kpts, counts, bool(ovf.value)

    def head_shapes(self, h: int, w: int, imgsz: int, pre_mode: int = PRE_LETTERBOX, letterbox_auto: bool = True) -> list:
        if pre_mode == PRE_PIL_STRETCH or not letterbox_auto:
            nh = nw = imgsz
        else:
            r = min(imgsz / h, imgsz / w)
            rw, rh = int(round(w * r)), int(round(h * r))
            nw, nh = rw + (imgsz - rw) % 32, rh + (imgsz - rh) % 32
        c = self.graph.bufs[self.graph.head_buf[0]][1]
        return [(nh >> (3 + l), nw >> (3 + l), c) for l in range(3)]

    def yolo_postprocess(self, heads, h: int, w: int, *, imgsz: int, conf: float, iou: float,
                         classes: Optional[Sequence[int]] = None, max_det: int = 300, pre_mode: int = PRE_LETTERBOX):
        heads = [np.ascontiguousarray(x, np.float32) for x in heads]
        n = heads[0].shape[0]
        assert [x.shape[1:] for x in heads] == [tuple(s) for s in self.head_shapes(h, w, imgsz, pre_mode)], [x.shape for x in heads]
        p, cls_arr = _yolo_params(classes, imgsz=imgsz, pre_mode=pre_mode, channel_reverse=0, letterbox_auto=1, conf=conf, iou=iou,
                                  max_det=max_det, frames_on_device=0)
        ptrs = (C.c_void_p * 3)(*[x.ctypes.data for x in heads])
        boxes, kpts, counts = self._fresh_outputs(n, max_det)
        self.engine._check(self.engine.lib.pa_yolo_postprocess(self.handle, ptrs, n, h, w, C.byref(p), boxes.ctypes.data,
                                                               kpts.ctypes.data if kpts is not None else None, counts.ctypes.data))
        return boxes, kpts, counts

    def fill_arena(self, byte_value: int = 0xFF) -> None:
        self.engine._check(self.engine.lib.pa_model_fill_arena(self.handle, int(byte_value)))

    def take_overflow(self) -> bool:
        v = C.c_int(0)
        self.engine._check(self.engine.lib.pa_model_take_overflow(self.handle, C.byref(v)))
        return bool(v.value)

    def read_head(self, level: int, n: int) -> np.ndarray:
        hh, ww, cc = C.c_int(), C.c_int(), C.c_int()
        self.engine._check(self.engine.lib.pa_yolo_head_shape(self.handle, level, C.byref(hh), C.byref(ww), C.byref(cc)))
        out = np.empty((n, hh.value, ww.value, cc.value), np.float32)
        self.engine._check(self.engine.lib.pa_yolo_read_head(self.handle, level, n, out.ctypes.data))
        return out

    def read_netin(self, n: int) -> np.ndarray:
        hh, ww = C.c_int(), C.c_int()
        self.engine._check(self.engine.lib.pa_yolo_netin_shape(self.handle, C.byref(hh), C.byref(ww)))
        out = np.empty((n, hh.value, ww.value, 4), np.uint8)
        self.engine._check(self.engine.lib.pa_yolo_read_netin(self.handle, n, out.ctypes.data))
        return out

    def plan_bytes(self) -> tuple:
        a, l = C.c_size_t(), C.c_size_t()
        self.engine._check(self.engine.lib.pa_model_plan_bytes(self.handle, C.byref(a), C.byref(l)))
        return a.value, l.value

    def tracknet_infer(self, x: np.ndarray) -> np.ndarray:
        x = np.ascontiguousarray(x, np.float16 if self.graph.dtype == G.DTYPE_F16 else np.float32)
        n, h, w, c = x.shape
        assert c == self.graph.bufs[0][1], (c, self.graph.bufs[0])
        lvl, cout = self.graph.bufs[self.graph.head_buf[0]]
        out = np.empty((n, h >> lvl, w >> lvl, cout), np.float32)
        self.engine._check(self.engine.lib.pa_tracknet_infer(self.handle, x.ctypes.data, n, h, w, 0, out.ctypes.data, 0))
        return out

    def resnet_infer(self, frames, n: int, h: int, w: int, *, want_logits: bool = False):
        frames, ptr, n, on_dev = _frames_arg(frames, n, h, w)
        c = next((o["cout"] for o in self.graph.ops if o["kind"] == G.OP_GAP_FC), 0)
        xy = np.zeros((n, c), np.float32) if c else None
        logits = np.zeros((n, c), np.float32) if (c and want_logits) else None
        self.engine._check(self.engine.lib.pa_resnet_infer(self.handle, ptr, n, h, w, int(on_dev),
                                                           xy.ctypes.data if c else None,
                                                           logits.ctypes.data if logits is not None else None))
        return xy, logits

    def resnet_read_netin(self, n: int) -> np.ndarray:
        out = np.empty((n, G.RESNET_INPUT, G.RESNET_INPUT, 4), np.uint8)
        self.engine._check(self.engine.lib.pa_resnet_read_netin(self.handle, n, out.ctypes.data))
        return out

    def read_fc(self, n: int):
        c = next(o["cout"] for o in self.graph.ops if o["kind"] == G.OP_GAP_FC)
        xy, logits = np.empty((n, c), np.float32), np.empty((n, c), np.float32)
        self.engine._check(self.engine.lib.pa_resnet_read_fc(self.handle, n, xy.ctypes.data, logits.ctypes.data))
        return xy, logits

    def resnet_read_head(self, n: int) -> np.ndarray:
        lvl, ch = self.graph.bufs[self.graph.head_buf[0]]
        out = np.empty((n, G.RESNET_INPUT >> lvl, G.RESNET_INPUT >> lvl, ch), np.float32)
        self.engine._check(self.engine.lib.pa_resnet_read_head(self.handle, n, out.ctypes.data))
        return out

    def last_profile(self, cap: int = 4096):
        kinds = np.zeros(cap, np.int32)
        ms = np.zeros(cap, np.float32)
        fl = np.zeros(cap, np.float64)
        ks = np.zeros(cap, np.int32)
        n = self.engine.lib.pa_model_last_profile(self.handle, cap, kinds.ctypes.data, ms.ctypes.data, fl.ctypes.data,
                                                  ks.ctypes.data)
        return [dict(kind=int(kinds[i]), ms=float(ms[i]), flops=float(fl[i]), ksize=int(ks[i])) for i in range(n)]

    def profile_rows(self):
        buf = C.create_string_buffer(1 << 20)
        self.engine.lib.pa_model_profile_text(self.handle, buf, len(buf))
        return parse_profile_text(buf.value.decode())

    def close(self):
        if self.handle:
            self.engine.lib.pa_model_destroy(self.handle)
            self.handle = None
            self._free_rings()


PROF_PRE, PROF_DECODE, PROF_NMS = 100, 101, 102


def parse_profile_text(text: str):
    rows = []
    for line in text.splitlines():
        f = line.split(",")
        k, ks, M, co, ci, st, mf, nf, ms, fl, res = (f + ["0"])[:11]
        rows.append(dict(kind=int(k), ksize=int(ks), M=int(M), cout=int(co), cin=int(ci), stride=int(st),
                         mf=int(mf), nf=int(nf), ms=float(ms), flops=float(fl), res=int(res),
                         tile=int(f[11]) if len(f) > 11 and f[11] else -1, family=f[12] if len(f) > 12 else ""))
    return rows


class NativeByteTrack:

    def __init__(self, track_activation_threshold: float = 0.25, lost_track_buffer: int = 30,
                 minimum_matching_threshold: float = 0.8, frame_rate: int = 30):
        self.lib = load_library()
        h = C.c_void_p()
        if self.lib.pa_bytetrack_create(track_activation_threshold, lost_track_buffer, minimum_matching_threshold,
                                        int(frame_rate), C.byref(h)) != 0:
            raise EngineError("pa_bytetrack_create failed")
        self.handle = h

    def reset(self) -> None:
        self.lib.pa_bytetrack_reset(self.handle)

    def update_batch(self, boxes: np.ndarray, counts: np.ndarray, keep: Optional[np.ndarray] = None) -> np.ndarray:
        boxes = np.ascontiguousarray(boxes, np.float32)
        counts = np.ascontiguousarray(counts, np.int32)
        n, stride, six = boxes.shape
        assert six == 6 and counts.shape == (n,)
        kp = None
        if keep is not None:
            keep = np.ascontiguousarray(keep, np.uint8)
            assert keep.shape == (n, stride)
            kp = keep.ctypes.data
        ids = np.empty((n, stride), np.int32)
        if self.lib.pa_bytetrack_update_batch(self.handle, boxes.ctypes.data, counts.ctypes.data, kp, n, stride,
                                              ids.ctypes.data) != 0:
            raise EngineError("pa_bytetrack_update_batch failed")
        return ids

    def update_with_detections(self, detections):
        n = len(detections)
        boxes = np.zeros((1, max(n, 1), 6), np.float32)
        boxes[0, :n, :4] = detections.xyxy
        boxes[0, :n, 4] = 1.0 if detections.confidence is None else detections.confidence
        ids = self.update_batch(boxes, np.array([n], np.int32))[0, :n]
        out = detections[np.nonzero(ids >= 0)[0]]
        out.tracker_id = ids[ids >= 0].astype(int)
        return out

    def __del__(self):
        if getattr(self, "handle", None):
            self.lib.pa_bytetrack_destroy(self.handle)
            self.handle = None


class BallSession:

    H, W = 288, 512

    def __init__(self, model: Model, src_h: int, src_w: int):
        self.model, self.src_h, self.src_w = model, src_h, src_w
        h = C.c_void_p()
        model.engine._check(model.engine.lib.pa_ball_create(model.handle, src_h, src_w, C.byref(h)))
        self.handle = h
        self.max_feed = model.max_batch

    def set_background(self, median_rgb: np.ndarray):
        m = np.ascontiguousarray(median_rgb, np.uint8)
        assert m.shape == (self.src_h, self.src_w, 3), m.shape
        self.model.engine._check(self.model.engine.lib.pa_ball_set_background(self.handle, m.ctypes.data))

    def background_from_frames(self, frames_bgr, want_median: bool = False, n: Optional[int] = None):
        on_dev = isinstance(frames_bgr, DeviceBuffer)
        frames_bgr, ptr, n, _ = _frames_arg(frames_bgr, n if on_dev else None, self.src_h, self.src_w)
        med = np.empty((self.src_h, self.src_w, 3), np.uint8) if want_median else None
        self.model.engine._check(self.model.engine.lib.pa_ball_background_from_frames(
            self.handle, ptr, n, int(on_dev), med.ctypes.data if want_median else None))
        return med

    def feed(self, frames_bgr, flush: bool = False, want_heat: bool = False,
             want_rects: bool = False, want_masks: bool = True, n: Optional[int] = None):
        on_dev = isinstance(frames_bgr, DeviceBuffer)
        ptr = None
        if not on_dev:
            n = 0 if frames_bgr is None else len(frames_bgr)
        if on_dev or n:
            frames_bgr, ptr, n, _ = _frames_arg(frames_bgr, n, self.src_h, self.src_w)
            assert 0 < n <= self.max_feed
        masks = np.empty((n + 7, self.H, self.W), np.uint8) if (want_masks or not want_rects) else None
        heat = np.empty((n + 7, self.H, self.W), np.float32) if want_heat else None
        rects = np.empty((n + 7, 4), np.int32) if want_rects else None
        cnt = C.c_int(0)
        self.model.engine._check(self.model.engine.lib.pa_ball_feed(
            self.handle, ptr, n, int(on_dev), int(flush), masks.ctypes.data if masks is not None else None,
            heat.ctypes.data if want_heat else None, rects.ctypes.data if want_rects else None, C.byref(cnt)))
        k = cnt.value
        out = (None if masks is None else masks[:k], heat[:k] if want_heat else None)
        return out + (rects[:k],) if want_rects else out

    def locate(self, masks: np.ndarray) -> np.ndarray:
        masks = np.ascontiguousarray(masks, np.uint8)
        n = len(masks)
        assert masks.shape == (n, self.H, self.W)
        rects = np.empty((n, 4), np.int32)
        self.model.engine._check(self.model.engine.lib.pa_ball_locate(self.handle, masks.ctypes.data, n, rects.ctypes.data))
        return rects

    def read_resized(self, frame: Optional[int] = None) -> np.ndarray:
        out = np.empty((self.H, self.W, 3), np.uint8)
        self.model.engine._check(self.model.engine.lib.pa_ball_read_resized(self.handle, -1 if frame is None else int(frame),
                                                                            out.ctypes.data))
        return out

    def close(self):
        if self.handle:
            self.model.engine.lib.pa_ball_destroy(self.handle)
            self.handle = None
```

Before: 1035.

## Fuse YOLO head tail 1x1 convs with DFL decode into one h2 kernel

Result: faster. 1051, median of 6 (+1.5%).

```diff
diff --git a/include/padel_hip.h b/include/padel_hip.h
--- a/include/padel_hip.h
+++ b/include/padel_hip.h
@@ -199,6 +199,7 @@
 
 int pa_yolo_head_shape(pa_model* m, int level, int* h, int* w, int* c);
 int pa_yolo_read_head(pa_model* m, int level, int n, float* out);
+int pa_yolo_last_post_path(pa_model* m);
 
 int pa_yolo_netin_shape(pa_model* m, int* h, int* w);
 int pa_yolo_read_netin(pa_model* m, int n, uint8_t* out);
diff --git a/padel_analytics_amd/csrc/decode_math.h b/padel_analytics_amd/csrc/decode_math.h
--- /dev/null
+++ b/padel_analytics_amd/csrc/decode_math.h
@@ -0,0 +1,33 @@
+#pragma once
+#include <hip/hip_runtime.h>
+
+namespace padel {
+
+__device__ __forceinline__ float sigmoidf_(float x) { return 1.0f / (1.0f + expf(-x)); }
+
+__device__ __forceinline__ float dfl_expect(float (&v)[16]) {
+#pragma clang fp contract(off)
+    float m = v[0];
+#pragma unroll
+    for (int i = 0; i < 16; ++i) m = fmaxf(m, v[i]);
+    float sum = 0.0f;
+#pragma unroll
+    for (int i = 0; i < 16; ++i) { v[i] = expf(v[i] - m); sum += v[i]; }
+    float e = 0.0f;
+#pragma unroll
+    for (int i = 0; i < 16; ++i) e = fmaf(v[i] / sum, (float)i, e);
+    return e;
+}
+
+__device__ __forceinline__ void dfl_box(const float (&d)[4], int pix, int W, int stride, float (&bx)[4]) {
+#pragma clang fp contract(off)
+    const float ax = (float)(pix % W) + 0.5f, ay = (float)(pix / W) + 0.5f;
+    const float st = (float)stride;
+    const float x1 = ax - d[0], y1 = ay - d[1], x2 = ax + d[2], y2 = ay + d[3];
+    const float mx = (x1 + x2) / 2.0f, my = (y1 + y2) / 2.0f;
+    const float w = (x2 - x1) * st, hh = (y2 - y1) * st;
+    const float hw = w / 2.0f, hhh = hh / 2.0f;
+    bx[0] = fmaf(mx, st, -hw); bx[1] = fmaf(my, st, -hhh); bx[2] = fmaf(mx, st, hw); bx[3] = fmaf(my, st, hhh);
+}
+
+}
diff --git a/padel_analytics_amd/csrc/engine.cpp b/padel_analytics_amd/csrc/engine.cpp
--- a/padel_analytics_amd/csrc/engine.cpp
+++ b/padel_analytics_amd/csrc/engine.cpp
@@ -15,6 +15,7 @@
     {"fold_up", "PADEL_FOLD_UP", &Tuning::fold_up, knob_flag},
     {"fuse_stem", "PADEL_FUSE_STEM", &Tuning::fuse_stem, knob_raw},
     {"fuse_sppf", "PADEL_FUSE_SPPF", &Tuning::fuse_sppf, knob_raw},
+    {"fuse_head", "PADEL_FUSE_HEAD", &Tuning::fuse_head, knob_flag},
     {"w_single", nullptr, &Tuning::w_single, knob_flag},
 };
 
@@ -44,6 +45,7 @@
     if (r == hipSuccess) r = hipMemset(e->zeros, 0, 256);
     if (r != hipSuccess) { delete e; PA_FAIL((pa_engine*)nullptr, "zero page: %s", hipGetErrorString(r)); }
     r = padel::init_misc_kernels();
+    if (r == hipSuccess) r = padel::init_head_tail_kernels();
     if (r != hipSuccess) { delete e; PA_FAIL((pa_engine*)nullptr, "kernel attributes: %s", hipGetErrorString(r)); }
     if (const char* v = getenv("PADEL_CONV_IMPL")) {
         if (v[0] == 'l') { delete e; PA_FAIL((pa_engine*)nullptr, "PADEL_CONV_IMPL=%s: the LDS kernel was retired in round 5; tap or bx3", v); }
@@ -169,6 +171,12 @@
     find_upsample_folds(m->d, m->fold_src, m->fold_dst);
     m->stem_fuse.resize(m->ops.size());
     for (size_t i = 0; i < m->ops.size(); ++i) m->stem_fuse[i] = stem_fusable(m->d, i);
+    m->tail = find_head_tail(m->d, m->fold_src);
+    m->tail_op.assign(m->ops.size(), 0);
+    if (m->tail.found)
+        for (int l = 0; l < 3; ++l)
+            for (int c = 0; c < 3; ++c)
+                if (m->tail.op[l][c] >= 0) m->tail_op[m->tail.op[l][c]] = 1;
     m->n_w = n_floats;
     hipError_t r = hipMalloc((void**)&m->d_w, n_floats * sizeof(float) + kConvReadSlack);
     if (r == hipSuccess)
@@ -206,6 +214,7 @@
     m->d_cand = nullptr; m->d_cidx = m->d_ccnt = nullptr; m->d_keys = nullptr; m->d_order = nullptr; m->d_supp = nullptr;
     m->d_oboxes = m->d_okpts = nullptr; m->d_ocnt = nullptr;
     m->planned = false;
+    m->heads_stale = false;
 }
 
 void pa_model_destroy(pa_model* m) {
@@ -258,7 +267,7 @@
     pa_engine* e = m->e;
     BufferPlan bp;
     std::string why;
-    if (plan_activations(m->d, m->fold_src, m->net_h, m->net_w, batch, e->t.alias != 0, bp, why)) PA_FAIL(e, "%s", why.c_str());
+    if (plan_activations(m->d, m->fold_src, m->net_h, m->net_w, batch, e->t.alias != 0, bp, why, &m->tail)) PA_FAIL(e, "%s", why.c_str());
     m->fc_nout = 0;
     for (const auto& o : m->ops) if (o.kind == PA_OP_GAP_FC) m->fc_nout = o.cout;
     if (m->fc_nout) {
@@ -339,11 +348,54 @@
     return lv;
 }
 
+void head_tail_convs(const pa_model* m, HeadTailArgs& a) {
+    bool single = m->e->t.w_single != 0;
+    for (int l = 0; l < 3; ++l)
+        for (int c = 0; c < 3; ++c) {
+            HeadTailConv& v = a.cv[l][c];
+            v = HeadTailConv{};
+            const int i = m->tail.op[l][c];
+            if (i < 0) continue;
+            const pa_op_desc& o = m->ops[i];
+            v.in = m->bptr[o.in_buf]; v.in_cs = m->bufs[o.in_buf].channels; v.in_choff = o.in_choff;
+            v.w = m->d_w + o.w_off; v.bias = m->d_w + o.b_off; v.oscale = m->d_w + o.reserved;
+            v.cin = o.cin; v.n16 = o.npad / 16;
+            single = single && (o.flags & PA_CONV_W_SINGLE);
+        }
+    a.w_single = single ? 1 : 0;
+}
+
+bool head_fused(const pa_model* m) {
+    const pa_engine* e = m->e;
+    if (!e->t.fuse_head || m->d.dtype != PA_DTYPE_H2 || !m->tail.found || e->profiling || e->t.timeline || !m->planned) return false;
+    HeadTailArgs a{};
+    a.d.cs = m->bufs[m->d.head_buf[0]].channels; a.d.nc = m->d.nc; a.d.nk = m->d.nk;
+    head_tail_convs(m, a);
+    return head_tail_h2_supported(a);
+}
+
+int run_tail_ops(pa_model* m, int n) {
+    pa_engine* e = m->e;
+    for (int l = 0; l < 3; ++l)
+        for (int c = 0; c < 3; ++c) {
+            const int i = m->tail.op[l][c];
+            if (i < 0) continue;
+            ConvArgs a{};
+            int path = CONV_PATH_TAP;
+            const int lv = conv_launch_args(m, (size_t)i, n, a, &path);
+            const hipError_t r = launch_conv(path, a, lv, e->stream);
+            if (r != hipSuccess) PA_FAIL(e, "op %d (head tail) launch failed: %s", i, hipGetErrorString(r));
+        }
+    return 0;
+}
+
 static int run_ops(pa_model* m, int n, size_t* pi) {
     pa_engine* e = m->e;
     hipStream_t s = e->stream;
+    const bool skip_tail = head_fused(m);
     for (size_t i = 0; i < m->ops.size(); ++i) {
         const pa_op_desc& o = m->ops[i];
+        if (skip_tail && m->tail_op[i]) continue;
         const pa_buf_desc& ob = m->bufs[o.out_buf];
         const int Ho = m->net_h >> ob.level, Wo = m->net_w >> ob.level;
         hipError_t r = hipSuccess;
diff --git a/padel_analytics_amd/csrc/engine_internal.h b/padel_analytics_amd/csrc/engine_internal.h
--- a/padel_analytics_amd/csrc/engine_internal.h
+++ b/padel_analytics_amd/csrc/engine_internal.h
@@ -25,6 +25,7 @@
     int fuse_stem = 1;
     int w_single = 1;
     int fuse_sppf = 1;
+    int fuse_head = 1;
     int fold_up = 1;
 };
 
@@ -90,6 +91,8 @@
     std::vector<int> fold_src;
     std::vector<int> fold_dst;
     std::vector<char> stem_fuse;
+    HeadTail tail;
+    std::vector<char> tail_op;
     float* d_w = nullptr;
     size_t n_w = 0;
     char* d_wr = nullptr;
@@ -128,6 +131,8 @@
     float* d_oboxes = nullptr; float* d_okpts = nullptr; int32_t* d_ocnt = nullptr;
     int32_t* d_classes = nullptr; int classes_cap = 0;
     int last_n = 0;
+    int last_post_path = 0;
+    bool heads_stale = false;
     std::vector<ProfRec> prof;
     size_t n_prof = 0;
 };
@@ -138,6 +143,9 @@
 void free_plan(pa_model* m);
 int plan_buffers(pa_model* m, int batch);
 int run_graph(pa_model* m, int n, size_t* pi);
+bool head_fused(const pa_model* m);
+void head_tail_convs(const pa_model* m, HeadTailArgs& a);
+int run_tail_ops(pa_model* m, int n);
 
 void jpeg_scratch_free(pa_engine* e);
 
diff --git a/padel_analytics_amd/csrc/engine_yolo.cpp b/padel_analytics_amd/csrc/engine_yolo.cpp
--- a/padel_analytics_amd/csrc/engine_yolo.cpp
+++ b/padel_analytics_amd/csrc/engine_yolo.cpp
@@ -40,7 +40,7 @@
 }
 
 static int run_post(pa_model* m, const pa_yolo_params* p, int nb, int oh, int ow, size_t* ppi, float* out_boxes, float* out_kpts,
-                int32_t* out_counts, int ovf_slot) {
+                int32_t* out_counts, int ovf_slot, bool fused) {
     pa_engine* e = m->e;
     hipStream_t s = e->stream;
     size_t& pi = *ppi;
@@ -54,9 +54,18 @@
     da.A = m->A; da.B = nb; da.conf = p->conf; da.classes = m->d_classes; da.n_classes = p->n_classes;
     da.cand = m->d_cand; da.cand_idx = m->d_cidx; da.cand_cnt = m->d_ccnt;
     pr = prof_begin(m, pi++, PROF_DECODE, 0, 0.0);
-    r = launch_decode(da, s);
+    if (fused) {
+        HeadTailArgs ha{};
+        ha.d = da;
+        head_tail_convs(m, ha);
+        r = launch_head_tail_h2(ha, s);
+    } else {
+        r = launch_decode(da, s);
+    }
     prof_end(m, pr);
-    if (r != hipSuccess) PA_FAIL(e, "decode launch failed: %s", hipGetErrorString(r));
+    if (r != hipSuccess) PA_FAIL(e, "%s launch failed: %s", fused ? "fused head tail" : "decode", hipGetErrorString(r));
+    m->last_post_path = fused ? 1 : 0;
+    m->heads_stale = fused;
     NmsArgs na{};
     na.cand = m->d_cand; na.cand_idx = m->d_cidx; na.cand_cnt = m->d_ccnt; na.keys = m->d_keys;
     na.order = m->d_order; na.supp = m->d_supp;
@@ -141,8 +150,9 @@
     }
     prof_end(m, pr);
     if (r != hipSuccess) PA_FAIL(e, "preprocess launch failed: %s", hipGetErrorString(r));
+    const bool fused = head_fused(m);
     if (run_graph(m, nb, &pi)) return 1;
-    return run_post(m, p, nb, oh, ow, &pi, out_boxes, m->d.nk ? out_kpts : nullptr, out_counts, ovf_slot);
+    return run_post(m, p, nb, oh, ow, &pi, out_boxes, m->d.nk ? out_kpts : nullptr, out_counts, ovf_slot, fused);
 }
 
 int pa_yolo_infer(pa_model* m, const uint8_t* frames, int n, int h, int w, const pa_yolo_params* p,
@@ -225,7 +235,7 @@
     const int S = p->imgsz;
     const int oh = p->pre_mode == PA_PRE_PIL_STRETCH ? S : h, ow = p->pre_mode == PA_PRE_PIL_STRETCH ? S : w;
     size_t pi = 0;
-    if (run_post(m, p, n, oh, ow, &pi, out_boxes, out_kpts, out_counts, PA_MAX_INFLIGHT)) return 1;
+    if (run_post(m, p, n, oh, ow, &pi, out_boxes, out_kpts, out_counts, PA_MAX_INFLIGHT, false)) return 1;
     PA_HIP(e, hipStreamSynchronize(s));
     m->last_n = n;
     finish_profile(m, pi);
@@ -242,11 +252,17 @@
     pa_engine* e = m->e;
     if (!m->planned || level < 0 || level > 2 || n > m->last_n) PA_FAIL(e, "pa_yolo_read_head: no plan / bad level / n");
     PA_HIP(e, hipSetDevice(e->dev));
+    if (m->heads_stale) {
+        if (run_tail_ops(m, m->last_n)) return 1;
+        m->heads_stale = false;
+    }
     const size_t bytes = (size_t)n * m->lv[level].H * m->lv[level].W * m->bufs[m->d.head_buf[0]].channels * sizeof(float);
     PA_HIP(e, hipMemcpyAsync(out, m->lv[level].buf, bytes, hipMemcpyDeviceToHost, e->stream));
     PA_HIP(e, hipStreamSynchronize(e->stream));
     return 0;
 }
+
+int pa_yolo_last_post_path(pa_model* m) { return m ? m->last_post_path : 0; }
 
 int pa_yolo_netin_shape(pa_model* m, int* h, int* w) {
     if (!m->planned || m->d.task == PA_TASK_TRACKNET) PA_FAIL(m->e, "pa_yolo_netin_shape: no YOLO plan");
diff --git a/padel_analytics_amd/csrc/graph_plan.cpp b/padel_analytics_amd/csrc/graph_plan.cpp
--- a/padel_analytics_amd/csrc/graph_plan.cpp
+++ b/padel_analytics_amd/csrc/graph_plan.cpp
@@ -192,8 +192,38 @@
     return true;
 }
 
+HeadTail find_head_tail(const pa_model_desc& d, const std::vector<int>& fold_src) {
+    HeadTail none, t;
+    if ((d.task != PA_TASK_DETECT && d.task != PA_TASK_POSE) || d.dtype != PA_DTYPE_H2 || d.nc < 1 || d.nk < 0) return none;
+    for (int l = 0; l < 3; ++l)
+        if (d.head_buf[l] < 0 || d.head_buf[l] >= d.n_bufs) return none;
+    const int want = d.nk > 0 ? 3 : 2;
+    for (int i = 0; i < d.n_ops; ++i) {
+        const pa_op_desc& o = d.ops[i];
+        const bool reads_in = o.kind != PA_OP_STEM && o.kind != PA_OP_STEM7;
+        if (reads_in && is_head_buf(d, o.in_buf)) return none;
+        if ((o.kind == PA_OP_CONV || o.kind == PA_OP_DWCONV3) && o.res_buf >= 0 && is_head_buf(d, o.res_buf)) return none;
+        if (o.kind == PA_OP_GAP_FC || !is_head_buf(d, o.out_buf)) continue;
+        int l = 0;
+        while (d.head_buf[l] != o.out_buf) ++l;
+        if (d.head_buf[(l + 1) % 3] == o.out_buf || d.head_buf[(l + 2) % 3] == o.out_buf) return none;
+        if (o.kind != PA_OP_CONV || o.ksize != 1 || o.stride != 1 || o.act != PA_ACT_NONE || o.res_buf >= 0) return none;
+        if (i < (int)fold_src.size() && fold_src[i] >= 0) return none;
+        const int c = o.out_choff == 0 ? 0 : o.out_choff == 64 ? 1 : (d.nk > 0 && o.out_choff == 64 + d.nc) ? 2 : -1;
+        if (c < 0 || o.cout != (c == 0 ? 64 : c == 1 ? d.nc : d.nk) || t.op[l][c] >= 0) return none;
+        for (int k = i + 1; k < d.n_ops; ++k)
+            if (d.ops[k].kind != PA_OP_GAP_FC && d.ops[k].out_buf == o.in_buf) return none;
+        t.op[l][c] = i;
+    }
+    for (int l = 0; l < 3; ++l)
+        for (int c = 0; c < want; ++c)
+            if (t.op[l][c] < 0) return none;
+    t.found = true;
+    return t;
+}
+
 int plan_activations(const pa_model_desc& d, const std::vector<int>& fold_src, int net_h, int net_w, int batch, bool alias,
-                     BufferPlan& out, std::string& err) {
+                     BufferPlan& out, std::string& err, const HeadTail* tail) {
     int maxl = 0;
     for (int i = 0; i < d.n_bufs; ++i) maxl = std::max(maxl, d.bufs[i].level);
     const int mask = (1 << maxl) - 1;
@@ -211,6 +241,10 @@
     if (d.task == PA_TASK_TRACKNET) touch(0, -1);
     const bool f16 = d.dtype == PA_DTYPE_F16;
     for (int l = 0; l < 3; ++l) touch(d.head_buf[l], nops + 1);
+    if (tail && tail->found)
+        for (int l = 0; l < 3; ++l)
+            for (int c = 0; c < 3; ++c)
+                if (tail->op[l][c] >= 0) touch(d.ops[tail->op[l][c]].in_buf, nops + 1);
     if (f16) for (int l = 0; l < 3; ++l) touch(d.head_buf[l], -1);
     std::vector<size_t> bytes(nb), off(nb, 0);
     size_t logical = 0;
diff --git a/padel_analytics_amd/csrc/graph_plan.h b/padel_analytics_amd/csrc/graph_plan.h
--- a/padel_analytics_amd/csrc/graph_plan.h
+++ b/padel_analytics_amd/csrc/graph_plan.h
@@ -14,12 +14,18 @@
 void find_upsample_folds(const pa_model_desc& d, std::vector<int>& fold_src, std::vector<int>& fold_dst);
 bool stem_fusable(const pa_model_desc& d, size_t i);
 
+struct HeadTail {
+    bool found = false;
+    int op[3][3] = {{-1, -1, -1}, {-1, -1, -1}, {-1, -1, -1}};
+};
+HeadTail find_head_tail(const pa_model_desc& d, const std::vector<int>& fold_src);
+
 struct BufferPlan {
     std::vector<size_t> off, bytes;
     size_t arena_bytes = 0, logical_bytes = 0;
 };
 int plan_activations(const pa_model_desc& d, const std::vector<int>& fold_src, int net_h, int net_w, int batch, bool alias,
-                     BufferPlan& out, std::string& err);
+                     BufferPlan& out, std::string& err, const HeadTail* tail = nullptr);
 
 struct YoloGeometry {
     int rw = 0, rh = 0, top = 0, left = 0, net_h = 0, net_w = 0, lb_mode = 0;
diff --git a/padel_analytics_amd/csrc/head_tail_h2.hip b/padel_analytics_amd/csrc/head_tail_h2.hip
--- /dev/null
+++ b/padel_analytics_amd/csrc/head_tail_h2.hip
@@ -0,0 +1,319 @@
+#include "h2_common.h"
+#include "decode_math.h"
+#include <algorithm>
+
+namespace padel {
+
+namespace {
+
+constexpr int kHtWaves = 4;
+constexpr int kHtClsFrags = 5;
+constexpr int kHtKptFrags = 4;
+constexpr int kHtRow = 68;
+constexpr size_t kHtMaxLds = 160 * 1024;
+
+constexpr size_t ht_conv_lds(int n16, int K, int P) { return (size_t)n16 * K * P * 1024 + (size_t)n16 * 16 * 8; }
+
+template <int K, int P>
+__device__ __forceinline__ void ht_stage(const HeadTailConv& cv, char* dst, int tid) {
+    const char* wsrc = reinterpret_cast<const char*>(cv.w);
+    const int units = cv.n16 * K * P * 64;
+    for (int u = tid; u < units; u += 64 * kHtWaves) {
+        const int ln = u & 63, t = u >> 6;
+        const int p = t % P, k = (t / P) % K, j = t / (P * K);
+        const char* src = wsrc + ((size_t)(j * 16 + (ln & 15)) * (K * 128) + k * 128 + p * 64 + (ln >> 4) * 16);
+        *reinterpret_cast<u32x4*>(dst + (size_t)u * 16) = *reinterpret_cast<const u32x4*>(src);
+    }
+    float* bs = reinterpret_cast<float*>(dst + (size_t)units * 16);
+    const int npad = cv.n16 * 16;
+    for (int u = tid; u < npad; u += 64 * kHtWaves) { bs[u] = cv.bias[u]; bs[npad + u] = cv.oscale[u]; }
+}
+
+template <int K>
+__device__ __forceinline__ void ht_load(const HeadTailConv& cv, int m, int lq, h16x8 (&ah)[K], h16x8 (&am)[K]) {
+    const float* p = cv.in + ((long long)m * cv.in_cs + cv.in_choff + (lq >> 1) * 16 + (lq & 1) * 4);
+    const bool absent = (cv.cin & 16) && lq >= 2;
+#pragma unroll
+    for (int k = 0; k < K; ++k) {
+        f32x4 h = {0.f, 0.f, 0.f, 0.f}, mm = h;
+        if (!(k == K - 1 && absent)) {
+            h = *reinterpret_cast<const f32x4*>(p + k * 32);
+            mm = *reinterpret_cast<const f32x4*>(p + k * 32 + 8);
+        }
+        ah[k] = __builtin_bit_cast(h16x8, h);
+        am[k] = __builtin_bit_cast(h16x8, mm);
+    }
+}
+
+template <int K, bool WS>
+__device__ __forceinline__ f32x4 ht_frag(const char* wl, const float* bs, int npad, int j, int lane, const h16x8 (&ah)[K], const h16x8 (&am)[K]) {
+    constexpr int P = WS ? 1 : 2;
+    const char* wj = wl + ((size_t)j * K * P * 64 + lane) * 16;
+    f32x4 cross = {0.f, 0.f, 0.f, 0.f}, part = cross, acc = cross;
+#pragma unroll
+    for (int k = 0; k < K; ++k) {
+        const h16x8 wh = __builtin_bit_cast(h16x8, *reinterpret_cast<const f32x4*>(wj + (k * P) * 1024));
+        cross = __builtin_amdgcn_mfma_f32_16x16x32_f16(wh, am[k], cross, 0, 0, 0);
+        if constexpr (!WS) {
+            const h16x8 wm = __builtin_bit_cast(h16x8, *reinterpret_cast<const f32x4*>(wj + (k * P + 1) * 1024));
+            cross = __builtin_amdgcn_mfma_f32_16x16x32_f16(wm, ah[k], cross, 0, 0, 0);
+        }
+        part = __builtin_amdgcn_mfma_f32_16x16x32_f16(wh, ah[k], k == 0 ? (f32x4){0.f, 0.f, 0.f, 0.f} : part, 0, 0, 0);
+    }
+    acc += part;
+    const int co0 = j * 16 + (lane >> 4) * 4;
+    const f32x4 b = *reinterpret_cast<const f32x4*>(bs + co0), sc = *reinterpret_cast<const f32x4*>(bs + npad + co0);
+    f32x4 v;
+#pragma unroll
+    for (int r = 0; r < 4; ++r) v[r] = h2_conv_value(cross[r], acc[r], sc[r], b[r]);
+    return v;
+}
+
+__device__ __forceinline__ void ht_wave_sync() {
+    __builtin_amdgcn_fence(__ATOMIC_RELEASE, "wavefront");
+    __builtin_amdgcn_wave_barrier();
+    __builtin_amdgcn_fence(__ATOMIC_ACQUIRE, "wavefront");
+}
+
+}
+
+template <int K2, int K3, int K4, bool WS>
+__global__ void __launch_bounds__(64 * kHtWaves, K2 + K3 + K4 <= 10 ? 3 : 2) head_tail_h2_kernel(const HeadTailArgs a) {
+    extern __shared__ __attribute__((aligned(16))) char ht_lds[];
+    constexpr int P = WS ? 1 : 2;
+    constexpr int K4A = K4 > 0 ? K4 : 1;
+    const int tid = threadIdx.x, lane = tid & 63, lr = lane & 15, lq = lane >> 4;
+    const int wave = __builtin_amdgcn_readfirstlane(tid >> 6);
+    const int bid = blockIdx.x;
+    const int l = bid >= a.wg_end[1] ? 2 : bid >= a.wg_end[0] ? 1 : 0;
+    const int wg0 = l == 2 ? a.wg_end[1] : l == 1 ? a.wg_end[0] : 0, nwg = (l == 2 ? a.wg_end[2] : l == 1 ? a.wg_end[1] : a.wg_end[0]) - wg0;
+    const HeadLevel lv = l == 2 ? a.d.lv[2] : l == 1 ? a.d.lv[1] : a.d.lv[0];
+    const HeadTailConv cbox = l == 2 ? a.cv[2][0] : l == 1 ? a.cv[1][0] : a.cv[0][0];
+    const HeadTailConv ccls = l == 2 ? a.cv[2][1] : l == 1 ? a.cv[1][1] : a.cv[0][1];
+    const HeadTailConv ckpt = l == 2 ? a.cv[2][2] : l == 1 ? a.cv[1][2] : a.cv[0][2];
+    const int nf3 = ccls.n16, nf4 = K4 > 0 ? ckpt.n16 : 0;
+    char* const wbox = ht_lds;
+    char* const wcls = wbox + ht_conv_lds(cbox.n16, K2, P);
+    char* const wkpt = wcls + ht_conv_lds(nf3, K3, P);
+    float* const tr = reinterpret_cast<float*>(wkpt + ht_conv_lds(nf4, K4A, P)) + wave * (16 * kHtRow);
+    const float* const bbox = reinterpret_cast<const float*>(wbox + (size_t)cbox.n16 * K2 * P * 1024);
+    const float* const bcls = reinterpret_cast<const float*>(wcls + (size_t)nf3 * K3 * P * 1024);
+    const float* const bkpt = reinterpret_cast<const float*>(wkpt + (size_t)nf4 * K4A * P * 1024);
+    ht_stage<K2, P>(cbox, wbox, tid);
+    ht_stage<K3, P>(ccls, wcls, tid);
+    if constexpr (K4 > 0) ht_stage<K4, P>(ckpt, wkpt, tid);
+    __syncthreads();
+
+    const int HW = lv.H * lv.W;
+    const int M = a.d.B * HW;
+    const int nfrag = (M + 15) >> 4;
+    const int nc = a.d.nc, nk = a.d.nk;
+    for (int f = (bid - wg0) * kHtWaves + wave; f < nfrag; f += nwg * kHtWaves) {
+        const int m_ = f * 16 + lr;
+        const bool valid = m_ < M;
+        const int m = valid ? m_ : M - 1;
+        h16x8 ah2[K2], am2[K2], ah3[K3], am3[K3], ah4[K4A], am4[K4A];
+        ht_load<K3>(ccls, m, lq, ah3, am3);
+        ht_load<K2>(cbox, m, lq, ah2, am2);
+        if constexpr (K4 > 0) ht_load<K4>(ckpt, m, lq, ah4, am4);
+
+        float cl[kHtClsFrags][4];
+        float mx = -INFINITY;
+#pragma unroll
+        for (int j = 0; j < kHtClsFrags; ++j) {
+            if (j < nf3) {
+                const f32x4 v = ht_frag<K3, WS>(wcls, bcls, nf3 * 16, j, lane, ah3, am3);
+#pragma unroll
+                for (int r = 0; r < 4; ++r) {
+                    cl[j][r] = v[r];
+                    if (j * 16 + lq * 4 + r < nc) mx = fmaxf(mx, v[r]);
+                }
+            }
+        }
+        mx = fmaxf(mx, __shfl_xor(mx, 16));
+        mx = fmaxf(mx, __shfl_xor(mx, 32));
+        const float score = sigmoidf_(mx);
+        bool pass = valid && score > a.d.conf;
+        if (__builtin_amdgcn_ballot_w64(pass) == 0ull) continue;
+        int cls = 0x7fffffff;
+        if (pass) {
+#pragma unroll
+            for (int j = 0; j < kHtClsFrags; ++j) {
+                if (j < nf3) {
+#pragma unroll
+                    for (int r = 0; r < 4; ++r) {
+                        const int c = j * 16 + lq * 4 + r;
+                        if (c < nc && c < cls && sigmoidf_(cl[j][r]) == score) cls = c;
+                    }
+                }
+            }
+        }
+        cls = min(cls, __shfl_xor(cls, 16));
+        cls = min(cls, __shfl_xor(cls, 32));
+        if (pass && a.d.n_classes > 0) {
+            bool ok = false;
+            for (int k = 0; k < a.d.n_classes; ++k) ok |= (a.d.classes[k] == cls);
+            pass = ok;
+        }
+        if (__builtin_amdgcn_ballot_w64(pass) == 0ull) continue;
+
+#pragma unroll
+        for (int j = 0; j < 4; ++j) {
+            const f32x4 v = ht_frag<K2, WS>(wbox, bbox, 64, j, lane, ah2, am2);
+            *reinterpret_cast<f32x4*>(tr + lr * kHtRow + j * 16 + lq * 4) = v;
+        }
+        ht_wave_sync();
+        float bins[16];
+#pragma unroll
+        for (int q = 0; q < 4; ++q) {
+            const f32x4 t = *reinterpret_cast<const f32x4*>(tr + lr * kHtRow + lq * 16 + q * 4);
+#pragma unroll
+            for (int r = 0; r < 4; ++r) bins[q * 4 + r] = t[r];
+        }
+        ht_wave_sync();
+        const float side = dfl_expect(bins);
+        float d[4];
+#pragma unroll
+        for (int s = 0; s < 4; ++s) d[s] = __shfl(side, lr + 16 * s);
+        const int b = m / HW, pix = m - b * HW;
+        float bx[4];
+        dfl_box(d, pix, lv.W, lv.stride, bx);
+
+        const bool mine = pass && lq == 0;
+        unsigned long long rem = __builtin_amdgcn_ballot_w64(mine);
+        while (rem) {
+            const int first = __builtin_ctzll(rem);
+            const int bb = __shfl(b, first);
+            const bool now = mine && b == bb;
+            const unsigned long long mk = __builtin_amdgcn_ballot_w64(now);
+            int base = 0;
+            if (lane == first) base = atomicAdd(&a.d.cand_cnt[bb], __builtin_popcountll(mk));
+            base = __shfl(base, first);
+            if (now) {
+                const int slot = base + __builtin_popcountll(mk & ((1ull << lane) - 1ull));
+                float* o = a.d.cand + ((long long)bb * a.d.A + slot) * 6;
+                o[0] = bx[0]; o[1] = bx[1]; o[2] = bx[2]; o[3] = bx[3]; o[4] = score; o[5] = (float)cls;
+                a.d.cand_idx[(long long)bb * a.d.A + slot] = lv.anchor0 + pix;
+            }
+            rem &= ~mk;
+        }
+
+        if constexpr (K4 > 0) {
+            float* const hk = const_cast<float*>(lv.buf) + ((long long)m * a.d.cs + 64 + nc);
+            for (int j = 0; j < nf4; ++j) {
+                const f32x4 v = ht_frag<K4, WS>(wkpt, bkpt, nf4 * 16, j, lane, ah4, am4);
+                if (pass) {
+#pragma unroll
+                    for (int r = 0; r < 4; ++r) {
+                        const int c = j * 16 + lq * 4 + r;
+                        if (c < nk) hk[c] = v[r];
+                    }
+                }
+            }
+        }
+    }
+}
+
+__global__ void head_tail_zero_kernel(int32_t* p, int n) {
+    const int i = blockIdx.x * 256 + threadIdx.x;
+    if (i < n) p[i] = 0;
+}
+
+namespace {
+
+struct HtShape { int k3, k4, nf3, nf4; bool ok; };
+
+HtShape ht_shape(const HeadTailArgs& a) {
+    HtShape s{0, 0, 0, 0, false};
+    const bool pose = a.d.nk > 0;
+    for (int l = 0; l < 3; ++l)
+        for (int c = 0; c < 3; ++c) {
+            const HeadTailConv& v = a.cv[l][c];
+            if (c == 2 && !pose) { if (v.in) return s; continue; }
+            const HeadTailConv& v0 = a.cv[0][c];
+            if (!v.in || !v.w || !v.bias || !v.oscale || v.cin < 16 || (v.cin & 15) || ((v.in_cs | v.in_choff) & 15) || v.cin != v0.cin || v.n16 != v0.n16)
+                return s;
+        }
+    const auto ksteps = [](int cin) { return (cin + 31) >> 5; };
+    s.k3 = ksteps(a.cv[0][1].cin); s.nf3 = a.cv[0][1].n16;
+    s.k4 = pose ? ksteps(a.cv[0][2].cin) : 0; s.nf4 = pose ? a.cv[0][2].n16 : 0;
+    if (ksteps(a.cv[0][0].cin) != 2 || a.cv[0][0].n16 != 4) return s;
+    if (s.k3 != 2 && s.k3 != 3 && s.k3 != 4 && s.k3 != 6 && s.k3 != 8) return s;
+    if (a.d.nc < 1 || s.nf3 < 1 || s.nf3 > kHtClsFrags || s.nf3 * 16 < a.d.nc) return s;
+    if (pose && (s.k4 != 2 || s.nf4 < 1 || s.nf4 > kHtKptFrags || s.nf4 * 16 < a.d.nk)) return s;
+    if (a.d.cs < 64 + a.d.nc + a.d.nk) return s;
+    s.ok = true;
+    return s;
+}
+
+size_t ht_lds_bytes(const HtShape& s, bool ws) {
+    const int P = ws ? 1 : 2;
+    return ht_conv_lds(4, 2, P) + ht_conv_lds(s.nf3, s.k3, P) + ht_conv_lds(s.nf4, s.k4 > 0 ? s.k4 : 1, P) + (size_t)kHtWaves * 16 * kHtRow * 4;
+}
+
+typedef void (*HtKernel)(const HeadTailArgs);
+template <int K3>
+HtKernel ht_pick(int k4, bool ws) {
+    if (k4) return ws ? head_tail_h2_kernel<2, K3, 2, true> : head_tail_h2_kernel<2, K3, 2, false>;
+    return ws ? head_tail_h2_kernel<2, K3, 0, true> : head_tail_h2_kernel<2, K3, 0, false>;
+}
+HtKernel ht_kernel(int k3, int k4, bool ws) {
+    switch (k3) {
+        case 2: return ht_pick<2>(k4, ws);
+        case 3: return ht_pick<3>(k4, ws);
+        case 4: return ht_pick<4>(k4, ws);
+        case 6: return ht_pick<6>(k4, ws);
+        case 8: return ht_pick<8>(k4, ws);
+    }
+    return nullptr;
+}
+
+}
+
+bool head_tail_h2_supported(const HeadTailArgs& a) {
+    const HtShape s = ht_shape(a);
+    return s.ok && ht_lds_bytes(s, a.w_single != 0) <= kHtMaxLds;
+}
+
+hipError_t init_head_tail_kernels() {
+    static const int k3s[] = {2, 3, 4, 6, 8};
+    for (int k3 : k3s)
+        for (int k4 = 0; k4 <= 2; k4 += 2)
+            for (int ws = 0; ws < 2; ++ws) {
+                const hipError_t e = hipFuncSetAttribute(reinterpret_cast<const void*>(ht_kernel(k3, k4, ws != 0)), hipFuncAttributeMaxDynamicSharedMemorySize, (int)kHtMaxLds);
+                if (e != hipSuccess) return e;
+            }
+    return hipSuccess;
+}
+
+hipError_t launch_head_tail_h2(const HeadTailArgs& a_in, hipStream_t s) {
+    const HtShape sh = ht_shape(a_in);
+    const bool ws = a_in.w_single != 0;
+    const size_t lds = ht_lds_bytes(sh, ws);
+    if (!sh.ok || lds > kHtMaxLds) return hipErrorNotSupported;
+    HeadTailArgs a = a_in;
+    static int ncu = 0;
+    if (!ncu) {
+        int dev = 0, n = 0;
+        if (hipGetDevice(&dev) != hipSuccess || hipDeviceGetAttribute(&n, hipDeviceAttributeMultiprocessorCount, dev) != hipSuccess || n < 1) n = 256;
+        ncu = n;
+    }
+    long long frags[3], total = 0;
+    for (int l = 0; l < 3; ++l) { frags[l] = ((long long)a.d.B * a.d.lv[l].H * a.d.lv[l].W + 15) / 16; total += frags[l]; }
+    if (total < 1) return hipErrorInvalidValue;
+    const long long budget = (long long)ncu * 3;
+    int end = 0;
+    for (int l = 0; l < 3; ++l) {
+        long long w = (budget * frags[l] + total - 1) / total;
+        w = std::min(w, (frags[l] + kHtWaves - 1) / kHtWaves);
+        end += (int)std::max(w, 1ll);
+        a.wg_end[l] = end;
+    }
+    hipLaunchKernelGGL(head_tail_zero_kernel, dim3((a.d.B + 255) / 256), dim3(256), 0, s, a.d.cand_cnt, a.d.B);
+    hipError_t e = hipGetLastError();
+    if (e != hipSuccess) return e;
+    hipLaunchKernelGGL(ht_kernel(sh.k3, sh.k4, ws), dim3(end), dim3(64 * kHtWaves), lds, s, a);
+    return hipGetLastError();
+}
+
+}
diff --git a/padel_analytics_amd/csrc/kernels.h b/padel_analytics_amd/csrc/kernels.h
--- a/padel_analytics_amd/csrc/kernels.h
+++ b/padel_analytics_amd/csrc/kernels.h
@@ -230,6 +230,23 @@
 };
 hipError_t launch_decode(const DecodeArgs& a, hipStream_t s);
 
+struct HeadTailConv {
+    const float* in;
+    const float* w;
+    const float* bias;
+    const float* oscale;
+    int in_cs, in_choff, cin, n16;
+};
+struct HeadTailArgs {
+    DecodeArgs d;
+    HeadTailConv cv[3][3];
+    int w_single;
+    int wg_end[3];
+};
+bool head_tail_h2_supported(const HeadTailArgs& a);
+hipError_t init_head_tail_kernels();
+hipError_t launch_head_tail_h2(const HeadTailArgs& a, hipStream_t s);
+
 struct NmsArgs {
     const float* cand; const int32_t* cand_idx; const int32_t* cand_cnt;
     uint64_t* keys;
diff --git a/padel_analytics_amd/csrc/postproc.hip b/padel_analytics_amd/csrc/postproc.hip
--- a/padel_analytics_amd/csrc/postproc.hip
+++ b/padel_analytics_amd/csrc/postproc.hip
@@ -1,8 +1,7 @@
 #include "kernels.h"
+#include "decode_math.h"
 
 namespace padel {
-
-__device__ __forceinline__ float sigmoidf_(float x) { return 1.0f / (1.0f + expf(-x)); }
 
 __global__ void __launch_bounds__(256) decode_kernel(const DecodeArgs a) {
     const int b = blockIdx.y;
@@ -39,24 +38,11 @@
 #pragma unroll
         for (int s = 0; s < 4; ++s) {
             float v[16];
-            float m = h[s * 16];
 #pragma unroll
-            for (int i = 0; i < 16; ++i) { v[i] = h[s * 16 + i]; m = fmaxf(m, v[i]); }
-            float sum = 0.0f;
-#pragma unroll
-            for (int i = 0; i < 16; ++i) { v[i] = expf(v[i] - m); sum += v[i]; }
-            float e = 0.0f;
-#pragma unroll
-            for (int i = 0; i < 16; ++i) e += (v[i] / sum) * (float)i;
-            d[s] = e;
-        }
-        const float ax = (float)(pix % lv.W) + 0.5f, ay = (float)(pix / lv.W) + 0.5f;
-        const float st = (float)lv.stride;
-        const float x1 = ax - d[0], y1 = ay - d[1], x2 = ax + d[2], y2 = ay + d[3];
-        const float cx = ((x1 + x2) / 2.0f) * st, cy = ((y1 + y2) / 2.0f) * st;
-        const float w = (x2 - x1) * st, hh = (y2 - y1) * st;
-        const float hw = w / 2.0f, hhh = hh / 2.0f;
-        bx[0] = cx - hw; bx[1] = cy - hhh; bx[2] = cx + hw; bx[3] = cy + hhh;
+            for (int i = 0; i < 16; ++i) v[i] = h[s * 16 + i];
+            d[s] = dfl_expect(v);
+        }
+        dfl_box(d, pix, lv.W, lv.stride, bx);
     }
     const unsigned long long m = __builtin_amdgcn_ballot_w64(pass);
     if (m == 0ull) return;
diff --git a/padel_analytics_amd/engine.py b/padel_analytics_amd/engine.py
--- a/padel_analytics_amd/engine.py
+++ b/padel_analytics_amd/engine.py
@@ -85,6 +85,7 @@
 
 PRE_LETTERBOX, PRE_PIL_STRETCH = 0, 1
 YUV_NV12, YUV_I420 = 0, 1
+POST_PATH_DECODE, POST_PATH_FUSED = 0, 1
 YUV_PATH_VECTOR, YUV_PATH_BYTE = 1, 2
 
 ABI_SYMBOLS = [
@@ -106,6 +107,7 @@
     "pa_render", "pa_render_check", "pa_render_last_path", "pa_glyph_rows", "pa_ball_read_resized",
     "pa_jpeg_encode", "pa_jpeg_check", "pa_jpeg_interval_bytes",
     "pa_jpeg_parse", "pa_jpeg_decode", "pa_jpeg_decode_last_path", "pa_jpeg_decode_last_times",
+    "pa_yolo_last_post_path",
 ]
 
 
@@ -144,6 +146,7 @@
     lib.pa_yolo_wait.argtypes = [vp, i32, C.POINTER(C.c_int)]
     lib.pa_yolo_head_shape.argtypes = [vp, i32, C.POINTER(i32), C.POINTER(i32), C.POINTER(i32)]
     lib.pa_yolo_read_head.argtypes = [vp, i32, i32, vp]
+    lib.pa_yolo_last_post_path.argtypes = [vp]
     lib.pa_tracknet_infer.argtypes = [vp, vp, i32, i32, i32, i32, vp, i32]
     lib.pa_resnet_infer.argtypes = [vp, vp, i32, i32, i32, i32, vp, vp]
     lib.pa_resnet_read_netin.argtypes = [vp, i32, vp]
@@ -760,6 +763,9 @@
         self.engine._check(self.engine.lib.pa_yolo_read_head(self.handle, level, n, out.ctypes.data))
         return out
 
+    def last_post_path(self) -> int:
+        return int(self.engine.lib.pa_yolo_last_post_path(self.handle))
+
     def read_netin(self, n: int) -> np.ndarray:
         hh, ww = C.c_int(), C.c_int()
         self.engine._check(self.engine.lib.pa_yolo_netin_shape(self.handle, C.byref(hh), C.byref(ww)))
```
